# dgrzech/ir-sgmcmc

Measured on AMD Instinct MI355X. Metric: SG-MCMC transitions/sec (full _SGLD_transition), higher is better.
Workload: dtype f32; 1 GPU; 256^3 synthetic pair, SVF_3D 12 steps, GMM(K=4)/LCC(s=1) + virtual decimation, RegLoss_L2 w=1.4, Sobolev s=3, uniform noise 0.1, SGLD lr 0.4, Philox noise; init=identity, chains=1, parallelism=1 independent chain(s)

## Files before the change

### include/irsgmcmc.h

```cpp
#ifndef IRSGMCMC_H
#define IRSGMCMC_H

#include <stddef.h>
#include <stdint.h>

#ifdef __cplusplus
extern "C" {
#endif
#pragma GCC visibility push(default)

#define IRS_MAX_COMPONENTS 8
#define IRS_MAX_CHAINS 8
#define IRS_MAX_HALF_WIDTH 4
#define IRS_MAX_LABELS 64
#define IRS_HAUSDORFF_MAX_PERCENTILES 4

enum { IRS_DATA_GMM_LCC = 0, IRS_DATA_SSD = 1 };
enum { IRS_REG_L2 = 0, IRS_REG_LOGNORMAL = 1, IRS_REG_STUDENT = 2, IRS_REG_LOGNORMAL_L2 = 3 };


int irs_perturb_smooth(const float* v, const float* sigma, const float* eps, float tau, const float* kernel, int s,
                       int C, int D, int H, int W, float* tmp, float* out, uint64_t seed, uint64_t iteration,
                       void* stream);

// ... 178 lines not shown
#define IRS_RESIDUAL_MAX_BINS 512
#define IRS_RESIDUAL_MAX_BLOCKS 1024
#define IRS_RESIDUAL_WS_BYTES (IRS_MAX_CHAINS * IRS_RESIDUAL_MAX_BLOCKS * (3 + 4) * 8)
#define IRS_RESIDUAL_MAP_SUMMARY_INTS 2
#define IRS_RESIDUAL_MAP_SUMMARY_FLOATS 2
#define IRS_RESIDUAL_MAP_WS_BYTES (1024 * (IRS_RESIDUAL_MAP_SUMMARY_INTS + IRS_RESIDUAL_MAP_SUMMARY_FLOATS) * 8)
int irs_residual_histogram(const float* residuals, int C, const uint8_t* mask, int D, int H, int W, float half_range, int bins,
                           long long* hist, long long* counts, double* sums, int records_before, void* ws, size_t ws_bytes,
                           void* stream);
int irs_residual_nll_update(const float* residuals, int C, int D, int H, int W, const double* log_weight, const double* inv_std,
                            int K, float* mean, int32_t* count, int records_before, void* stream);
int irs_residual_nll_finalize(const float* mean, const int32_t* count, const uint8_t* mask, int D, int H, int W,
                              long long* isummary, double* fsummary, void* ws, size_t ws_bytes, void* stream);

int irs_restrict_image(const float* im, int Cim, int D, int H, int W, float* out, int d, int h, int w, void* stream);
int irs_restrict_mask(const uint8_t* mask, int Cm, int D, int H, int W, uint8_t* out, int d, int h, int w, void* stream);
int irs_prolong_field(const float* x, int C, int ch, int d, int h, int w, float* out, int D, int H, int W, void* stream);

#define IRS_AFFINE_SUMS 94
#define IRS_AFFINE_PARTIALS 76
#define IRS_AFFINE_MAX_BLOCKS 512
#define IRS_AFFINE_WS_BYTES (IRS_AFFINE_MAX_BLOCKS * IRS_AFFINE_PARTIALS * 8)
int irs_affine_normal_equations(const float* fixed, const float* moving, const uint8_t* mask, int D, int H, int W, const double* lin,
                                const double* shift, double* sums, void* ws, size_t ws_bytes, void* stream);
int irs_affine_transformation(const double* lin, const double* shift, float* out, int D, int H, int W, void* stream);
int irs_affine_compose(const float* transformation, const double* lin, const double* shift, float* total_transformation,
                       float* total_displacement, int C, int D, int H, int W, void* stream);

int irs_bspline_prefilter(const float* im, float* coeff, int Cim, int D, int H, int W, void* stream);
int irs_bspline_warp(const float* coeff, int Cim, const float* transformation, float* out, int C, int D, int H, int W, void* stream);
int irs_native_warp_cubic(const float* displacement, int C, const int32_t* dims, const int32_t* native, const int32_t* padding,
                          const float* im, const float* coeff, int Cim, float fill, float* im_out, void* stream);

#define IRS_MASK_MIN_BINS 2
#define IRS_MASK_MAX_BINS 4096
#define IRS_MASK_MAX_KEEP 64
#define IRS_MASK_MAX_RADIUS 16
int irs_intensity_histogram(const float* im, int C, const uint8_t* mask, int Cm, int D, int H, int W, float lo, float hi, int bins,
                            long long* hist, void* stream);
int irs_mask_threshold(const float* im, int C, int D, int H, int W, float threshold, uint8_t* out, void* stream);
int irs_connected_components_workspace(int C, int D, int H, int W, size_t* bytes);
int irs_connected_components(const uint8_t* mask, int C, int D, int H, int W, int connectivity, int32_t* labels, int32_t* counts,
                             void* ws, size_t ws_bytes, void* stream);
int irs_mask_select_workspace(int C, int D, int H, int W, size_t* bytes);
int irs_mask_keep_largest(const uint8_t* mask, int C, int D, int H, int W, int connectivity, int keep, uint8_t* out, void* ws,
                          size_t ws_bytes, void* stream);
int irs_mask_fill_holes(const uint8_t* mask, int C, int D, int H, int W, uint8_t* out, void* ws, size_t ws_bytes, void* stream);
int irs_mask_morphology_workspace(int C, int D, int H, int W, size_t* bytes);
int irs_mask_dilate(const uint8_t* mask, int C, int D, int H, int W, int r2, int erode, uint8_t* out, void* ws, size_t ws_bytes,
                    void* stream);

#define IRS_LANDMARK_MAX_POINTS (1 << 24)
#define IRS_LANDMARK_COLUMNS 10
#define IRS_LANDMARK_SUMMARY_INTS 3
#define IRS_LANDMARK_SUMMARY_FLOATS 4
#define IRS_LANDMARK_WS_BYTES (1024 * (IRS_LANDMARK_SUMMARY_INTS + IRS_LANDMARK_SUMMARY_FLOATS) * 8)
int irs_transform_points(const float* points, int K, const float* displacement, int C, int D, int H, int W, const float* scale,
                         const float* offset, float* sampled, float* mapped, void* stream);
int irs_landmark_update(const float* mapped, const float* target, int C, int K, double* mean, double* comoment, double* tre_mean,
                        double* tre_m2, double* tre_max, int32_t* count, int records_before, void* stream);
int irs_landmark_finalize(const double* mean, const double* comoment, const double* tre_mean, const double* tre_m2,
                          const double* tre_max, const int32_t* count, const float* target, int K, double* out, long long* isummary,
                          double* fsummary, void* ws, size_t ws_bytes, void* stream);


typedef struct irs_config {
    int32_t dims[3];
    int32_t cps[3];
    int32_t no_chains;
    int32_t no_steps;
    int32_t sobolev_s;
    float sobolev_kernel[2 * IRS_MAX_HALF_WIDTH + 1];
    float lr;
    float uniform_alpha;
    int32_t virtual_decimation;
    int32_t data_loss;
    int32_t lcc_s;
    int32_t gmm_components;
    float ssd_sigma;
    float gmm_lr_log_std, gmm_lr_logits, gmm_lr_decay;
    float adam_beta1, adam_beta2, adam_eps;
    float scale_prior_loc, scale_prior_scale;
    float dirichlet_concentration[IRS_MAX_COMPONENTS];
    int32_t reg_loss;
    int32_t reg_learnable;
    float w_reg;
    double dof;
    float reg_lr0, reg_lr1, reg_lr_decay;
    float loc_prior_nu, loc_prior_w_reg;
    float reg_scale_prior_loc, reg_scale_prior_scale;
    double w_reg_prior_shape, w_reg_prior_rate;
    uint64_t seed;
} irs_config;

typedef struct irs_state {
    float gmm_log_std[IRS_MAX_COMPONENTS];
    float gmm_logits[IRS_MAX_COMPONENTS];
    double gmm_adam_m[2][IRS_MAX_COMPONENTS];
    double gmm_adam_v[2][IRS_MAX_COMPONENTS];
    int64_t gmm_adam_step[2];
    double reg_param[2];
    double reg_adam_m[2], reg_adam_v[2];
    int64_t reg_adam_step[2];
    uint64_t iteration;
} irs_state;

typedef struct irs_scalars {
    double alpha[IRS_MAX_CHAINS];
    double data_term[IRS_MAX_CHAINS];
    double reg_term[IRS_MAX_CHAINS];
    double reg_energy[IRS_MAX_CHAINS];
    double n_mask[IRS_MAX_CHAINS];
} irs_scalars;

typedef struct irs_io {
    const float* fixed_im;
    const float* moving_im;
    const uint8_t* mask;
    int32_t fixed_chains, moving_chains, mask_chains;
    float* v;
    const float* sigma;
    const float* eps;
    const float* unif;
    float* curr_state;
    float* im_moving_warped;
    float* residuals;
    float* displacement;
    float* transformation;
    float* grad_v;
} irs_io;

typedef struct irs_ctx irs_ctx;

int irs_create(const irs_config* cfg, irs_ctx** out);
void irs_destroy(irs_ctx* ctx);
size_t irs_workspace_bytes(const irs_ctx* ctx);
int irs_velocity_dims(const irs_ctx* ctx, int32_t out[3]);

int irs_set_fixed(irs_ctx* ctx, const float* fixed_im, int fixed_chains, void* stream);
int irs_get_state(irs_ctx* ctx, irs_state* out, void* stream);
int irs_set_state(irs_ctx* ctx, const irs_state* in, void* stream);
int irs_get_scalars(irs_ctx* ctx, irs_scalars* out, void* stream);

int irs_gmm_init(irs_ctx* ctx, const irs_io* io, const float* v_sample, int warm_up, void* stream);

int irs_transition(irs_ctx* ctx, const irs_io* io, void* stream);

int irs_flush(irs_ctx* ctx, void* stream);
int irs_recovered_transitions(const irs_ctx* ctx, uint64_t* out);
int irs_sparse_adjoint_set(irs_ctx* ctx, int on);
int irs_sparse_adjoint_get(irs_ctx* ctx, int32_t* out, void* stream);
int irs_sparse_data_set(irs_ctx* ctx, int on);
int irs_sparse_data_get(irs_ctx* ctx, int32_t* out, void* stream);

typedef struct irs_timings {
    float total_ms;
    float exp_fwd_ms;
    float exp_bwd_kernel_ms;
    float exp_bwd_total_ms;
    float smooth_ms;
    float data_ms;
    float update_ms;
    float exp_bwd_primary_avg_ms;
} irs_timings;
int irs_transition_timed(irs_ctx* ctx, const irs_io* io, void* stream, irs_timings* out);

typedef struct irs_comm irs_comm;
#define IRS_COMM_ID_BYTES 128
int irs_comm_unique_id(uint8_t id[IRS_COMM_ID_BYTES]);
int irs_comm_create_rccl(const uint8_t id[IRS_COMM_ID_BYTES], int rank, int world, irs_comm** out);
int irs_comm_create_ipc(const char* name, int rank, int world, irs_comm** out);
typedef struct irs_xfer {
    void* ptr;
    size_t bytes;
    int32_t peer;
    int32_t recv;
} irs_xfer;
typedef int (*irs_exchange_fn)(void* user, const irs_xfer* xfers, int n, void* stream);
typedef int (*irs_allreduce_fn)(void* user, void* buf, size_t count, int kind, void* stream);
int irs_comm_create_callbacks(irs_exchange_fn ex, irs_allreduce_fn ar, void* user, int rank, int world, irs_comm** out);
void irs_comm_destroy(irs_comm* comm);
int irs_comm_probe(irs_comm* comm, size_t bytes, size_t ar_doubles, int iters, void* stream, double usec[2]);
int irs_comm_describe(const irs_comm* comm, char* out, size_t n);
int irs_comm_rank(const irs_comm* comm);
int irs_comm_world(const irs_comm* comm);
int irs_comm_selftest(irs_comm* comm, void* stream);

typedef struct irs_slab_config {
    int32_t ghost_max;
    int32_t margin;
} irs_slab_config;
typedef struct irs_slab_layout {
    int32_t rank, world;
    int32_t a, b;
    int32_t lo, hi;
    int32_t margin, ghost_max;
} irs_slab_layout;
int irs_slab_plan_layout(const irs_config* cfg, const irs_slab_config* scfg, int rank, int world, irs_slab_layout* out);
int irs_slab_create(const irs_config* cfg, const irs_slab_config* scfg, irs_comm* comm, irs_ctx** out);
int irs_slab_get_layout(const irs_ctx* ctx, irs_slab_layout* out);
int irs_slab_transition(irs_ctx* ctx, const irs_io* io, void* stream);
int irs_slab_gmm_init(irs_ctx* ctx, const irs_io* io, const float* v_sample, int warm_up, void* stream);
typedef struct irs_slab_status {
    uint64_t transitions, exact_transitions;
    uint64_t exchanges, exchanged_bytes;
    uint64_t mispredictions;
    int32_t last_fwd_rounds, last_bwd_rounds;
} irs_slab_status;
int irs_slab_status_get(irs_ctx* ctx, irs_slab_status* out, void* stream);
typedef struct irs_slab_timeline_entry {
    int32_t kind;
    int32_t stage;
    int32_t k, width;
    float ready_us;
    float handover_us;
    float wait_at_us;
    float stall_us;
} irs_slab_timeline_entry;
int irs_slab_timeline_arm(irs_ctx* ctx, int transitions);
int irs_slab_timeline_get(irs_ctx* ctx, irs_slab_timeline_entry* out, int max_entries, int32_t* n_entries, float* total_us, void* stream);

int irs_slab_plan_rounds(const int32_t* h, int n, int ghost_max, int min_slab, int n_buffers, int32_t* fwd_round, int32_t* fwd_width,
                         int32_t* n_fwd, int32_t* bwd_round, int32_t* bwd_width, int32_t* n_bwd);

enum { IRS_OP_LAUNCH = 0, IRS_OP_EXCHANGE = 1, IRS_OP_ALLREDUCE = 2, IRS_OP_WAIT = 3 };
enum {
    IRS_SG_PERTURB = 0, IRS_SG_COPY_V, IRS_SG_SMOOTH, IRS_SG_ENERGY, IRS_SG_EXP_FWD, IRS_SG_OUTPUTS, IRS_SG_WARP, IRS_SG_RESIDUAL,
    IRS_SG_STATS, IRS_SG_DATA_BWD, IRS_SG_WARP_BWD, IRS_SG_EXP_BWD, IRS_SG_UPDATE, IRS_SG_FFD_UP, IRS_SG_FFD_ADJ,
    IRS_SG_SCALARS = 32,
    IRS_SG_CHAIN_SCALAR = 32, IRS_SG_REG_SCALAR, IRS_SG_FINALIZE, IRS_SG_VERDICT
};
enum {
    IRS_SB_V = 0, IRS_SB_NOISY, IRS_SB_VS, IRS_SB_WARPED, IRS_SB_Z, IRS_SB_GM, IRS_SB_GRAD_A, IRS_SB_GRAD_B,
    IRS_SB_DENSE,
    IRS_SB_GRAD_C,
    IRS_SB_STEP0 = 16
};
enum { IRS_AR_ENERGY = 0, IRS_AR_DMAX = 1, IRS_AR_NLL = 2, IRS_AR_STATS = 3, IRS_AR_CPGRAD = 4, IRS_AR_MOMENTS = 7 };
typedef struct irs_slab_op {
    int32_t kind;
    int32_t stage;
    int32_t k;
    int32_t lo0, hi0, lo1, hi1;
    int32_t in0, in1;
    int32_t reach;
    int32_t out;
    int32_t width;
    int32_t id;
} irs_slab_op;
int irs_slab_trace(const irs_config* cfg, const irs_slab_config* scfg, int rank, int world, const int32_t* h, irs_slab_op* ops,
                   int max_ops, int32_t* n_ops);

int irs_option_set(irs_ctx* ctx, const char* name, int value);

const char* irs_last_error(void);
const char* irs_version(void);

#pragma GCC visibility pop
#ifdef __cplusplus
}
#endif
#endif
```

### ir_sgmcmc_amd/_lib.py

```python
import ctypes as C
import os

import torch

_HERE = os.path.dirname(os.path.abspath(__file__))
LIB_PATH = os.environ.get('IRS_LIB') or os.path.join(_HERE, 'csrc', 'libirsgmcmc.so')

IRS_MAX_COMPONENTS = 8
IRS_MAX_CHAINS = 8
IRS_MAX_HALF_WIDTH = 4
IRS_MAX_LABELS = 64
IRS_HAUSDORFF_MAX_PERCENTILES = 4
IRS_LABEL_BINS = 10
IRS_JACOBIAN_SUMMARY_INTS, IRS_JACOBIAN_SUMMARY_FLOATS = 4, 5
IRS_JACOBIAN_WS_BYTES = 1024 * (IRS_JACOBIAN_SUMMARY_INTS + IRS_JACOBIAN_SUMMARY_FLOATS) * 8
IRS_IMAGE_POSTERIOR_MAX_VOLUMES, IRS_IMAGE_POSTERIOR_SUMMARY_INTS, IRS_IMAGE_POSTERIOR_SUMMARY_FLOATS = 8, 4, 6
IRS_IMAGE_POSTERIOR_WS_BYTES = 1024 * (IRS_IMAGE_POSTERIOR_SUMMARY_INTS + IRS_IMAGE_POSTERIOR_SUMMARY_FLOATS) * 8
IRS_COVARIANCE_SUMMARY_INTS, IRS_COVARIANCE_SUMMARY_FLOATS = 2, 8
IRS_COVARIANCE_WS_BYTES = 1024 * (IRS_COVARIANCE_SUMMARY_INTS + IRS_COVARIANCE_SUMMARY_FLOATS) * 8
IRS_COMPARE_SUMMARY_INTS, IRS_COMPARE_SUMMARY_FLOATS = 4, 13
IRS_COMPARE_WS_BYTES = 1024 * (IRS_COMPARE_SUMMARY_INTS + IRS_COMPARE_SUMMARY_FLOATS) * 8
IRS_QUANTILE_MIN_BINS, IRS_QUANTILE_MAX_BINS, IRS_QUANTILE_MAX_PROBS, IRS_QUANTILE_MAX_RECORDS = 4, 256, 8, 65535
IRS_QUANTILE_SUMMARY_INTS, IRS_QUANTILE_SUMMARY_FLOATS = 3, 5
IRS_QUANTILE_WS_BYTES = 1024 * (IRS_QUANTILE_SUMMARY_INTS + IRS_QUANTILE_SUMMARY_FLOATS) * 8
# ... 61 lines not shown
        ('fixed_im', C.c_void_p), ('moving_im', C.c_void_p), ('mask', C.c_void_p),
        ('fixed_chains', C.c_int32), ('moving_chains', C.c_int32), ('mask_chains', C.c_int32),
        ('v', C.c_void_p), ('sigma', C.c_void_p), ('eps', C.c_void_p), ('unif', C.c_void_p),
        ('curr_state', C.c_void_p), ('im_moving_warped', C.c_void_p), ('residuals', C.c_void_p),
        ('displacement', C.c_void_p), ('transformation', C.c_void_p), ('grad_v', C.c_void_p),
    ]


class IrsTimings(C.Structure):
    _fields_ = [(n, C.c_float) for n in ('total_ms', 'exp_fwd_ms', 'exp_bwd_kernel_ms', 'exp_bwd_total_ms', 'smooth_ms',
                                         'data_ms', 'update_ms', 'exp_bwd_primary_avg_ms')]


class IrsXfer(C.Structure):
    _fields_ = [('ptr', C.c_void_p), ('bytes', C.c_size_t), ('peer', C.c_int32), ('recv', C.c_int32)]


class IrsSlabConfig(C.Structure):
    _fields_ = [('ghost_max', C.c_int32), ('margin', C.c_int32)]


class IrsSlabLayout(C.Structure):
    _fields_ = [(n, C.c_int32) for n in ('rank', 'world', 'a', 'b', 'lo', 'hi', 'margin', 'ghost_max')]


class IrsSlabStatus(C.Structure):
    _fields_ = [('transitions', C.c_uint64), ('exact_transitions', C.c_uint64), ('exchanges', C.c_uint64),
                ('exchanged_bytes', C.c_uint64), ('mispredictions', C.c_uint64), ('last_fwd_rounds', C.c_int32),
                ('last_bwd_rounds', C.c_int32)]


class IrsSlabTimelineEntry(C.Structure):
    _fields_ = [('kind', C.c_int32), ('stage', C.c_int32), ('k', C.c_int32), ('width', C.c_int32), ('ready_us', C.c_float),
                ('handover_us', C.c_float), ('wait_at_us', C.c_float), ('stall_us', C.c_float)]


class IrsSlabOp(C.Structure):
    _fields_ = [(n, C.c_int32) for n in ('kind', 'stage', 'k', 'lo0', 'hi0', 'lo1', 'hi1', 'in0', 'in1', 'reach', 'out', 'width', 'id')]


IRS_OP_LAUNCH, IRS_OP_EXCHANGE, IRS_OP_ALLREDUCE, IRS_OP_WAIT = range(4)
(IRS_SG_PERTURB, IRS_SG_COPY_V, IRS_SG_SMOOTH, IRS_SG_ENERGY, IRS_SG_EXP_FWD, IRS_SG_OUTPUTS, IRS_SG_WARP, IRS_SG_RESIDUAL, IRS_SG_STATS,
 IRS_SG_DATA_BWD, IRS_SG_WARP_BWD, IRS_SG_EXP_BWD, IRS_SG_UPDATE, IRS_SG_FFD_UP, IRS_SG_FFD_ADJ) = range(15)
IRS_SG_CHAIN_SCALAR, IRS_SG_REG_SCALAR, IRS_SG_FINALIZE = 32, 33, 34
(IRS_SB_V, IRS_SB_NOISY, IRS_SB_VS, IRS_SB_WARPED, IRS_SB_Z, IRS_SB_GM, IRS_SB_GRAD_A, IRS_SB_GRAD_B, IRS_SB_DENSE, IRS_SB_GRAD_C) = range(10)
IRS_SB_STEP0 = 16
IRS_COMM_ID_BYTES = 128
EXCHANGE_FN = C.CFUNCTYPE(C.c_int, C.c_void_p, C.POINTER(IrsXfer), C.c_int, C.c_void_p)
ALLREDUCE_FN = C.CFUNCTYPE(C.c_int, C.c_void_p, C.c_void_p, C.c_size_t, C.c_int, C.c_void_p)

_P, _I, _F, _U64 = C.c_void_p, C.c_int, C.c_float, C.c_uint64
_I32P = C.POINTER(C.c_int32)

SIGNATURES = {
    'irs_perturb_smooth': [_P, _P, _P, _F, _P, _I, _I, _I, _I, _I, _P, _P, _U64, _U64, _P],
    'irs_svf_exp_fwd': [_P, _P, _P, _P, _I, _I, _I, _I, _I, _P],
    'irs_svf_exp_bwd': [_P, _P, _P, _P, _P, _I, _I, _I, _I, _I, _P],
    'irs_ffd_up': [_P, _P, _P, _I, _I, _I, _I, _I, _I, _I, _P],
    'irs_ffd_adjoint': [_P, _P, _P, _I, _I, _I, _I, _I, _I, _I, _P],
    'irs_warp_fwd': [_P, _I, _P, _P, _F, _P, _I, _I, _I, _I, _U64, _U64, _P],
    'irs_warp_bwd': [_P, _I, _P, _P, _F, _P, _P, _I, _I, _I, _I, _U64, _U64, _P],
    'irs_warp_transformation': [_P, _I, _P, _P, _I, _I, _I, _I, _P],
    'irs_warp_nearest_u8': [_P, _I, _P, _P, _I, _I, _I, _I, _P],
    'irs_warp_nearest_i16': [_P, _I, _P, _P, _I, _I, _I, _I, _P],
    'irs_lcc_normalise': [_P, _P, _P, _I, _I, _I, _I, _I, _P],
    'irs_lcc_map_fwd': [_P, _I, _P, _P, _P, _I, _I, _I, _I, _I, _P],
    'irs_lcc_map_bwd': [_P, _I, _P, _P, _P, _P, _I, _I, _I, _I, _I, _P],
    'irs_reg_energy': [_P, _P, _P, _I, _I, _I, _I, _P],
    'irs_reduce_scratch_doubles': [],
    'irs_gradient_operator': [_P, _P, _I, _I, _I, _I, _I, _P],
    'irs_log_det_jacobian': [_P, _P, _P, _I, _I, _I, _I, _P],
    'irs_label_boxes': [_P, _I, _P, _I32P, _I, _P, _I, _I, _I, _I, _P],
    'irs_surface_distance_workspace': [_I32P, _I, _I, _I, _I, C.POINTER(C.c_size_t)],
    'irs_label_surface_distance': [_P, _I, _P, _I32P, _I, C.POINTER(C.c_float), _I32P, _P, C.c_size_t, _P, _P, _I, _I, _I, _I,
                                   _P],
    'irs_hausdorff_workspace': [_I32P, _I, _I, _I, _I, _I, C.POINTER(C.c_size_t)],
    'irs_label_hausdorff_distance': [_P, _I, _P, _I32P, _I, C.POINTER(C.c_float), _I32P, _P, C.c_size_t, C.POINTER(C.c_double), _I,
                                     _P, _P, _P, _P, _I, _I, _I, _I, _P],
    'irs_surface_posterior_workspace': [_I32P, _I, _I, _I, _I, C.POINTER(C.c_size_t)],
    'irs_surface_posterior_update': [_P, _P, _I32P, _I, C.POINTER(C.c_float), _I32P, _P, C.c_size_t, _P, _P, _P, _I, _I, _I, _I, _P],
    'irs_surface_posterior_finalize': [_P, _I32P, _I, _P, _P, _P, _P, C.POINTER(C.c_double), _I, _P, _P, _P, _P, _P, C.c_size_t,
                                       _I, _I, _I, _P],
    'irs_chain_moments_update': [_P, _I, _I, _I, _I, _I, _I, _P, _P, _P],
    'irs_split_rhat_workspace': [_I, _I, _I, _I, C.POINTER(C.c_size_t)],
    'irs_split_rhat': [_P, _P, _I, _I, _P, C.c_float, C.c_float, _P, _P, _P, C.c_size_t, _I, _I, _I, _P],
    'irs_chain_variogram_update': [_P, _I, _I, _I, _I, _I, _I, _P, _P, _P],
    'irs_split_ess_workspace': [_I, _I, _I, _I, C.POINTER(C.c_size_t)],
    'irs_split_ess': [_P, _P, _P, _I, _I, _I, _P, C.c_float, _P, _P, _P, _P, C.c_size_t, _I, _I, _I, _P],
    'irs_label_posterior_workspace': [_I, _I, _I, _I, _I, C.POINTER(C.c_size_t)],
    'irs_label_posterior_update': [_P, _I, _I, _I, _I, _I32P, _I, _P, _P, _I, _P, C.c_size_t, _P],
    'irs_label_posterior_finalize': [_P, _I, _I, _I, _I, _I, _I32P, _P, _P, _P, _P, _P, _P, _P, C.c_size_t, _P],
    'irs_jacobian_posterior_update': [_P, _I, _I, _I, _I, _P, _P, _P, _I, _P],
    'irs_jacobian_posterior_finalize': [_P, _P, _P, _I, _I, _I, _I, _P, _P, _P, _P, _P, _P, _P, C.c_size_t, _P],
    'irs_image_posterior_update': [_P, _I, _P, _I, _I, _I, _I, _P, _P, _P, _P, _I, _P],
    'irs_image_posterior_finalize': [_P, _P, _P, _P, _I, _I, _I, _I, _P, _F, _P, _P, _P, _P, _P, _P, _P, C.c_size_t, _P],
    'irs_displacement_covariance_update': [_P, _I, _I, _I, _I, _P, _P, _I, _P],
    'irs_displacement_covariance_finalize': [_P, _P, _I, _I, _I, _I, C.POINTER(C.c_float), _P, _P, _P, _P, _P, _P, _P, C.c_size_t, _P],
    'irs_posterior_compare': [_P, _P, _I, _P, _P, _I, _I, _I, _I, C.POINTER(C.c_float), C.c_double, _P, _P, _P, _P, _P, _P, _P, _P, C.c_size_t,
                              _P],
    'irs_displacement_quantiles_update': [_P, _I, _I, _I, _I, _P, _P, _I, C.POINTER(C.c_float), _I, _P],
    'irs_displacement_quantiles_finalize': [_P, _P, _I, _I, _I, _I, _I, C.POINTER(C.c_float), C.POINTER(C.c_float),
                                            C.POINTER(C.c_double), _I, _P, _P, _P, _P, _P, _P, C.c_size_t, _P],
    'irs_svf_exp_inverse': [_P, _P, _P, _P, _I, _I, _I, _I, _I, _P],
    'irs_inverse_consistency': [_P, _P, _P, C.POINTER(C.c_float), _P, _I, _P, _P, _P, _P, _P, C.c_size_t, _I, _I, _I, _I, _P],
    'irs_inverse_consistency_update': [_P, _I, _I, _I, _I, _P, _P, _I, _P],
    'irs_inverse_consistency_finalize': [_P, _P, _I, _I, _I, _P, _F, _P, _P, _P, C.c_size_t, _P],
    'irs_native_warp': [_P, _I, _I32P, _I32P, _I32P, _P, _P, _P, _I, _F, C.POINTER(C.c_float), _P, _P, _P, _P, _P],
    'irs_image_similarity_workspace': [_I, _I, C.POINTER(C.c_size_t)],
    'irs_image_similarity': [_P, _I, _P, _I, _P, _I, _I, _I, _F, _F, _F, _F, _I, _P, _P, _P, C.c_size_t, _P],
    'irs_transform_points': [_P, _I, _P, _I, _I, _I, _I, C.POINTER(C.c_float), _P, _P, _P, _P],
    'irs_landmark_update': [_P, _P, _I, _I, _P, _P, _P, _P, _P, _P, _I, _P],
    'irs_landmark_finalize': [_P, _P, _P, _P, _P, _P, _P, _I, _P, _P, _P, _P, C.c_size_t, _P],
    'irs_local_similarity': [_P, _I, _P, _I, _P, _I, _I, _I, _I, C.c_double, C.c_double, C.c_double, C.c_double, _P, _P, _P, _P,
                             C.c_size_t, _P],
    'irs_local_similarity_update': [_P, _I, _I, _I, _I, _P, _P, _P, _I, _P],
    'irs_local_similarity_finalize': [_P, _P, _P, _P, _I, _I, _I, _P, _P, _P, C.c_size_t, _P],
    'irs_residual_histogram': [_P, _I, _P, _I, _I, _I, _F, _I, _P, _P, _P, _I, _P, C.c_size_t, _P],
    'irs_residual_nll_update': [_P, _I, _I, _I, _I, C.POINTER(C.c_double), C.POINTER(C.c_double), _I, _P, _P, _I, _P],
    'irs_residual_nll_finalize': [_P, _P, _P, _I, _I, _I, _P, _P, _P, C.c_size_t, _P],
    'irs_restrict_image': [_P, _I, _I, _I, _I, _P, _I, _I, _I, _P],
    'irs_restrict_mask': [_P, _I, _I, _I, _I, _P, _I, _I, _I, _P],
    'irs_prolong_field': [_P, _I, _I, _I, _I, _I, _P, _I, _I, _I, _P],
    'irs_affine_normal_equations': [_P, _P, _P, _I, _I, _I, C.POINTER(C.c_double), C.POINTER(C.c_double), _P, _P, C.c_size_t, _P],
    'irs_affine_transformation': [C.POINTER(C.c_double), C.POINTER(C.c_double), _P, _I, _I, _I, _P],
    'irs_affine_compose': [_P, C.POINTER(C.c_double), C.POINTER(C.c_double), _P, _P, _I, _I, _I, _I, _P],
    'irs_bspline_prefilter': [_P, _P, _I, _I, _I, _I, _P],
    'irs_bspline_warp': [_P, _I, _P, _P, _I, _I, _I, _I, _P],
    'irs_native_warp_cubic': [_P, _I, _I32P, _I32P, _I32P, _P, _P, _I, _F, _P, _P],
    'irs_intensity_histogram': [_P, _I, _P, _I, _I, _I, _I, _F, _F, _I, _P, _P],
    'irs_mask_threshold': [_P, _I, _I, _I, _I, _F, _P, _P],
    'irs_connected_components_workspace': [_I, _I, _I, _I, C.POINTER(C.c_size_t)],
    'irs_connected_components': [_P, _I, _I, _I, _I, _I, _P, _P, _P, C.c_size_t, _P],
    'irs_mask_select_workspace': [_I, _I, _I, _I, C.POINTER(C.c_size_t)],
    'irs_mask_keep_largest': [_P, _I, _I, _I, _I, _I, _I, _P, _P, C.c_size_t, _P],
    'irs_mask_fill_holes': [_P, _I, _I, _I, _I, _P, _P, C.c_size_t, _P],
    'irs_mask_morphology_workspace': [_I, _I, _I, _I, C.POINTER(C.c_size_t)],
    'irs_mask_dilate': [_P, _I, _I, _I, _I, _I, _I, _P, _P, C.c_size_t, _P],
    'irs_create': [C.POINTER(IrsConfig), C.POINTER(_P)],
    'irs_destroy': [_P],
    'irs_workspace_bytes': [_P],
    'irs_velocity_dims': [_P, C.POINTER(C.c_int32 * 3)],
    'irs_set_fixed': [_P, _P, _I, _P],
    'irs_get_state': [_P, C.POINTER(IrsState), _P],
    'irs_set_state': [_P, C.POINTER(IrsState), _P],
    'irs_get_scalars': [_P, C.POINTER(IrsScalars), _P],
    'irs_gmm_init': [_P, C.POINTER(IrsIO), _P, _I, _P],
    'irs_transition': [_P, C.POINTER(IrsIO), _P],
    'irs_flush': [_P, _P],
    'irs_recovered_transitions': [_P, C.POINTER(C.c_uint64)],
    'irs_sparse_adjoint_set': [_P, _I],
    'irs_sparse_adjoint_get': [_P, _I32P, _P],
    'irs_sparse_data_set': [_P, _I],
    'irs_sparse_data_get': [_P, _I32P, _P],
    'irs_transition_timed': [_P, C.POINTER(IrsIO), _P, C.POINTER(IrsTimings)],
    'irs_comm_unique_id': [C.POINTER(C.c_uint8 * IRS_COMM_ID_BYTES)],
    'irs_comm_create_rccl': [C.POINTER(C.c_uint8 * IRS_COMM_ID_BYTES), _I, _I, C.POINTER(_P)],
    'irs_comm_create_ipc': [C.c_char_p, _I, _I, C.POINTER(_P)],
    'irs_comm_create_callbacks': [EXCHANGE_FN, ALLREDUCE_FN, _P, _I, _I, C.POINTER(_P)],
    'irs_comm_destroy': [_P],
    'irs_comm_probe': [_P, C.c_size_t, C.c_size_t, _I, _P, C.POINTER(C.c_double * 2)],
    'irs_comm_describe': [_P, C.c_char_p, C.c_size_t],
    'irs_comm_rank': [_P],
    'irs_comm_world': [_P],
    'irs_comm_selftest': [_P, _P],
    'irs_slab_plan_layout': [C.POINTER(IrsConfig), C.POINTER(IrsSlabConfig), _I, _I, C.POINTER(IrsSlabLayout)],
    'irs_slab_create': [C.POINTER(IrsConfig), C.POINTER(IrsSlabConfig), _P, C.POINTER(_P)],
    'irs_slab_get_layout': [_P, C.POINTER(IrsSlabLayout)],
    'irs_slab_transition': [_P, C.POINTER(IrsIO), _P],
    'irs_slab_gmm_init': [_P, C.POINTER(IrsIO), _P, _I, _P],
    'irs_slab_status_get': [_P, C.POINTER(IrsSlabStatus), _P],
    'irs_slab_timeline_arm': [_P, _I],
    'irs_slab_timeline_get': [_P, C.POINTER(IrsSlabTimelineEntry), _I, _I32P, C.POINTER(C.c_float), _P],
    'irs_slab_trace': [C.POINTER(IrsConfig), C.POINTER(IrsSlabConfig), _I, _I, _I32P, C.POINTER(IrsSlabOp), _I, _I32P],
    'irs_slab_plan_rounds': [_I32P, _I, _I, _I, _I, _I32P, _I32P, _I32P, _I32P, _I32P, _I32P],
    'irs_option_set': [_P, C.c_char_p, _I],
    'irs_last_error': [],
    'irs_version': [],
}
_RESTYPES = {'irs_reduce_scratch_doubles': C.c_size_t, 'irs_workspace_bytes': C.c_size_t, 'irs_destroy': None,
             'irs_comm_destroy': None,
             'irs_last_error': C.c_char_p, 'irs_version': C.c_char_p}

_lib = None


class IrsError(RuntimeError):
    pass


def load(path=None):
    global _lib
    if _lib is not None and path is None:
        return _lib
    p = path or LIB_PATH
    if not os.path.isfile(p):
        raise IrsError(f'{p} not found: build it with `python -c "import __graft_entry__ as g; g.build()"` '
                       f'(or `make -C ir_sgmcmc_amd/csrc`). There is no CPU fallback.')
    lib = C.CDLL(p)
    for name, argtypes in SIGNATURES.items():
        fn = getattr(lib, name)
        fn.argtypes = argtypes
        fn.restype = _RESTYPES.get(name, C.c_int)
    if path is None:
        _lib = lib
    return lib


def option_set(name, value, ctx=None):
    check(load().irs_option_set(ctx, name.encode(), int(value)))


def check(rc):
    if rc != 0:
        raise IrsError(load().irs_last_error().decode())


def stream_ptr():
    return C.c_void_p(torch.cuda.current_stream().cuda_stream)


def dev_ptr(t, dtype=None, allow_none=False):
    if t is None:
        if allow_none:
            return None
        raise IrsError('required tensor is None')
    if not t.is_cuda:
        raise IrsError('ir_sgmcmc_amd operators run on the GPU only (got a CPU tensor); there is no CPU fallback')
    if dtype is not None and t.dtype != dtype:
        raise IrsError(f'expected {dtype}, got {t.dtype}')
    if not t.is_contiguous():
        raise IrsError('tensor must be contiguous')
    return C.c_void_p(t.data_ptr())
```

### ir_sgmcmc_amd/csrc/adjoint_plan.h

```cpp
#pragma once

#if defined(__HIPCC__)
#define IRS_HD __host__ __device__ inline
#else
#define IRS_HD inline
#endif

namespace irs {

#ifndef IRS_MTX
#define IRS_MTX 32
#define IRS_MTY 8
#endif
constexpr int kPlanTX = IRS_MTX, kPlanTY = IRS_MTY;
#ifndef IRS_BWD_MAX_SEG
#define IRS_BWD_MAX_SEG 64
#endif
constexpr int kPlanMaxLen = IRS_BWD_MAX_SEG;
constexpr int kPlanMinLen = 8;
constexpr int kPlanMinForced = 4;
constexpr int kPlanStats = 4;

struct PlanEntry {
    int chain, tile, z0, z1, fill, pad;
};

struct ColPlan {
    int lo, hi, f0, f1;
};

IRS_HD int plan_min(int a, int b) { return a < b ? a : b; }
IRS_HD int plan_max(int a, int b) { return a > b ? a : b; }

IRS_HD void plan_widen(int a, int b, int m, int D, int& lo, int& hi) {
    lo = hi = 0;
    if (b <= 0) return;
    lo = plan_max(D - a - m, 0);
    hi = plan_min(b + m, D);
}

IRS_HD ColPlan plan_column(int lo, int hi, int nlo, int nhi) {
    const bool run = hi > lo, need = nhi > nlo;
    if (!run) return need ? ColPlan{nhi, nhi, nlo, nhi} : ColPlan{0, 0, 0, 0};
    return ColPlan{lo, hi, need ? plan_min(lo, nlo) : lo, need ? plan_max(hi, nhi) : hi};
}

IRS_HD ColPlan plan_column_of(const int* runs, int k, int col, int C, int ntx, int nty, int D) {
    const int tiles = ntx * nty, chain = col / tiles, tile = col - chain * tiles, tx = tile % ntx, ty = tile / ntx;
    const int* r = runs + ((long long)k * C * tiles + col) * 2;
    int nlo = 0, nhi = D;
    if (k > 0) {
        nlo = D;
        nhi = 0;
        const int* prev = runs + ((long long)(k - 1) * C + chain) * tiles * 2;
        for (int dy = -1; dy <= 1; ++dy)
            for (int dx = -1; dx <= 1; ++dx) {
                const int ux = plan_min(plan_max(tx + dx, 0), ntx - 1), uy = plan_min(plan_max(ty + dy, 0), nty - 1);
                const int l = prev[(uy * ntx + ux) * 2], h = prev[(uy * ntx + ux) * 2 + 1];
                if (h > l) {
                    nlo = plan_min(nlo, plan_max(l - 1, 0));
                    nhi = plan_max(nhi, plan_min(h + 1, D));
                }
            }
    }
    return plan_column(r[0], r[1], nlo, nhi);
}

constexpr int kLccTX = 32, kLccTY = 16;
constexpr int kWarpTX = 64, kWarpTY = 8;
constexpr int kDataKernels = 4;
enum PlanFill { kFillNext = 0, kFillAll = 1, kFillNone = 2 };
struct PlanShape {
    int tx, ty;
    int reach0, reach_dec;
    int fill[2];
    int G[2];
    int lmin;
};
IRS_HD int plan_reach(const PlanShape& s, int k) { return s.reach0 - k * s.reach_dec; }
IRS_HD int plan_fill_of(const PlanShape& s, int k) { return s.fill[k > 0 ? 1 : 0]; }
IRS_HD int plan_resident_of(const PlanShape& s, int k) { return s.G[k > 0 ? 1 : 0]; }
IRS_HD void plan_tile_window(int t, int size, int m, int n, int& a, int& b) {
    a = plan_max(t * size - m, 0);
    b = plan_min(t * size + size + m, n);
}
IRS_HD ColPlan plan_column_by(const int* runs, int k, int col, int C, int ntx, int nty, int D, int fill) {
    if (fill == kFillNext) return plan_column_of(runs, k, col, C, ntx, nty, D);
    const int* r = runs + ((long long)k * C * ntx * nty + col) * 2;
    return fill == kFillAll ? plan_column(r[0], r[1], 0, D) : plan_column(r[0], r[1], 0, 0);
}

IRS_HD int plan_pieces(int len, int L) { return len > 0 ? (len + L - 1) / L : 0; }

IRS_HD void plan_cut(int lo, int len, int np, int j, int& z0, int& z1) {
    z0 = lo + (int)((long long)len * j / np);
    z1 = lo + (int)((long long)len * (j + 1) / np);
}

IRS_HD PlanEntry plan_entry(const ColPlan& c, int chain, int tile, int np, int j) {
    int z0, z1;
    plan_cut(c.lo, c.hi - c.lo, np, j, z0, z1);
    return PlanEntry{chain, tile, z0, z1, 0, 0};
}
IRS_HD bool plan_has_fill(const ColPlan& c, int side) { return side == 0 ? c.f0 < c.lo : c.hi < c.f1 && c.hi > c.lo; }
IRS_HD PlanEntry plan_fill_entry(const ColPlan& c, int chain, int tile, int side) {
    return side == 0 ? PlanEntry{chain, tile, c.f0, c.lo, 1, 0} : PlanEntry{chain, tile, c.hi, c.f1, 1, 0};
}

IRS_HD int plan_pick_len(const int* pieces, int G, int lmin, int lmax) {
    for (int L = lmin; L < lmax; ++L)
        if (pieces[L] <= G) return L;
    return lmax;
}

IRS_HD int plan_run_bound(int columns, int D, int G, int forced_len) {
    const int lmax = plan_max(plan_min(kPlanMaxLen, D), 1);
    if (forced_len > 0) return columns * plan_pieces(D, plan_min(plan_max(forced_len, kPlanMinForced), lmax));
    return plan_max(G, columns * plan_pieces(D, lmax));
}

IRS_HD int plan_entries_cap(int columns, int D) { return columns * ((D + kPlanMinForced - 1) / kPlanMinForced + 2); }

IRS_HD int plan_swizzle(int id, int count, int run) {
    if (run <= 1) return id;
    const int group = 8 * run;
    if (id >= count / group * group) return id;
    const int g = id / group, w = id - g * group;
    return g * group + (w & 7) * run + (w >> 3);
}

}
```

### ir_sgmcmc_amd/csrc/adjoint_plan.hip

```cpp
#include "adjoint_plan.h"

#include "kernels.h"

namespace irs {

constexpr int kExtChunk = 32;

template <typename T>
__device__ __forceinline__ void extent_body(const T* __restrict__ g, int* __restrict__ ext, const Vol& vol) {
    const int x = (int)blockIdx.x * 64 + ((int)threadIdx.x & 63), y = (int)blockIdx.y * 4 + ((int)threadIdx.x >> 6);
    const int nch = (vol.D + kExtChunk - 1) / kExtChunk;
    const int chain = (int)blockIdx.z / nch, za = ((int)blockIdx.z - chain * nch) * kExtChunk, zb = min(za + kExtChunk, vol.D);
    if (x >= vol.W || y >= vol.H) return;
    const int64_t plane = (int64_t)vol.H * vol.W;
    const T* __restrict__ p = g + (int64_t)chain * vol.V + (int64_t)y * vol.W + x;
    int lo = vol.D, hi = -1;
#pragma unroll 8
    for (int z = za; z < zb; ++z) {
        const bool nz = p[z * plane] != (T)0;
        lo = nz ? min(lo, z) : lo;
        hi = nz ? z : hi;
    }
    if (hi < 0) return;
    int* e = ext + ((int64_t)chain * plane + (int64_t)y * vol.W + x) * 2;
// ... 14 lines not shown
    else hipLaunchKernelGGL(mask_extent_kernel, grid, dim3(kBlock), 0, st, mask, ext, vol);
}

__device__ __forceinline__ bool chain_is_dense(const unsigned* __restrict__ dmax, int chain, int C, int no_steps) {
    bool dense = false;
    if (!dmax) return false;
    for (int k = 0; k < no_steps; ++k) {
        const unsigned* b = dmax + ((int64_t)k * C + chain) * 4;
        const float m = fmaxf(fmaxf(__uint_as_float(b[0]), __uint_as_float(b[1])), __uint_as_float(b[2]));
        dense |= !(m < 1.0f);
    }
    return dense;
}

__global__ __launch_bounds__(kWave) void plan_runs_kernel(const int* __restrict__ ext, int ext_chains, const unsigned* __restrict__ dmax,
                                                          int* __restrict__ runs, Vol vol, int C, int no_steps, int ntx, int nty,
                                                          PlanShape shape) {
    const int col = (int)blockIdx.x, k = (int)blockIdx.y, tiles = ntx * nty;
    const int chain = col / tiles, tile = col - chain * tiles, tx = tile % ntx, ty = tile / ntx;
    int* out = runs + ((int64_t)k * C * tiles + col) * 2;
    if (chain_is_dense(dmax, chain, C, no_steps)) {
        if (threadIdx.x == 0) {
            out[0] = 0;
            out[1] = vol.D;
        }
        return;
    }
    const int m = plan_reach(shape, k);
    int x0, x1, y0, y1;
    plan_tile_window(tx, shape.tx, m, vol.W, x0, x1);
    plan_tile_window(ty, shape.ty, m, vol.H, y0, y1);
    const int nx = x1 - x0, n = nx * (y1 - y0);
    const int* __restrict__ e = ext + (int64_t)(ext_chains == 1 ? 0 : chain) * vol.H * vol.W * 2;
    int lo = vol.D, hi = 0;
    for (int i = (int)threadIdx.x; i < n; i += kWave) {
        const int yy = i / nx, xx = i - yy * nx;
        const int2 ab = *reinterpret_cast<const int2*>(e + ((int64_t)(y0 + yy) * vol.W + x0 + xx) * 2);
        int l, h;
        plan_widen(ab.x, ab.y, m, vol.D, l, h);
        if (h > l) {
            lo = min(lo, l);
            hi = max(hi, h);
        }
    }
#pragma unroll
    for (int off = kWave / 2; off > 0; off >>= 1) {
        lo = min(lo, __shfl_xor(lo, off, kWave));
        hi = max(hi, __shfl_xor(hi, off, kWave));
    }
    if (threadIdx.x == 0) {
        out[0] = hi > lo ? lo : 0;
        out[1] = hi > lo ? hi : 0;
    }
}

constexpr int kPlanBlock = 1024;
__device__ __forceinline__ int block_rank(bool flag, int* wave_tot, int& total) {
    const unsigned long long b = __ballot(flag);
    const int lane = (int)threadIdx.x & (kWave - 1), w = (int)threadIdx.x / kWave;
    if (lane == 0) wave_tot[w] = __popcll(b);
    __syncthreads();
    int before = 0;
    total = 0;
#pragma unroll
    for (int i = 0; i < kPlanBlock / kWave; ++i) {
        before += i < w ? wave_tot[i] : 0;
        total += wave_tot[i];
    }
    __syncthreads();
    return before + __popcll(b & ((1ull << lane) - 1ull));
}

__global__ __launch_bounds__(kPlanBlock) void plan_lists_kernel(const int* __restrict__ runs, const unsigned* __restrict__ dmax,
                                                                ColPlan* __restrict__ colplan, PlanEntry* __restrict__ entries,
                                                                int* __restrict__ count, int* __restrict__ stats, Vol vol, int C,
                                                                int no_steps, int ntx, int nty, int cap, PlanShape shape, int forced_len) {
    __shared__ int pieces[kPlanMaxLen + 1], s_maxlen, s_L, s_nrun, wave_tot[kPlanBlock / kWave];
    __shared__ int s_pieces[IRS_MAX_CHAINS], s_planes[IRS_MAX_CHAINS];
    const int k = (int)blockIdx.x, tiles = ntx * nty, cols = C * tiles, tid = (int)threadIdx.x;
    const int lmax = max(min(kPlanMaxLen, vol.D), 1), lmin = min(shape.lmin, lmax);
    const int fill = plan_fill_of(shape, k);
    ColPlan* __restrict__ cps = colplan + (int64_t)k * cols;
    for (int i = tid; i <= kPlanMaxLen; i += kPlanBlock) pieces[i] = 0;
    if (tid < IRS_MAX_CHAINS) s_pieces[tid] = s_planes[tid] = 0;
    if (tid == 0) s_maxlen = s_nrun = 0;
    __syncthreads();
    for (int col = tid; col < cols; col += kPlanBlock) {
        const ColPlan cp = plan_column_by(runs, k, col, C, ntx, nty, vol.D, fill);
        cps[col] = cp;
        const int len = cp.hi - cp.lo;
        if (len > 0) {
            atomicMax(&s_maxlen, len);
            atomicAdd(&s_planes[col / tiles], len);
        }
    }
    __syncthreads();
    const int n_len = lmax - lmin + 1, groups = kPlanBlock / n_len;
    if (forced_len <= 0 && tid < groups * n_len) {
        const int L = lmin + tid % n_len;
        int sum = 0;
        for (int col = tid / n_len; col < cols; col += groups) sum += plan_pieces(cps[col].hi - cps[col].lo, L);
        atomicAdd(&pieces[L], sum);
    }
    __syncthreads();
    if (tid == 0)
        s_L = forced_len > 0 ? min(max(forced_len, kPlanMinForced), lmax) : plan_pick_len(pieces, plan_resident_of(shape, k), lmin, lmax);
    __syncthreads();
    const int L = s_L, levels = plan_pieces(s_maxlen, L);
    PlanEntry* list = entries + (int64_t)k * cap;
    const int stream = (levels + 2) * cols;
    int base = 0;
    for (int i0 = 0; i0 < stream; i0 += kPlanBlock) {
        const int i = i0 + tid;
        bool flag = false;
        ColPlan cp = {0, 0, 0, 0};
        int np = 0, j = 0, col = 0;
        if (i < stream) {
            j = i / cols;
            col = i - j * cols;
            cp = cps[col];
            np = plan_pieces(cp.hi - cp.lo, L);
            flag = j < levels ? j < np : plan_has_fill(cp, j - levels);
        }
        const unsigned long long runs_here = __ballot(flag && j < levels);
        if ((tid & (kWave - 1)) == 0 && runs_here) atomicAdd(&s_nrun, __popcll(runs_here));
        int total;
        const int pos = base + block_rank(flag, wave_tot, total);
        if (flag && pos < cap) {
            list[pos] = j < levels ? plan_entry(cp, col / tiles, col % tiles, np, j) : plan_fill_entry(cp, col / tiles, col % tiles, j - levels);
            atomicAdd(&s_pieces[col / tiles], 1);
        }
        base += total;
    }
    __syncthreads();
    if (tid == 0) {
        count[2 * k] = min(base, cap);
        count[2 * k + 1] = min(s_nrun, cap);
    }
    if (tid < C) {
        int* s = stats + ((int64_t)k * C + tid) * kPlanStats;
        s[0] = chain_is_dense(dmax, tid, C, no_steps) ? 0 : 1;
        s[1] = L;
        s[2] = s_pieces[tid];
        s[3] = s_planes[tid];
    }
}

static size_t plan_align(size_t b) { return (b + 255) / 256 * 256; }

struct PlanLayout {
    size_t ext, runs, colplan, entries, count, stats, total;
    int cap, ntx, nty;
};
static PlanLayout plan_layout(Vol vol, int C, int no_steps) {
    PlanLayout l;
    l.ntx = (vol.W + kPlanTX - 1) / kPlanTX;
    l.nty = (vol.H + kPlanTY - 1) / kPlanTY;
    const size_t cols = (size_t)C * l.ntx * l.nty;
    l.cap = plan_entries_cap((int)cols, vol.D);
    size_t off = 0;
    auto take = [&](size_t bytes) { const size_t o = off; off += plan_align(bytes); return o; };
    l.ext = take(sizeof(int) * 2 * (size_t)C * vol.H * vol.W);
    l.runs = take(sizeof(int) * 2 * cols * no_steps);
    l.colplan = take(sizeof(ColPlan) * cols * no_steps);
    l.entries = take(sizeof(PlanEntry) * (size_t)l.cap * no_steps);
    l.count = take(sizeof(int) * 2 * no_steps);
    l.stats = take(sizeof(int) * kPlanStats * (size_t)C * no_steps);
    l.total = off;
    return l;
}

size_t adjoint_plan_bytes(Vol vol, int C, int no_steps) { return plan_layout(vol, C, no_steps).total; }

AdjointPlan adjoint_plan_views(char* base, Vol vol, int C, int no_steps) {
    const PlanLayout l = plan_layout(vol, C, no_steps);
    AdjointPlan p;
    p.ext = (int*)(base + l.ext);
    p.runs = (int*)(base + l.runs);
    p.colplan = (ColPlan*)(base + l.colplan);
    p.entries = (PlanEntry*)(base + l.entries);
    p.count = (int*)(base + l.count);
    p.stats = (int*)(base + l.stats);
    p.cap = l.cap;
    p.ntx = l.ntx;
    p.nty = l.nty;
    return p;
}

void launch_adjoint_plan(const float* g_warped, const unsigned* dmax, const AdjointPlan& plan, int no_steps, int C, Vol vol,
                         int64_t G, int forced_len, hipStream_t st) {
    const int g = (int)(G > 0 ? G : 1024);
    const PlanShape shape{kPlanTX, kPlanTY, no_steps, 1, {kFillNext, kFillNext}, {g, g}, kPlanMinLen};
    launch_extent(g_warped, nullptr, plan.ext, C, vol, st);
    hipLaunchKernelGGL(plan_runs_kernel, dim3((unsigned)(C * plan.ntx * plan.nty), (unsigned)no_steps), dim3(kWave), 0, st, plan.ext, C, dmax,
                       plan.runs, vol, C, no_steps, plan.ntx, plan.nty, shape);
    hipLaunchKernelGGL(plan_lists_kernel, dim3((unsigned)no_steps), dim3(kPlanBlock), 0, st, plan.runs, dmax, plan.colplan, plan.entries, plan.count,
                       plan.stats, vol, C, no_steps, plan.ntx, plan.nty, plan.cap, shape, forced_len);
}

struct DataLayout {
    size_t ext, runs, hull, colplan, entries, count, stats, nll, total;
    int cap, ntx, nty, wtx, wty;
};
static DataLayout data_layout(Vol vol, int C) {
    DataLayout l;
    l.ntx = (vol.W + kLccTX - 1) / kLccTX;
    l.nty = (vol.H + kLccTY - 1) / kLccTY;
    l.wtx = (vol.W + kWarpTX - 1) / kWarpTX;
    l.wty = (vol.H + kWarpTY - 1) / kWarpTY;
    const size_t cols = (size_t)C * l.ntx * l.nty;
    l.cap = plan_entries_cap((int)cols, vol.D);
    size_t off = 0;
    auto take = [&](size_t bytes) { const size_t o = off; off += plan_align(bytes); return o; };
    l.ext = take(sizeof(int) * 2 * (size_t)C * vol.H * vol.W);
    l.runs = take(sizeof(int) * 2 * cols * 2);
    l.hull = take(sizeof(int) * 2 * (size_t)C * l.wtx * l.wty);
    l.colplan = take(sizeof(ColPlan) * cols * 2);
    l.entries = take(sizeof(PlanEntry) * (size_t)l.cap * 2);
    l.count = take(sizeof(int) * 2 * 2);
    l.stats = take(sizeof(int) * kPlanStats * (size_t)C * 2);
    l.nll = take(sizeof(double) * (size_t)l.cap);
    l.total = off;
    return l;
}

size_t data_plan_bytes(Vol vol, int C) { return data_layout(vol, C).total; }

DataPlan data_plan_views(char* base, Vol vol, int C) {
    const DataLayout l = data_layout(vol, C);
    DataPlan p;
    p.ext = (int*)(base + l.ext);
    p.runs = (int*)(base + l.runs);
    p.hull = (int*)(base + l.hull);
    p.colplan = (ColPlan*)(base + l.colplan);
    p.entries = (PlanEntry*)(base + l.entries);
    p.count = (int*)(base + l.count);
    p.stats = (int*)(base + l.stats);
    p.nll = (double*)(base + l.nll);
    p.cap = l.cap;
    p.ntx = l.ntx;
    p.nty = l.nty;
    p.wtx = l.wtx;
    p.wty = l.wty;
    return p;
}

static int data_list_resident(int s, bool bwd, int C) {
    const int64_t res = lcc_plan_resident(s, bwd, bwd && C > 1);
    return (int)(res > 0 ? res : 1024);
}
int data_plan_run_bound(const DataPlan& plan, int s, bool bwd, int C, Vol vol) {
    return plan_run_bound(C * plan.ntx * plan.nty, vol.D, data_list_resident(s, bwd, C), plan.forced_len);
}

void launch_data_plan(const uint8_t* mask, int mask_chains, const DataPlan& plan, int s, bool lists, int C, Vol vol, hipStream_t st) {
    launch_extent(nullptr, mask, plan.ext, mask_chains, vol, st);
    const PlanShape warp{kWarpTX, kWarpTY, 3 * s, 0, {kFillNone, kFillNone}, {1, 1}, kPlanMinLen};
    hipLaunchKernelGGL(plan_runs_kernel, dim3((unsigned)(C * plan.wtx * plan.wty), 1u), dim3(kWave), 0, st, plan.ext, mask_chains, nullptr,
                       plan.hull, vol, C, 1, plan.wtx, plan.wty, warp);
    if (!lists) return;
    const PlanShape lcc{kLccTX, kLccTY, 2 * s, s, {kFillAll, kFillNone}, {data_list_resident(s, true, C), data_list_resident(s, false, C)},
                        kPlanMinLen};
    hipLaunchKernelGGL(plan_runs_kernel, dim3((unsigned)(C * plan.ntx * plan.nty), 2u), dim3(kWave), 0, st, plan.ext, mask_chains, nullptr,
                       plan.runs, vol, C, 2, plan.ntx, plan.nty, lcc);
    hipLaunchKernelGGL(plan_lists_kernel, dim3(2u), dim3(kPlanBlock), 0, st, plan.runs, nullptr, plan.colplan, plan.entries, plan.count, plan.stats,
                       vol, C, 2, plan.ntx, plan.nty, plan.cap, lcc, plan.forced_len);
}

}
```

### ir_sgmcmc_amd/csrc/api_ctx.hip

```cpp
#include <math.h>
#include <string.h>

#include <new>

#include "adjoint_plan.h"
#include "api_checks.h"
#include "comm.h"

using namespace irs;

static size_t align_up(size_t x) { return (x + 255) & ~(size_t)255; }

static bool is_capturing(hipStream_t st) {
    hipStreamCaptureStatus cap = hipStreamCaptureStatusNone;
    (void)hipStreamIsCapturing(st, &cap);
    return cap != hipStreamCaptureStatusNone;
}


int irs::create_ctx(const irs_config* cfg, const SlabInfo* sl, irs_ctx** out) {
    if (!cfg || !out) return fail("irs_create: null argument");
    const int D = cfg->dims[0], H = cfg->dims[1], W = cfg->dims[2], C = cfg->no_chains;
    if (!dims_ok(C, D, H, W) || !chain_count_ok(C)) return fail("irs_create: bad dims / chains (C <= %d)", IRS_MAX_CHAINS);
    if (cfg->no_steps < 1 || cfg->no_steps > 30) return fail("irs_create: no_steps out of range");
    if (cfg->sobolev_s < 0 || cfg->sobolev_s > IRS_MAX_HALF_WIDTH) return fail("irs_create: sobolev_s out of range");
    if (cfg->data_loss != IRS_DATA_GMM_LCC && cfg->data_loss != IRS_DATA_SSD) return fail("irs_create: unknown data loss");
    if (cfg->data_loss == IRS_DATA_GMM_LCC) {
        if (!lcc_ok(cfg->lcc_s, D, H, W)) return fail("irs_create: LCC half width must be 1 or 2");
        if (cfg->gmm_components < 1 || cfg->gmm_components > IRS_MAX_COMPONENTS) return fail("irs_create: 1..%d mixture components", IRS_MAX_COMPONENTS);
    } else if (!(cfg->ssd_sigma > 0.0f)) return fail("irs_create: ssd_sigma must be positive");
    if (cfg->reg_loss < IRS_REG_L2 || cfg->reg_loss > IRS_REG_LOGNORMAL_L2) return fail("irs_create: unknown regulariser");
    if ((cfg->reg_loss == IRS_REG_STUDENT || cfg->reg_loss == IRS_REG_LOGNORMAL_L2) && cfg->reg_learnable)
        return fail("irs_create: RegLoss_Student / RegLoss_LogNormal_L2 have no learnable parameters");
    if (cfg->reg_loss == IRS_REG_STUDENT && !(cfg->w_reg_prior_rate > 0.0 && cfg->w_reg_prior_shape > 0.0))
        return fail("irs_create: RegLoss_Student needs a0 > 0 and b0 > 0 (w_reg_prior_shape / w_reg_prior_rate)");
    const bool any_cps = cfg->cps[0] || cfg->cps[1] || cfg->cps[2];
    if (any_cps && (cfg->cps[0] < 1 || cfg->cps[1] < 1 || cfg->cps[2] < 1 || cfg->cps[0] > 8 || cfg->cps[1] > 8 || cfg->cps[2] > 8))
        return fail("irs_create: control point spacing must be 1..8 on every axis");

    irs_ctx* c = new (std::nothrow) irs_ctx();
    if (!c) return fail("irs_create: out of host memory");
    memset((void*)c, 0, sizeof(*c));
    context_born();
    c->kn = global_knobs();
    c->sparse_adjoint = true;
    c->sparse_data = 1;
    c->cfg = *cfg;
    c->C = C;
    c->vol = make_vol(D, H, W);
    if (sl && sl->on) {
        c->sl = *sl;
        c->vol.V = (int64_t)(sl->hi - sl->lo) * H * W;
    }
    c->ffd = any_cps;
    c->volv = c->ffd ? make_vol(control_points(D, cfg->cps[0]), control_points(H, cfg->cps[1]), control_points(W, cfg->cps[2]))
                     : c->vol;
    c->sob.s = cfg->sobolev_s;
    for (int i = 0; i <= 2 * cfg->sobolev_s; ++i) c->sob.k[i] = cfg->sobolev_kernel[i];
    if (c->ffd)
        for (int a = 0; a < 3; ++a) c->spl[a] = make_spline(cfg->cps[a]);

    DevCfg& d = c->dcfg;
    d.K = cfg->data_loss == IRS_DATA_GMM_LCC ? cfg->gmm_components : 1;
    d.mode = cfg->data_loss;
    d.vd = cfg->virtual_decimation;
    d.C = C;
    d.gmm_lr_log_std = cfg->gmm_lr_log_std;
    d.gmm_lr_logits = cfg->gmm_lr_logits;
    d.gmm_lr_decay = cfg->gmm_lr_decay;
    d.beta1 = cfg->adam_beta1 > 0 ? cfg->adam_beta1 : 0.9f;
    d.beta2 = cfg->adam_beta2 > 0 ? cfg->adam_beta2 : 0.999f;
    d.eps = cfg->adam_eps > 0 ? cfg->adam_eps : 1e-8f;
    d.scale_prior_loc = cfg->scale_prior_loc;
    d.scale_prior_scale = cfg->scale_prior_scale;
    for (int k = 0; k < IRS_MAX_COMPONENTS; ++k) d.conc[k] = cfg->dirichlet_concentration[k];
    d.reg_loss = cfg->reg_loss;
    d.reg_learnable = cfg->reg_learnable;
    d.dof = cfg->dof;
    d.reg_lr0 = cfg->reg_lr0;
    d.reg_lr1 = cfg->reg_lr1;
    d.reg_lr_decay = cfg->reg_lr_decay;
    d.loc_prior_nu = cfg->loc_prior_nu;
    d.loc_prior_w_reg = cfg->loc_prior_w_reg;
    d.reg_scale_prior_loc = cfg->reg_scale_prior_loc;
    d.reg_scale_prior_scale = cfg->reg_scale_prior_scale;
    d.w_reg_prior_shape = cfg->w_reg_prior_shape;
    d.w_reg_prior_rate = cfg->w_reg_prior_rate;

    const size_t fieldI = (size_t)C * 3 * c->vol.V * sizeof(float);
    const size_t fieldV = (size_t)C * 3 * c->volv.V * sizeof(float);
    const size_t imageI = (size_t)C * c->vol.V * sizeof(float);
    size_t ffd_tmp = 0;
    if (c->ffd) {
        const size_t planes = (size_t)(c->vol.V / ((int64_t)H * W)), g1 = c->volv.H, g2 = c->volv.W;
        ffd_tmp = sizeof(float) * (size_t)C * 3 * planes * ((size_t)g1 * g2 + (size_t)H * g2 + (size_t)H * W);
    }
    c->nll_seg_C = (C > 1 && !sl && cfg->data_loss == IRS_DATA_GMM_LCC && c->kn.data_batch != 0) ? C : 1;
    c->nll_blocks = data_bwd_blocks(cfg->data_loss, c->vol, c->nll_seg_C);
    size_t off = 0;
    auto take = [&](size_t bytes) { size_t o = off; off += align_up(bytes); return o; };
    const size_t o_steps = take(fieldI * cfg->no_steps);
    const size_t o_tmpA = take(fieldV > ffd_tmp ? fieldV : ffd_tmp);
    const size_t o_tmpB = take(fieldV);
    const size_t o_vs = take(fieldV);
    const size_t o_gA = take(fieldI), o_gB = take(fieldI);
    const bool third = sl && sl->on && sl->world > 1;
    const size_t o_gC = third ? take(fieldI) : 0;
    const size_t o_warped = take(imageI), o_z = take(imageI), o_sig = take(imageI), o_fhat = take(imageI), o_gM = take(imageI);
    const size_t o_dense = take(c->ffd ? fieldI : 0);
    const size_t o_stat = take(sizeof(double) * kMaxPartialBlocks * kStatVals);
    const size_t o_energy = take(sizeof(double) * kMaxPartialBlocks * IRS_MAX_CHAINS);
    const size_t o_nll = take(sizeof(double) * (size_t)c->nll_blocks * C);
    const size_t o_sums = take(sizeof(double) * (kStatVals + 2 * IRS_MAX_CHAINS));
    const size_t o_dmax = take(sizeof(unsigned) * 4 * IRS_MAX_CHAINS * 32);
    const size_t o_cmm = take(coarse_minmax_bytes(c->vol, C));
    const bool planned = !sl;
    const size_t o_plan = take(planned ? adjoint_plan_bytes(c->vol, C, cfg->no_steps) : 0);
    const size_t o_dplan = take(planned ? data_plan_bytes(c->vol, C) : 0);
    const size_t o_state = take(sizeof(DevState));
    c->slab_bytes = off;
    if (hipMalloc((void**)&c->slab, off) != hipSuccess) {
        irs_destroy(c);
        return fail("irs_create: hipMalloc of %zu workspace bytes failed", off);
    }
    if (hipMemset(c->slab, 0, off) != hipSuccess ||
        hipMemsetD32((hipDeviceptr_t)(c->slab + o_sig), 0x3f800000, imageI / sizeof(float)) != hipSuccess) {
        irs_destroy(c);
        return fail("irs_create: clearing the workspace failed");
    }
    c->steps = (float*)(c->slab + o_steps);
    c->tmpA = (float*)(c->slab + o_tmpA);
    c->tmpB = (float*)(c->slab + o_tmpB);
    c->vs = (float*)(c->slab + o_vs);
    c->gA = (float*)(c->slab + o_gA);
    c->gB = (float*)(c->slab + o_gB);
    c->gC = third ? (float*)(c->slab + o_gC) : nullptr;
    c->warped = (float*)(c->slab + o_warped);
    c->z = (float*)(c->slab + o_z);
    c->sigM = (float*)(c->slab + o_sig);
    c->fhat = (float*)(c->slab + o_fhat);
    c->gM = (float*)(c->slab + o_gM);
    c->dense = c->ffd ? (float*)(c->slab + o_dense) : nullptr;
    c->stat_partials = (double*)(c->slab + o_stat);
    c->energy_partials = (double*)(c->slab + o_energy);
    c->nll_partials = (double*)(c->slab + o_nll);
    c->stat_sum = (double*)(c->slab + o_sums);
    c->energy_sum = c->stat_sum + kStatVals;
    c->nll_sum = c->energy_sum + IRS_MAX_CHAINS;
    c->dmax = (unsigned*)(c->slab + o_dmax);
    c->cmm = (float*)(c->slab + o_cmm);
    if (planned) c->plan = adjoint_plan_views(c->slab + o_plan, c->vol, C, cfg->no_steps);
    if (planned) c->dplan = data_plan_views(c->slab + o_dplan, c->vol, C);
    c->state = (DevState*)(c->slab + o_state);

    if (ensure_lin_tables(c->lin, D, H, W, nullptr)) {
        irs_destroy(c);
        return fail("irs_create: identity grid allocation failed");
    }
    DevState init;
    memset(&init, 0, sizeof(init));
    init.K = d.K;
    init.mode = d.mode;
    init.ssd_inv_sigma = cfg->data_loss == IRS_DATA_SSD ? 1.0f / cfg->ssd_sigma : 0.0f;
    if (cfg->reg_loss == IRS_REG_L2 || cfg->reg_loss == IRS_REG_LOGNORMAL_L2) init.st.reg_param[0] = log((double)cfg->w_reg);
    for (int ch = 0; ch < IRS_MAX_CHAINS; ++ch) init.sc.alpha[ch] = 1.0;
    hipError_t e = hipMemcpy(c->state, &init, sizeof(init), hipMemcpyHostToDevice);
    if (e == hipSuccess) {
        launch_refresh_derived(c->state, c->dcfg, nullptr);
        e = hipDeviceSynchronize();
    }
    for (int i = 0; i < 8 && e == hipSuccess; ++i) e = hipEventCreate(&c->ev[i]);
    for (int i = 0; i < 64 && e == hipSuccess; ++i) e = hipEventCreate(&c->ev_bwd[i]);
    for (int i = 0; i < 4 && e == hipSuccess; ++i) e = hipEventCreateWithFlags(&c->ra_ev[i], hipEventDisableTiming);
    if (c->C > 1 && !c->sl.on && c->kn.chain_overlap) {
        if (e == hipSuccess) e = hipStreamCreateWithFlags(&c->side, hipStreamNonBlocking);
        for (int i = 0; i < 2 * c->C && e == hipSuccess; ++i) e = hipEventCreateWithFlags(&c->ev_side[i], hipEventDisableTiming);
    }
    if (e == hipSuccess) e = hipHostMalloc((void**)&c->hint, sizeof(unsigned) * kHintWords, hipHostMallocDefault);
    if (e == hipSuccess)
        for (int i = 0; i < kHintWords; ++i) c->hint[i] = i < kHintWords - 8 ? 0x7f800000u : 0u;
    if (e != hipSuccess) {
        irs_destroy(c);
        return fail("irs_create: state initialisation failed: %s", hipGetErrorString(e));
    }
    *out = c;
    return 0;
}

int irs::check_io(const irs_ctx* c, const irs_io* io, const char* who) {
    if (!c || !io) return fail("%s: null argument", who);
    if (!io->fixed_im || !io->moving_im || !io->mask) return fail("%s: fixed_im, moving_im and mask are required", who);
    if (!broadcast_ok(io->fixed_chains, c->C) || !broadcast_ok(io->moving_chains, c->C) || !broadcast_ok(io->mask_chains, c->C))
        return fail("%s: *_chains must be 1 or no_chains", who);
    if (c->cfg.data_loss == IRS_DATA_GMM_LCC && !c->fixed_set) return fail("%s: call irs_set_fixed first", who);
    return 0;
}

extern "C" {

int irs_create(const irs_config* cfg, irs_ctx** out) { return irs::create_ctx(cfg, nullptr, out); }

void irs_destroy(irs_ctx* c) {
    if (!c) return;
    (void)hipDeviceSynchronize();
    if (c->sl.on) slab_release(c);
    for (int i = 0; i < 8; ++i)
        if (c->ev[i]) (void)hipEventDestroy(c->ev[i]);
    for (int i = 0; i < 64; ++i)
        if (c->ev_bwd[i]) (void)hipEventDestroy(c->ev_bwd[i]);
    for (int i = 0; i < 4; ++i)
        if (c->ra_ev[i]) (void)hipEventDestroy(c->ra_ev[i]);
    for (int i = 0; i < 2 * IRS_MAX_CHAINS; ++i)
        if (c->ev_side[i]) (void)hipEventDestroy(c->ev_side[i]);
    if (c->side) (void)hipStreamDestroy(c->side);
    if (c->lin.dev) (void)hipFree(c->lin.dev);
    if (c->hint) (void)hipHostFree(c->hint);
    if (c->slab) (void)hipFree(c->slab);
    delete c;
    context_gone();
}

size_t irs_workspace_bytes(const irs_ctx* c) { return c ? c->slab_bytes : 0; }

int irs_velocity_dims(const irs_ctx* c, int32_t out[3]) {
    if (!c || !out) return fail("irs_velocity_dims: null argument");
    out[0] = c->volv.D;
    out[1] = c->volv.H;
    out[2] = c->volv.W;
    return 0;
}

int irs_set_fixed(irs_ctx* c, const float* fixed_im, int fixed_chains, void* stream) {
    if (!c || !fixed_im || !broadcast_ok(fixed_chains, c->C)) return fail("irs_set_fixed: bad arguments");
    if (c->cfg.data_loss == IRS_DATA_GMM_LCC) {
        Vol w = c->vol;
        int64_t shift = 0;
        if (c->sl.on) {
            const int ls = c->cfg.lcc_s;
            w = window(c->vol, c->sl.lo + (c->sl.lo > 0 ? 2 * ls : 0), c->sl.hi - (c->sl.hi < c->vol.D ? 2 * ls : 0));
            shift = (int64_t)c->sl.lo * c->vol.H * c->vol.W;
        }
        launch_lcc_fwd_march(nullptr, 0, fixed_im - shift, c->fhat - shift, nullptr, c->cfg.lcc_s, fixed_chains, w, (hipStream_t)stream);
        LAUNCH_CHECK();
    }
    c->fhat_chains = fixed_chains;
    c->fixed_set = true;
    return 0;
}

static int flush_or_failed_transport(irs_ctx* c, void* stream) {
    if (!irs_flush(c, stream)) return 0;
    if (!(c->sl.on && c->comm && irs::comm_check(c->comm))) return 1;
    (void)hipStreamSynchronize((hipStream_t)stream);
    if (c->cs) (void)hipStreamSynchronize(c->cs);
    return 0;
}

int irs_get_state(irs_ctx* c, irs_state* out, void* stream) {
    if (!c || !out) return fail("irs_get_state: null argument");
    if (flush_or_failed_transport(c, stream)) return 1;
    HIP_TRY(hipMemcpyAsync(out, &c->state->st, sizeof(irs_state), hipMemcpyDeviceToHost, (hipStream_t)stream));
    HIP_TRY(hipStreamSynchronize((hipStream_t)stream));
    return 0;
}

static void drop_pending(irs_ctx* c);

int irs_set_state(irs_ctx* c, const irs_state* in, void* stream) {
    if (!c || !in) return fail("irs_set_state: null argument");
    if (is_capturing((hipStream_t)stream))
        return fail("irs_set_state: the stream is being captured -- this call waits for the stream, which a capture forbids");
    HIP_TRY(hipStreamSynchronize((hipStream_t)stream));
    if (c->sl.on) irs::slab_drop_pending(c);
    else drop_pending(c);
    HIP_TRY(hipMemcpyAsync(&c->state->st, in, sizeof(irs_state), hipMemcpyHostToDevice, (hipStream_t)stream));
    launch_refresh_derived(c->state, c->dcfg, (hipStream_t)stream);
    LAUNCH_CHECK();
    HIP_TRY(hipStreamSynchronize((hipStream_t)stream));
    return 0;
}

int irs_get_scalars(irs_ctx* c, irs_scalars* out, void* stream) {
    if (!c || !out) return fail("irs_get_scalars: null argument");
    if (flush_or_failed_transport(c, stream)) return 1;
    HIP_TRY(hipMemcpyAsync(out, &c->state->sc, sizeof(irs_scalars), hipMemcpyDeviceToHost, (hipStream_t)stream));
    HIP_TRY(hipStreamSynchronize((hipStream_t)stream));
    return 0;
}

static int forward_pass(irs_ctx* c, const irs_io* io, const float* v, bool with_noise, bool with_jitter, float* vs,
                        float* warped, float* z, float* gradm, int chains, hipStream_t st, int timed, int data_on = 0) {
    const irs_config& cfg = c->cfg;
    const int C = chains;
    const uint64_t* it = &c->state->st.iteration;
    if (!c->dmax_clean) HIP_TRY(hipMemsetAsync(c->dmax, 0, sizeof(unsigned) * 4 * c->C * (cfg.no_steps + 1), st));
    c->dmax_clean = false;
    bool have_dmax0 = false;
    const float amp = (float)sqrt(2.0 * (double)cfg.lr);
    if (with_noise && cfg.sobolev_s > 0 && !c->ffd && c->kn.fuse_noise && !(io->sigma && io->eps)) {
        have_dmax0 = true;
        launch_perturb_sobolev_march(v, io->sigma, io->eps, amp, vs, c->sob, C, c->volv, c->dmax, cfg.no_steps, cfg.seed, 0, it, st);
    } else {
        float* first = cfg.sobolev_s > 0 ? c->tmpA : vs;
        if (with_noise) launch_perturb(v, io->sigma, io->eps, amp, first, C, c->volv, cfg.seed, 0, it, st);
        else HIP_TRY(hipMemcpyAsync(first, v, (size_t)C * 3 * c->volv.V * sizeof(float), hipMemcpyDeviceToDevice, st));
        if (cfg.sobolev_s > 0) {
            have_dmax0 = !c->ffd;
            launch_sobolev_march(c->tmpA, vs, c->sob, C * 3, c->volv, have_dmax0 ? c->dmax : nullptr, cfg.no_steps, st);
        }
    }
    const float* dense = vs;
    if (c->ffd) {
        const int G[3] = {c->volv.D, c->volv.H, c->volv.W};
        ffd_up(vs, c->dense, c->tmpA, C, c->vol, G, c->spl, st);
        dense = c->dense;
    }
    if (timed) HIP_TRY(hipEventRecord(c->ev[1], st));
    const int64_t field = (int64_t)c->C * 3 * c->vol.V;
    const Lin lin = c->lin.lin();
    if (!have_dmax0) launch_field_absmax(dense, true, cfg.no_steps, c->dmax, C, c->vol, st);
    for (int k = 0; k < cfg.no_steps; ++k) {
        const float* in = k == 0 ? dense : c->steps + (int64_t)(k - 1) * field;
        float* out = c->steps + (int64_t)k * field;
        launch_exp_step_fwd_march(in, out, k == 0, cfg.no_steps, C, c->vol, lin, c->dmax + (int64_t)k * c->C * 4,
                                  c->dmax + (int64_t)(k + 1) * c->C * 4, predicted_small(c, k), fwd_lay(c, k), st);
    }
    if (timed) HIP_TRY(hipEventRecord(c->ev[2], st));
    const float* d_last = c->steps + (int64_t)(cfg.no_steps - 1) * field;
    const float alpha = with_jitter ? cfg.uniform_alpha : 0.0f;
    launch_warp_fwd(io->moving_im, io->moving_chains == 1 ? 0 : c->vol.V, d_last, io->unif, alpha, warped, gradm, 1, C, c->vol, lin,
                    cfg.seed, 0, it, st, data_on > 0 ? c->dplan.hull : nullptr);
    if (cfg.data_loss == IRS_DATA_GMM_LCC && data_on > 1)
        launch_lcc_fwd_plan(c->fhat, c->fhat_chains == 1 ? 0 : c->vol.V, warped, z, c->sigM, cfg.lcc_s, C, c->vol, c->dplan, st);
    else if (cfg.data_loss == IRS_DATA_GMM_LCC)
        launch_lcc_fwd_march(c->fhat, c->fhat_chains == 1 ? 0 : c->vol.V, warped, z, c->sigM, cfg.lcc_s, C, c->vol, st);
    else
        launch_residual_ssd(io->fixed_im, io->fixed_chains == 1 ? 0 : c->vol.V, warped, z, C, c->vol, st);
    LAUNCH_CHECK();
    return 0;
}

int irs_gmm_init(irs_ctx* c, const irs_io* io, const float* v_sample, int warm_up, void* stream) {
    if (check_io(c, io, "irs_gmm_init")) return 1;
    if (c->cfg.data_loss != IRS_DATA_GMM_LCC) return 0;
    hipStream_t st = (hipStream_t)stream;
    const size_t bytes = (size_t)3 * c->volv.V * sizeof(float);
    if (v_sample) HIP_TRY(hipMemcpyAsync(c->tmpB, v_sample, bytes, hipMemcpyDeviceToDevice, st));
    else HIP_TRY(hipMemsetAsync(c->tmpB, 0, bytes, st));
    if (forward_pass(c, io, c->tmpB, false, false, c->vs, c->warped, c->z, nullptr, 1, st, 0)) return 1;
    launch_masked_moments(c->z, io->mask, c->stat_partials, c->vol, st);
    launch_gmm_init_from_moments(c->state, c->stat_partials, stats_blocks(c->vol), c->dcfg, st);
    launch_stats(c->cfg.virtual_decimation, c->z, io->mask, c->state, c->stat_partials, c->vol, st, c->dcfg.K);
    launch_chain_scalar(c->state, c->stat_partials, stats_blocks(c->vol), 0, 1, c->dcfg, st);
    for (int i = 0; i < warm_up; ++i) {
        launch_stats(0, c->z, io->mask, c->state, c->stat_partials, c->vol, st, c->dcfg.K);
        launch_chain_scalar(c->state, c->stat_partials, stats_blocks(c->vol), 0, 2, c->dcfg, st);
    }
    LAUNCH_CHECK();
    return 0;
}

static int enqueue_transition(irs_ctx* c, const irs_io* io, hipStream_t st, int timed, bool no_assumptions) {

    const irs_config& cfg = c->cfg;
    const int C = c->C;
    const Vol vol = c->vol, volv = c->volv;
    const Lin lin = c->lin.lin();
    float* vs = io->curr_state ? io->curr_state : c->vs;
    float* warped = io->im_moving_warped ? io->im_moving_warped : c->warped;
    float* z = io->residuals ? io->residuals : c->z;
    const uint64_t* it = &c->state->st.iteration;
    const int saved_mode = c->kn.predict_variants;
    if (no_assumptions) c->kn.predict_variants = 0;
    struct Restore {
        irs_ctx* c;
        int mode;
        ~Restore() { c->kn.predict_variants = mode; }
    } restore{c, saved_mode};

    bool skip_any[32], skip_r2[32];
    note_hint_trend(c);
    Verdict vd = no_verdict();
    vd.bounds = c->dmax;
    vd.n = cfg.no_steps;
    vd.C = C;
    for (int k = 0; k < cfg.no_steps && k < 32; ++k) {
        skip_any[k] = predicted_below(c, k, global_knobs().lds_from <= 2 ? 0.75f : 1.5f);
        skip_r2[k] = skip_any[k] && predicted_tiny(c, k);
        if (skip_r2[k]) vd.need_lt1 |= 1u << k;
        else if (skip_any[k]) (global_knobs().lds_from > 2 ? vd.need_lt2 : vd.need_lt1) |= 1u << k;
    }

    if (timed) HIP_TRY(hipEventRecord(c->ev[0], st));
    const bool fuse_warp_bwd = c->kn.fuse_warp_bwd != 0;
    const bool lcc = cfg.data_loss == IRS_DATA_GMM_LCC;
    const int forced_piece = c->sparse_data > 1 ? c->sparse_data : 0;
    int data_on = 0;
    c->dplan.forced_len = forced_piece;
    if (c->sparse_data && c->dplan.entries && !io->im_moving_warped && !io->residuals &&
        (forced_piece > 0 || plan_min(lcc_dense_seg_len(vol, C, false), lcc_dense_seg_len(vol, c->nll_seg_C, true)) > kPlanMinLen)) {
        const bool one_launch = C == 1 || (c->kn.data_batch != 0 && !(c->side && c->kn.chain_overlap != 0));
        data_on = !lcc ? 1 : one_launch ? 3 : 2;
        launch_data_plan(io->mask, io->mask_chains, c->dplan, lcc ? cfg.lcc_s : 0, lcc, C, vol, st);
    }
    c->data_on = data_on;
    if (forward_pass(c, io, io->v, true, cfg.uniform_alpha > 0.0f, vs, warped, z, fuse_warp_bwd ? c->gA : nullptr, C, st, timed, data_on)) return 1;
    const int64_t field = (int64_t)C * 3 * vol.V;
    const float* d_last = c->steps + (int64_t)(cfg.no_steps - 1) * field;
    if (io->transformation || io->displacement) launch_svf_outputs(d_last, io->transformation, io->displacement, C, vol, lin, st);

    const int upd_blocks = sgld_update_blocks_per_chain(volv, C);
    const bool energy_in_update = (cfg.reg_loss == IRS_REG_L2 || cfg.reg_loss == IRS_REG_LOGNORMAL_L2) &&
                                  (int64_t)upd_blocks * C <= (int64_t)kMaxPartialBlocks * IRS_MAX_CHAINS &&
                                  c->kn.energy_in_update != 0;
    if (!energy_in_update) {
        launch_reg_energy(vs, c->energy_partials, C, volv, st);
        launch_reg_scalar(c->state, c->energy_partials, energy_blocks(volv), c->dcfg, st, vd);
    }

    const int sb = stats_blocks(vol);
    const bool overlap = C > 1 && c->side && c->kn.chain_overlap != 0;
    const bool batch = C > 1 && !overlap && cfg.data_loss == IRS_DATA_GMM_LCC && c->kn.data_batch != 0;
    for (int ch = 0; ch < C; ++ch) {
        const uint8_t* mask = io->mask + (io->mask_chains == 1 ? 0 : (int64_t)ch * vol.V);
        const float* zc = z + (int64_t)ch * vol.V;
        launch_stats(cfg.virtual_decimation, zc, mask, c->state, c->stat_partials, vol, st, c->dcfg.K);
        if (overlap && ch > 0) HIP_TRY(hipStreamWaitEvent(st, c->ev_side[2 * (ch - 1) + 1], 0));
        launch_chain_scalar(c->state, c->stat_partials, sb, ch, (ch == 0 ? 7 : 3) | (batch ? 8 : 0), c->dcfg, st, vd);
        if (batch || data_on == 3) continue;
        const float* f = cfg.data_loss == IRS_DATA_GMM_LCC ? c->fhat + (c->fhat_chains == 1 ? 0 : (int64_t)ch * vol.V) : nullptr;
        hipStream_t ds = st;
        if (overlap && ch + 1 < C) {
            HIP_TRY(hipEventRecord(c->ev_side[2 * ch], st));
            HIP_TRY(hipStreamWaitEvent(c->side, c->ev_side[2 * ch], 0));
            ds = c->side;
        }
        launch_data_bwd(cfg.data_loss, f, 0, zc, c->sigM + (int64_t)ch * vol.V, mask, 0, nullptr, c->state, ch,
                        c->gM + (int64_t)ch * vol.V, c->nll_partials + (int64_t)ch * c->nll_blocks, cfg.lcc_s, 1, vol, ds, c->nll_seg_C);
        if (ds != st) HIP_TRY(hipEventRecord(c->ev_side[2 * ch + 1], c->side));
    }
    if (data_on == 3)
        launch_lcc_data_bwd_plan(c->fhat, c->fhat_chains == 1 ? 0 : vol.V, z, c->sigM, io->mask, io->mask_chains == 1 ? 0 : vol.V, c->state, c->gM,
                                 cfg.lcc_s, C, vol, c->dplan, st);
    else if (batch)
        launch_data_bwd(cfg.data_loss, c->fhat, c->fhat_chains == 1 ? 0 : vol.V, z, c->sigM, io->mask, io->mask_chains == 1 ? 0 : vol.V, nullptr,
                        c->state, 0, c->gM, c->nll_partials, cfg.lcc_s, C, vol, st, c->nll_seg_C);
    if (!fuse_warp_bwd)
        launch_warp_bwd(io->moving_im, io->moving_chains == 1 ? 0 : vol.V, d_last, io->unif,
                        cfg.uniform_alpha > 0.0f ? cfg.uniform_alpha : 0.0f, c->gM, c->gA, C, vol, lin, cfg.seed, 0, it, st);
    const bool sparse = c->sparse_adjoint && c->plan.entries != nullptr &&
                        (global_knobs().march_seg > 0 || exp_bwd_dense_seg_len(vol, C) > kPlanMinLen);
    c->plan_on = sparse;
    if (sparse) launch_adjoint_plan(c->gM, c->dmax, c->plan, cfg.no_steps, C, vol, exp_bwd_plan_resident(), global_knobs().march_seg, st);
    LAUNCH_CHECK();
    if (timed) HIP_TRY(hipEventRecord(c->ev[3], st));
    const float* dense = c->ffd ? c->dense : vs;
    float* g0 = nullptr;
    {
        const float* G = c->gA;
        float* bufs[2] = {c->gB, c->gA};
        int cur = 0;
        for (int k = cfg.no_steps - 1; k >= 0; --k) {
            float* out = bufs[cur];
            const float* dk = k == 0 ? dense : c->steps + (int64_t)(k - 1) * field;
            if (timed) HIP_TRY(hipEventRecord(c->ev_bwd[2 * k], st));
            const unsigned* dm = c->dmax + (int64_t)k * C * 4;
            const float* gscale = fuse_warp_bwd && k == cfg.no_steps - 1 ? c->gM : nullptr;
            const int lay = bwd_lay(c, k) | (gscale ? 2 : 0);
            const bool sa = k < 32 && skip_any[k], s2 = k < 32 && skip_r2[k];
            const int gr = global_knobs().lds_from <= 2 ? 1 : 2;
            launch_exp_step_bwd_march(G, dk, out, k == 0, cfg.no_steps, C, vol, lin, dm, (s2 || (gr == 1 && !sa)) ? 1 : 2, sa, gscale, lay,
                                      timed ? c->ev_bwd[2 * k + 1] : nullptr, st, sparse ? &c->plan : nullptr, k);
            if (!sa) launch_exp_step_bwd_lds(G, dk, out, k == 0, cfg.no_steps, C, vol, lin, dm, 2, gr, gscale, lay, c->cmm, st);
            G = out;
            cur ^= 1;
        }
        g0 = const_cast<float*>(G);
    }
    if (timed) HIP_TRY(hipEventRecord(c->ev[4], st));
    float s[3];
    prescale_factors(vol, cfg.no_steps, s);
    if (c->ffd) {
        float* scaled = g0 == c->gA ? c->gB : c->gA;
        launch_scale_channels(g0, scaled, s[0], s[1], s[2], C, vol, st);
        const int G[3] = {volv.D, volv.H, volv.W};
        ffd_adjoint(scaled, c->tmpB, c->tmpA, C, vol, G, c->spl, st);
        launch_sgld_update(io->v, io->sigma, c->tmpB, vs, c->state, cfg.lr, 1.0f, 1.0f, 1.0f, io->grad_v, C, volv, st,
                           energy_in_update ? c->energy_partials : nullptr, energy_in_update);
    } else {
        launch_sgld_update(io->v, io->sigma, g0, vs, c->state, cfg.lr, s[0], s[1], s[2], io->grad_v, C, volv, st,
                           energy_in_update ? c->energy_partials : nullptr, energy_in_update);
    }
    launch_finalize(c->state, data_on == 3 ? c->dplan.nll : c->nll_partials, c->nll_blocks, c->dcfg, true, c->dmax, c->hint,
                    4 * C * (cfg.no_steps + 1), vd, kHintWords - 7, true, st, energy_in_update ? c->energy_partials : nullptr, upd_blocks,
                    data_on == 3 ? c->dplan.entries : nullptr, data_on == 3 ? c->dplan.count : nullptr);
    c->dmax_clean = true;
    LAUNCH_CHECK();
    if (timed) HIP_TRY(hipEventRecord(c->ev[5], st));
    if (is_capturing(st)) return 0;
    HIP_TRY(hipEventRecord(c->ra_ev[c->n_enqueued % 4], st));
    ++c->n_enqueued;
    return 0;
}

static void poll_failures(irs_ctx* c) {
    if (!c->hint) return;
    const unsigned f = ((volatile unsigned*)c->hint)[kHintWords - 7];
    if (f == c->fails_seen || (int)(f - c->fails_seen) < 0) return;
    c->makeup += (uint64_t)(f - c->fails_seen);
    c->fails_total += (uint64_t)(f - c->fails_seen);
    c->fails_seen = f;
    c->force_all_until = c->n_enqueued + c->makeup + 3;
}

static void drop_pending(irs_ctx* c) {
    poll_failures(c);
    c->makeup = 0;
}

static int transition_impl(irs_ctx* c, const irs_io* io, hipStream_t st, int timed) {
    if (check_io(c, io, "irs_transition")) return 1;
    if (!io->v) return fail("irs_transition: v is required");
    if (is_capturing(st)) {
        if (timed) return fail("irs_transition_timed: the stream is being captured -- per-stage timings need a stream that executes");
        c->last_io = *io;
        c->have_last_io = true;
        return enqueue_transition(c, io, st, 0, true);
    }
    const int depth = c->kn.run_ahead;
    if (depth > 0 && depth <= 3 && c->n_enqueued >= (uint64_t)depth) HIP_TRY(hipEventSynchronize(c->ra_ev[(c->n_enqueued - depth) % 4]));
    poll_failures(c);
    if (c->makeup && !c->kn.recover)
        return fail("irs_transition: an earlier transition skipped a kernel variant its displacement then needed and was dropped "
                    "(recover = 0); predict_variants = 0 launches every variant");
    while (c->makeup > 0) {
        --c->makeup;
        if (enqueue_transition(c, io, st, 0, true)) return 1;
    }
    c->last_io = *io;
    c->have_last_io = true;
    return enqueue_transition(c, io, st, timed, c->n_enqueued < c->force_all_until);
}

static int flush_impl(irs_ctx* c, hipStream_t st) {
    for (int guard = 0; guard < 8; ++guard) {
        HIP_TRY(hipStreamSynchronize(st));
        if (c->n_enqueued) HIP_TRY(hipEventSynchronize(c->ra_ev[(c->n_enqueued - 1) % 4]));
        poll_failures(c);
        if (!c->makeup) return 0;
        if (!c->kn.recover || !c->have_last_io) return fail("irs_flush: %llu transition(s) were dropped after a failed variant prediction", (unsigned long long)c->makeup);
        while (c->makeup > 0) {
            --c->makeup;
            if (enqueue_transition(c, &c->last_io, st, 0, true)) return 1;
        }
    }
    return fail("irs_flush: transitions keep failing");
}

int irs_flush(irs_ctx* c, void* stream) {
    if (!c) return fail("irs_flush: null argument");
    if (c->sl.on) return irs::slab_flush(c, (hipStream_t)stream);
    return flush_impl(c, (hipStream_t)stream);
}

int irs_recovered_transitions(const irs_ctx* c, uint64_t* out) {
    if (!c || !out) return fail("irs_recovered_transitions: null argument");
    *out = c->fails_total;
    return 0;
}

int irs_sparse_adjoint_set(irs_ctx* c, int on) {
    if (!c) return fail("irs_sparse_adjoint_set: null argument");
    c->sparse_adjoint = on != 0;
    return 0;
}

int irs_sparse_adjoint_get(irs_ctx* c, int32_t* out, void* stream) {
    if (!c || !out) return fail("irs_sparse_adjoint_get: null argument");
    const size_t n = (size_t)c->cfg.no_steps * c->C * kPlanStats;
    memset(out, 0, n * sizeof(int32_t));
    if (!c->plan.stats || !c->plan_on || c->n_enqueued == 0) return 0;
    if (irs_flush(c, stream)) return 1;
    HIP_TRY(hipMemcpyAsync(out, c->plan.stats, n * sizeof(int32_t), hipMemcpyDeviceToHost, (hipStream_t)stream));
    HIP_TRY(hipStreamSynchronize((hipStream_t)stream));
    return 0;
}

int irs_sparse_data_set(irs_ctx* c, int on) {
    if (!c) return fail("irs_sparse_data_set: null argument");
    if (on < 0) return fail("irs_sparse_data_set: 0 (off), 1 (on) or a piece length");
    c->sparse_data = on;
    return 0;
}

int irs_sparse_data_get(irs_ctx* c, int32_t* out, void* stream) {
    if (!c || !out) return fail("irs_sparse_data_get: null argument");
    const int C = c->C;
    memset(out, 0, (size_t)kDataKernels * C * kPlanStats * sizeof(int32_t));
    if (!c->dplan.entries || c->data_on == 0 || c->n_enqueued == 0) return 0;
    if (irs_flush(c, stream)) return 1;
    const size_t tiles = (size_t)c->dplan.wtx * c->dplan.wty;
    int* hull = (int*)malloc(sizeof(int) * 2 * tiles * C);
    int32_t lists[2 * IRS_MAX_CHAINS * kPlanStats];
    if (!hull) return fail("irs_sparse_data_get: out of host memory");
    hipError_t e = hipMemcpyAsync(hull, c->dplan.hull, sizeof(int) * 2 * tiles * C, hipMemcpyDeviceToHost, (hipStream_t)stream);
    if (e == hipSuccess) e = hipMemcpyAsync(lists, c->dplan.stats, sizeof(int32_t) * 2 * C * kPlanStats, hipMemcpyDeviceToHost, (hipStream_t)stream);
    if (e == hipSuccess) e = hipStreamSynchronize((hipStream_t)stream);
    if (e != hipSuccess) {
        free(hull);
        return fail("irs_sparse_data_get: read-back failed: %s", hipGetErrorString(e));
    }
    for (int ch = 0; ch < C; ++ch) {
        int32_t planes = 0;
        for (size_t t = 0; t < tiles; ++t) planes += hull[(ch * tiles + t) * 2 + 1] - hull[(ch * tiles + t) * 2];
        out[(size_t)ch * kPlanStats] = 1;
        out[(size_t)ch * kPlanStats + 3] = planes;
        if (c->data_on >= 2) memcpy(out + ((size_t)1 * C + ch) * kPlanStats, lists + ((size_t)C + ch) * kPlanStats, sizeof(int32_t) * kPlanStats);
        if (c->data_on >= 3) memcpy(out + ((size_t)3 * C + ch) * kPlanStats, lists + (size_t)ch * kPlanStats, sizeof(int32_t) * kPlanStats);
    }
    free(hull);
    return 0;
}

int irs_transition(irs_ctx* c, const irs_io* io, void* stream) { return transition_impl(c, io, (hipStream_t)stream, 0); }

int irs_transition_timed(irs_ctx* c, const irs_io* io, void* stream, irs_timings* out) {
    if (!out) return fail("irs_transition_timed: null output");
    if (c && c->cfg.no_steps > 32) return fail("irs_transition_timed: at most 32 steps");
    if (transition_impl(c, io, (hipStream_t)stream, 1)) return 1;
    HIP_TRY(hipEventSynchronize(c->ev[5]));
    memset(out, 0, sizeof(*out));
    HIP_TRY(hipEventElapsedTime(&out->total_ms, c->ev[0], c->ev[5]));
    HIP_TRY(hipEventElapsedTime(&out->smooth_ms, c->ev[0], c->ev[1]));
    HIP_TRY(hipEventElapsedTime(&out->exp_fwd_ms, c->ev[1], c->ev[2]));
    HIP_TRY(hipEventElapsedTime(&out->data_ms, c->ev[2], c->ev[3]));
    HIP_TRY(hipEventElapsedTime(&out->exp_bwd_total_ms, c->ev[3], c->ev[4]));
    HIP_TRY(hipEventElapsedTime(&out->update_ms, c->ev[4], c->ev[5]));
    for (int k = 0; k < c->cfg.no_steps; ++k) {
        float ms = 0.0f;
        HIP_TRY(hipEventElapsedTime(&ms, c->ev_bwd[2 * k], c->ev_bwd[2 * k + 1]));
        out->exp_bwd_kernel_ms += ms;
        if (k >= 1) out->exp_bwd_primary_avg_ms += ms / (float)(c->cfg.no_steps > 1 ? c->cfg.no_steps - 1 : 1);
    }
    return 0;
}

}
```

### ir_sgmcmc_amd/csrc/ctx.h

```cpp
#pragma once
#include <stdlib.h>
#include <string.h>

#include "kernels.h"
#include "scalar_kernels.h"

struct irs_comm;

namespace irs {

int fail(const char* fmt, ...);

#define HIP_TRY(expr)                                                                               \
    do {                                                                                            \
        hipError_t e_ = (expr);                                                                     \
        if (e_ != hipSuccess) return irs::fail("%s failed: %s", #expr, hipGetErrorString(e_));      \
    } while (0)

#define LAUNCH_CHECK()                                                                              \
    do {                                                                                            \
        hipError_t e_ = hipGetLastError();                                                          \
        if (e_ != hipSuccess) return irs::fail("kernel launch failed: %s", hipGetErrorString(e_)); \
    } while (0)


struct SlabInfo {
    bool on = false;
    int rank = 0, world = 1;
    int a = 0, b = 0;
    int lo = 0, hi = 0;
    int margin = 0;
    int gmax = 8;
    int min_slab = 0;
    bool has_lo = false, has_hi = false;
};

}

struct irs_ctx {
    irs_config cfg;
    irs::DevCfg dcfg;
    irs::Vol vol, volv;
    bool ffd;
    int C;
    irs::LinTables lin;
    irs::Taps sob;
    irs::SplineTaps spl[3];
    char* slab;
    size_t slab_bytes;
    float *steps, *tmpA, *tmpB, *vs, *gA, *gB, *gC, *warped, *z, *sigM, *fhat, *gM, *dense;
    double *stat_partials, *energy_partials, *nll_partials;
    double *stat_sum, *energy_sum, *nll_sum;
    unsigned* dmax;
    irs::AdjointPlan plan;
    bool sparse_adjoint = true;
    bool plan_on = false;
    irs::DataPlan dplan;
    int sparse_data = 1;
    int data_on = 0;
    float* cmm;
    unsigned* hint = nullptr;
    irs::DevState* state;
    int fhat_chains;
    bool fixed_set;
    int nll_blocks;
    int nll_seg_C;
    hipEvent_t ev[8];
    hipEvent_t ev_bwd[64];
    hipEvent_t ra_ev[4];
    hipStream_t side = nullptr;
    hipEvent_t ev_side[2 * IRS_MAX_CHAINS] = {};
    uint64_t n_enqueued = 0;
    irs::Knobs kn;
    bool dmax_clean = false;
    unsigned fails_seen = 0;
    uint64_t makeup = 0;
    uint64_t fails_total = 0;
    uint64_t force_all_until = 0;
    uint64_t exact_until = 0;
    float hint_seen[32] = {}, hint_before[32] = {};
    bool hint_trend[32] = {};
    irs_io last_io;
    bool have_last_io = false;
    irs::SlabInfo sl;
    irs_comm* comm = nullptr;
    hipStream_t cs = nullptr;
    hipEvent_t sev[28];
    unsigned* plan_hint = nullptr;
    double* hsum = nullptr;
    int pred[32];
    bool have_pred = false;
    uint64_t slab_exchanged_bytes = 0;
    uint64_t slab_exchanges = 0;
    uint64_t slab_exact = 0;
    uint64_t slab_mispredictions = 0;
    int last_nf = 0, last_nb = 0;
    struct TlRec {
        int32_t kind, stage, k, width;
        int eP, eR, eW0, eW1;
    };
    int tl_arm = 0;
    hipEvent_t* tl_ev = nullptr;
    int tl_ev_n = 0, tl_ev_used = 0;
    TlRec tl_rec[128];
    int tl_n = 0, tl_t0 = -1, tl_t1 = -1;
    bool tl_have = false;
};

namespace irs {

constexpr int kHintWords = 4 * IRS_MAX_CHAINS * 32 + 8;

inline float hint_row_max(const unsigned* row, int n, bool* valid) {
    const volatile unsigned* h = row;
    float m = 0.0f;
    *valid = true;
    for (int i = 0; i < n; ++i) {
        const unsigned bits = h[i];
        float f;
        memcpy(&f, &bits, sizeof(f));
        if (!(f >= 0.0f)) *valid = false;
        m = f > m ? f : m;
    }
    return m;
}

inline bool predicted_below(const irs_ctx* c, int k, float bound) {
    const int mode = c->kn.predict_variants;
    if (mode == 2 || mode == 3) return true;
    if (!mode || !c->hint) return false;
    bool valid;
    const float m = hint_row_max(c->hint + (size_t)k * c->C * 4, c->C * 4, &valid);
    return valid && m < bound;
}
inline bool bound_is_steady(const irs_ctx* c, int k) {
    if (k >= 32 || !c->hint_trend[k]) return false;
    const float a = c->hint_before[k], b = c->hint_seen[k];
    return a > 0.0f && b < 1.1f * a;
}
inline bool predicted_small(const irs_ctx* c, int k) {
    if (predicted_below(c, k, 0.9f)) return true;
    return c->kn.predict_variants == 1 && bound_is_steady(c, k) && predicted_below(c, k, 0.97f);
}
inline bool predicted_tiny(const irs_ctx* c, int k) {
    if (c->kn.predict_variants == 3) return true;
    if (c->kn.predict_variants != 1) return false;
    if (predicted_below(c, k, 0.4f)) return true;
    return bound_is_steady(c, k) && predicted_below(c, k, 0.66f);
}
inline void note_hint_trend(irs_ctx* c) {
    if (!c->hint) return;
    for (int k = 0; k < c->cfg.no_steps && k < 32; ++k) {
        bool valid;
        const float m = hint_row_max(c->hint + (size_t)k * c->C * 4, c->C * 4, &valid);
        if (!valid || m > 1.0e6f) {
            c->hint_trend[k] = false;
            c->hint_seen[k] = 0.0f;
            continue;
        }
        if (m != c->hint_seen[k]) {
            c->hint_trend[k] = c->hint_seen[k] > 0.0f;
            c->hint_before[k] = c->hint_seen[k];
            c->hint_seen[k] = m;
        }
    }
}

inline int fwd_lay(const irs_ctx* c, int k) { return (k > 0 ? 1 : 0) | (k < c->cfg.no_steps - 1 ? 4 : 0); }
inline int bwd_lay(const irs_ctx* c, int k) {
    return (k > 0 ? 1 : 0) | (k < c->cfg.no_steps - 1 ? 2 : 0) | (k > 0 ? 4 : 0);
}

inline void prescale_factors(Vol vol, int no_steps, float s[3]) {
    const double p = 1.0 / (double)(1 << no_steps);
    s[0] = (float)(2.0 / (double)(vol.W - 1) * p);
    s[1] = (float)(2.0 / (double)(vol.H - 1) * p);
    s[2] = (float)(2.0 / (double)(vol.D - 1) * p);
}

int create_ctx(const irs_config* cfg, const SlabInfo* sl, irs_ctx** out);
int check_io(const irs_ctx* c, const irs_io* io, const char* who);
void context_born();
void context_gone();
void slab_release(irs_ctx* c);
int slab_flush(irs_ctx* c, hipStream_t st);
void slab_drop_pending(irs_ctx* c);
int ffd_up(const float* v_cp, float* dense, float* tmp, int C, Vol vol, const int G[3], const SplineTaps spl[3], hipStream_t st,
           int w_lo = 0, int w_n = -1, int store_lo = 0, int store_n = -1);
int ffd_adjoint(const float* g_dense, float* g_cp, float* tmp, int C, Vol vol, const int G[3], const SplineTaps spl[3], hipStream_t st,
                int w_lo = 0, int w_n = -1, int store_lo = 0, int store_n = -1);

}
```

### ir_sgmcmc_amd/csrc/exp_kernels.hip

```cpp
#include "adjoint_plan.h"
#include "kernels.h"

#include <type_traits>

namespace irs {

#ifndef IRS_ETX
#define IRS_ETX 32
#define IRS_ETY 8
#define IRS_ETZ 8
#endif
constexpr int ETX = IRS_ETX, ETY = IRS_ETY, ETZ = IRS_ETZ, ETN = ETX * ETY * ETZ;
constexpr int kExpBlock = 512;

struct Scale3L {
    float nm1[3];
    float rnm1[3];
    float inv_pow;
};

typedef float F3 __attribute__((ext_vector_type(3)));
__device__ __forceinline__ F3 ld3g(const float* __restrict__ p) {
    F3 v;
    __builtin_memcpy(&v, p, 12);
// ... 1042 lines not shown
#endif
        }
    }
    };
    run();
}

template <bool PRESCALE, int R>
__global__ __launch_bounds__(kMarchBlock, R == 1 ? IRS_MARCH_WAVES : IRS_MARCH_WAVES_R2) void exp_bwd_march_kernel(
    const float* __restrict__ G, const float* __restrict__ dk, float* __restrict__ gout, Vol vol, Lin lin, Scale3L sc,
    const unsigned* __restrict__ dmax, int seg_len, int nseg, int r_lo, int own_rest, int swz_run, dim3 tiles,
    const float* __restrict__ gscale, int lay) {
    const int total = (int)(tiles.x * tiles.y * tiles.z);
    for (int id = blockIdx.x; id < total; id += gridDim.x)
        exp_bwd_march_tile<PRESCALE, R>(G, dk, gout, vol, lin, sc, dmax, seg_len, nseg, r_lo, own_rest, swz_run, id, tiles, gscale, lay);
}


constexpr int kPlanFillBlocks = 256;
__device__ __forceinline__ void plan_zero_fill(float* __restrict__ o, const Lay3 LO, const Vol vol, const int ox, const int oy, int za, int zb) {
    za = max(za, 0);
    zb = min(zb, vol.D);
    const int lx = threadIdx.x % MTX, ly = threadIdx.x / MTX;
    const int x = ox + lx, y = oy + ly;
    if (!(x < vol.W && y < vol.H)) return;
    const unsigned g = (unsigned)(y * vol.W + x) * 4u * (unsigned)LO.em;
    for (int z = za; z < zb; ++z) {
        const int64_t pl = (int64_t)z * vol.H * vol.W * LO.em;
        if (LO.em == 3) {
            st3_off(o + pl, g, 0.0f, 0.0f, 0.0f);
        } else {
            st_off(o + pl, g, 0.0f);
            st_off(o + LO.cs + pl, g, 0.0f);
            st_off(o + 2 * LO.cs + pl, g, 0.0f);
        }
    }
}
template <bool PRESCALE>
__global__ __launch_bounds__(kMarchBlock, IRS_MARCH_WAVES) void exp_bwd_march_plan_kernel(
    const float* __restrict__ G, const float* __restrict__ dk, float* __restrict__ gout, Vol vol, Lin lin, Scale3L sc,
    const unsigned* __restrict__ dmax, const PlanEntry* __restrict__ entries, const int* __restrict__ count, int swz_run, dim3 tiles,
    const float* __restrict__ gscale, int lay) {
    const int n = count[0], n_run = count[1];
    if (blockIdx.x < kPlanFillBlocks) {
        for (int id = n_run + (int)blockIdx.x; id < n; id += kPlanFillBlocks) {
            const PlanEntry e = entries[id];
            plan_zero_fill(gout + (int64_t)e.chain * 3 * vol.V, lay3(lay & 4, vol.V), vol, (e.tile % (int)tiles.x) * MTX,
                           (e.tile / (int)tiles.x) * MTY, e.z0, e.z1);
        }
        return;
    }
    const int first = (int)blockIdx.x - kPlanFillBlocks, stride = (int)gridDim.x - kPlanFillBlocks;
    for (int id = first; id < n_run; id += stride)
        exp_bwd_march_tile<PRESCALE, 1, true>(G, dk, gout, vol, lin, sc, dmax, 0, 1, 0, 0, 0, id, tiles, gscale, lay,
                                              entries[plan_swizzle(id, n_run, swz_run)]);
}
int64_t exp_bwd_plan_resident() {
    static int cache = 0;
    return resident_blocks((const void*)exp_bwd_march_plan_kernel<false>, kMarchBlock, &cache);
}

constexpr int kRareGrid = 256 * IRS_MARCH_WAVES_R2;


int exp_bwd_dense_seg_len(Vol vol, int C) {
    const int seg_env = global_knobs().march_seg;
    const int64_t per_layer = (int64_t)((vol.W + MTX - 1) / MTX) * ((vol.H + MTY - 1) / MTY) * C;
    int seg_len = pick_seg_len(vol.nz + vol.nzb, per_layer, 8, seg_env);
    if (global_knobs().seg_fit && seg_env <= 0) {
        static int cache = 0;
        const int64_t res = resident_blocks((const void*)exp_bwd_march_kernel<false, 1>, kMarchBlock, &cache);
        if (res > 0) seg_len = pick_seg_len_fit(vol.nz, vol.nzb, per_layer, 8, 2, res, 0, IRS_BWD_MAX_SEG);
    }
    return seg_len;
}

void launch_exp_step_bwd_march(const float* G, const float* dk, float* gout, bool prescale_in, int no_steps, int C, Vol vol,
                               Lin lin, const unsigned* dmax, int max_radius, bool r2_owns_rest, const float* gscale, int lay,
                               hipEvent_t after_primary, hipStream_t st, const AdjointPlan* plan, int step) {
    const int seg_env = global_knobs().march_seg;
    const int64_t per_layer = (int64_t)((vol.W + MTX - 1) / MTX) * ((vol.H + MTY - 1) / MTY) * C;
    const int seg_len = exp_bwd_dense_seg_len(vol, C);
    const int nseg = vol_nseg(vol, seg_len);
    const dim3 tiles((vol.W + MTX - 1) / MTX, (vol.H + MTY - 1) / MTY, (unsigned)(nseg * C));
    const int total = (int)(tiles.x * tiles.y * tiles.z);
    const Scale3L sc = make_scale_l(vol, no_steps);
    const int swz_env = global_knobs().swz_run;
    const int swz_run = swz_env >= 0 ? swz_env : (int)tiles.x;
    if (global_knobs().launch_log) {
        static int cache_l = 0;
        log_launch("exp_bwd_march_kernel<R=1>", MTX, MTY, total, kMarchBlock, seg_len, 2, vol.nz + vol.nzb, C,
                   resident_blocks((const void*)exp_bwd_march_kernel<false, 1>, kMarchBlock, &cache_l));
    }
    auto launch = [&](auto P, auto RR, int r_lo, int grid, int seg, int nseg_, dim3 tiles_, int total_) {
        hipLaunchKernelGGL((exp_bwd_march_kernel<decltype(P)::value, decltype(RR)::value>), dim3(grid), dim3(kMarchBlock), 0, st, G, dk, gout, vol,
                           lin, sc, dmax, seg, nseg_, r_lo, r2_owns_rest ? 1 : 0, grid == total_ ? swz_run : 0, tiles_, gscale, lay);
    };
    if (plan && vol.nzb == 0 && vol.z0 == 0 && vol.nz == vol.D) {
        const int64_t res = exp_bwd_plan_resident();
        const dim3 tiles2d(tiles.x, tiles.y, 1);
        with_bool(prescale_in, [&](auto P) {
            hipLaunchKernelGGL((exp_bwd_march_plan_kernel<decltype(P)::value>), dim3((unsigned)((res > 0 ? res : kExpGridCap) + kPlanFillBlocks)), dim3(kMarchBlock), 0,
                               st, G, dk, gout, vol, lin, sc, dmax, plan->entries + (int64_t)step * plan->cap, plan->count + 2 * step, swz_run, tiles2d,
                               gscale, lay);
        });
    } else {
        with_bool(prescale_in, [&](auto P) { launch(P, Int<1>{}, 0, total, seg_len, nseg, tiles, total); });
    }
    if (after_primary) (void)hipEventRecord(after_primary, st);
    if (max_radius >= 2) {
        int seg2 = seg_len;
        if (global_knobs().seg_fit && seg_env <= 0)
            seg2 = pick_seg_len_fit(vol.nz, vol.nzb, per_layer, 8, 4, kRareGrid, 0, IRS_BWD_MAX_SEG);
        const int nseg2 = vol_nseg(vol, seg2);
        const dim3 tiles2(tiles.x, tiles.y, (unsigned)(nseg2 * C));
        const int total2 = (int)(tiles2.x * tiles2.y * tiles2.z);
        const int rare = total2 < kRareGrid ? total2 : kRareGrid;
        with_bool(prescale_in, [&](auto P) { launch(P, Int<2>{}, 1, rare, seg2, nseg2, tiles2, total2); });
    }
}

#ifndef IRS_FTX
#define IRS_FTX 64
#define IRS_FTY 8
#define IRS_FROWS 2
#endif
#ifndef IRS_FWD_PITCH_ALIGN
#define IRS_FWD_PITCH_ALIGN 16
#endif
#ifndef IRS_FWD_WAVES
#define IRS_FWD_WAVES 4
#endif
constexpr int FTX = IRS_FTX, FTY = IRS_FTY, FROWS_BIG = IRS_FROWS;
template <int R, int FROWS = FROWS_BIG>
struct MarchF {
    static constexpr int kFwdBlock = FTX * FTY / FROWS;
    static constexpr int NP = 2 * R + 1, PX = FTX + 2 * R, PY = FTY + 2 * R, PN = PX * PY;
    static constexpr int NIT = (PN + kFwdBlock - 1) / kFwdBlock;
    static constexpr int PITCH = (IRS_FWD_PITCH_ALIGN > 1 && R == 1) ? (PX + IRS_FWD_PITCH_ALIGN - 1) / IRS_FWD_PITCH_ALIGN * IRS_FWD_PITCH_ALIGN : PX;
    static constexpr int PNP = PITCH * PY;
};
#ifdef IRS_FWD_TRACE
__device__ unsigned long long g_fwd_trace[8 * 64];
extern "C" __attribute__((visibility("default"))) int irs_debug_fwd_trace(unsigned long long* out) {
    return hipMemcpyFromSymbol(out, HIP_SYMBOL(g_fwd_trace), sizeof(g_fwd_trace)) == hipSuccess ? 0 : 1;
}
#define IRS_TR(slot)                                                                           \
    do {                                                                                       \
        if (trace_on && trace_it < 64) g_fwd_trace[trace_it * 8 + (slot)] = clock64();         \
    } while (0)
#else
#define IRS_TR(slot)
#endif
template <bool PRESCALE, int R, int FROWS, int PF>
__device__ __forceinline__ void exp_fwd_march_tile(const float* __restrict__ din, float* __restrict__ dout, const Vol vol,
                                                   const Lin lin, const Scale3L sc, const unsigned* __restrict__ dmax_in,
                                                   unsigned* __restrict__ dmax_out, const int seg_len, const int nseg,
                                                   const int h_lo, const int h_hi, const int swz_run, const int tile_id,
                                                   const dim3 tiles, const int lay) {
    using M = MarchF<R, FROWS>;
    constexpr int PX = M::PX, PN = M::PN, NIT = M::NIT, PITCH = M::PITCH, PNP = M::PNP, kFwdBlock = M::kFwdBlock;
    constexpr int NS = M::NP + 1;
    __shared__ float2 r_xy[NS * PNP];
    __shared__ float r_z[NS * PNP];
    __shared__ float red[3 * (kFwdBlock / kWave)];
    const int tile_ = xcd_swizzle_runs(tile_id, (int)(tiles.x * tiles.y * tiles.z), swz_run);
    const int tbx = tile_ % tiles.x, tby = (tile_ / tiles.x) % tiles.y, tbz = tile_ / (tiles.x * tiles.y);
    const int chain = tbz / nseg, seg = tbz % nseg;
    if (dmax_in) {
        const int need = max(max((int)ceilf(__uint_as_float(dmax_in[chain * 4 + 0])), (int)ceilf(__uint_as_float(dmax_in[chain * 4 + 1]))),
                             (int)ceilf(__uint_as_float(dmax_in[chain * 4 + 2])));
        if (need <= h_lo || need > h_hi) return;
    }
    const int ox = tbx * FTX, oy = tby * FTY;
    int z0, z1;
    seg_range(vol, seg, seg_len, z0, z1);
    const int64_t V = vol.V;
    const int64_t cb = (int64_t)chain * 3 * V;
    auto run = [&](auto LC) {
    constexpr int LAYC = decltype(LC)::value;
    const Lay3 LD = lay3(LAYC & 1, V), LO = lay3(LAYC & 4, V);
    const float* __restrict__ dx_ = din + cb;
    const float* __restrict__ dy_ = dx_ + LD.cs;
    const float* __restrict__ dz_ = dy_ + LD.cs;
    float* __restrict__ o = dout + cb;
    const int lx = threadIdx.x % FTX, ly0 = threadIdx.x / FTX;
    const int x = ox + lx;
    const float linx = x < vol.W ? lin.x[x] : 0.0f;

    int sxy[NIT], sld[NIT];
#pragma unroll
    for (int it = 0; it < NIT; ++it) {
        const int i = threadIdx.x + it * kFwdBlock;
        const int px = i % PX, py = i / PX;
        const int cx = min(max(ox - R + px, 0), vol.W - 1), cy = min(max(oy - R + py, 0), vol.H - 1);
        sxy[it] = i < PN ? cy * vol.W + cx : -1;
        sld[it] = py * PITCH + px;
    }
    float pre[PF][NIT][3];
    auto prefetch = [&](int s, float (&pre)[NIT][3]) {
        const int sc_ = min(max(s, 0), vol.D - 1);
        const int64_t zo = (int64_t)sc_ * vol.H * vol.W * LD.em;
        const float* __restrict__ px_ = dx_ + zo;
        const float* __restrict__ py_ = dy_ + zo;
        const float* __restrict__ pz_ = dz_ + zo;
#pragma unroll
        for (int it = 0; it < NIT; ++it) {
            if (sxy[it] < 0) continue;
            const unsigned g = (unsigned)sxy[it] * 4u * (unsigned)LD.em;
            if (LD.em == 3) {
                const F3 v = ld3_off(px_, g);
                pre[it][0] = v.x;
                pre[it][1] = v.y;
                pre[it][2] = v.z;
            } else {
                pre[it][0] = ld_off(px_, g);
                pre[it][1] = ld_off(py_, g);
                pre[it][2] = ld_off(pz_, g);
            }
        }
    };
    auto commit = [&](int slot, const float (&pre)[NIT][3]) {
#pragma unroll
        for (int it = 0; it < NIT; ++it) {
            if (sxy[it] < 0) continue;
            const int i = slot * PNP + sld[it];
            r_xy[i] = make_float2(PRESCALE ? prescale(pre[it][0], sc.nm1[0], sc.rnm1[0], sc.inv_pow) : pre[it][0],
                                  PRESCALE ? prescale(pre[it][1], sc.nm1[1], sc.rnm1[1], sc.inv_pow) : pre[it][1]);
            r_z[i] = PRESCALE ? prescale(pre[it][2], sc.nm1[2], sc.rnm1[2], sc.inv_pow) : pre[it][2];
        }
    };

    float m0 = 0.0f, m1 = 0.0f, m2 = 0.0f;
    const int sbase = z0 - R, slast = z1 - 1 + R;
    float liny_[FROWS];
#pragma unroll
    for (int j = 0; j < FROWS; ++j) liny_[j] = lin.y[min(oy + ly0 + j * (FTY / FROWS), vol.H - 1)];
    float linz_nx = lin.z[min(max(sbase - R, 0), vol.D - 1)];
#ifdef IRS_FWD_TRACE
    const bool trace_on = R == 1 && !PRESCALE && tile_id == (int)(tiles.x * tiles.y * tiles.z) / 2 + 3 && threadIdx.x == 64;
    int trace_it = 0;
    if (trace_on) {
        g_fwd_trace[63 * 8 + 0] = clock64();
        g_fwd_trace[63 * 8 + 1] = wall_clock64();
        g_fwd_trace[63 * 8 + 4] = (unsigned long long)(slast - sbase + 1);
    }
#endif
    static_assert(NS % PF == 0, "the buffer of plane s is (s - sbase) % PF == PH % PF");
    prefetch(sbase, pre[0]);
    if (PF > 1) prefetch(sbase + 1, pre[PF - 1]);
    for (int sb = sbase; sb <= slast; sb += NS) {
#pragma unroll
        for (int PH = 0; PH < NS; ++PH) {
            const int s = sb + PH;
            if (s > slast) break;
#ifdef IRS_FWD_TRACE
            IRS_TR(0);
            __builtin_amdgcn_s_waitcnt(0);
            IRS_TR(1);
#endif
            if (PF == 1) __builtin_amdgcn_s_waitcnt(0x0F70);
            commit(PH, pre[PH % PF]);
            IRS_TR(2);
            const float linz = linz_nx;
            linz_nx = lin.z[min(max(s + 1 - R, 0), vol.D - 1)];
            if (s + PF <= slast) prefetch(s + PF, pre[PH % PF]);
            IRS_TR(3);
            __syncthreads();
            IRS_TR(4);
            const int zo = s - R;
            if (zo >= z0 && zo < z1) {
#pragma unroll
                for (int j = 0; j < FROWS; ++j) {
                const int ly = ly0 + j * (FTY / FROWS), y = oy + ly;
                if (x >= vol.W || y >= vol.H) continue;
                const float liny = liny_[j];
                const int a = (PH - R + NS) % NS;
                const int ci = a * PNP + (ly + R) * PITCH + (lx + R);
                const float2 dxy = r_xy[ci];
                const float d0 = dxy.x, d1 = dxy.y, d2 = r_z[ci];
                const AxisTap tx = axis_tap(__fadd_rn(linx, d0), vol.W);
                const AxisTap ty = axis_tap(__fadd_rn(liny, d1), vol.H);
                const AxisTap tz = axis_tap(__fadd_rn(linz, d2), vol.D);
                const int bx0 = tx.i0 - (ox - R), by0 = ty.i0 - (oy - R), rel = tz.i0 - zo;
                const bool in_ring = (unsigned)bx0 < (unsigned)(PX - 1) && (unsigned)by0 < (unsigned)(M::PY - 1) && rel >= -R && rel < R;
                float a0 = 0.0f, a1 = 0.0f, a2 = 0.0f;
                auto ring_taps = [&]() {
                    const float wxy[2][2] = {{__fmul_rn(tx.w0, ty.w0), __fmul_rn(tx.w1, ty.w0)},
                                             {__fmul_rn(tx.w0, ty.w1), __fmul_rn(tx.w1, ty.w1)}};
                    int sl0 = ((a - R + NS) % NS) * PNP, sl1 = ((a - R + 1 + NS) % NS) * PNP;
#pragma unroll
                    for (int q = -R + 1; q < R; ++q) {
                        sl0 = rel == q ? ((a + q + NS) % NS) * PNP : sl0;
                        sl1 = rel == q ? ((a + q + 1 + NS) % NS) * PNP : sl1;
                    }
                    const int off = by0 * PITCH + bx0;
#pragma unroll
                    for (int cz = 0; cz < 2; ++cz) {
                        const int bs = (cz ? sl1 : sl0) + off;
#pragma unroll
                        for (int cy = 0; cy < 2; ++cy)
#pragma unroll
                            for (int cx = 0; cx < 2; ++cx) {
                                const float w = __fmul_rn(wxy[cy][cx], cz ? tz.w1 : tz.w0);
                                typedef float VF2 __attribute__((ext_vector_type(2)));
                                const VF2 tv = *(const volatile __attribute__((address_space(3))) VF2*)(&r_xy[bs + cy * PITCH + cx]);
                                const float t1 = *(const volatile __attribute__((address_space(3))) float*)(&r_z[bs + cy * PITCH + cx]);
                                a0 = fmaf(tv.x, w, a0);
                                a1 = fmaf(tv.y, w, a1);
                                a2 = fmaf(t1, w, a2);
                            }
                    }
                };
                if (__all(in_ring)) {
                    ring_taps();
                } else if (in_ring) {
                    ring_taps();
                } else {
#pragma unroll
                    for (int cz = 0; cz < 2; ++cz)
#pragma unroll
                        for (int cy = 0; cy < 2; ++cy)
#pragma unroll
                            for (int cx = 0; cx < 2; ++cx) {
                                const float w = __fmul_rn(__fmul_rn(cx ? tx.w1 : tx.w0, cy ? ty.w1 : ty.w0), cz ? tz.w1 : tz.w0);
                                const int64_t idx = (((int64_t)(cz ? tz.i1 : tz.i0) * vol.H + (cy ? ty.i1 : ty.i0)) * vol.W + (cx ? tx.i1 : tx.i0)) * LD.em;
                                a0 = fmaf(ldp<PRESCALE>(dx_, idx, sc.nm1[0], sc.rnm1[0], sc.inv_pow), w, a0);
                                a1 = fmaf(ldp<PRESCALE>(dy_, idx, sc.nm1[1], sc.rnm1[1], sc.inv_pow), w, a1);
                                a2 = fmaf(ldp<PRESCALE>(dz_, idx, sc.nm1[2], sc.rnm1[2], sc.inv_pow), w, a2);
                            }
                }
                const int64_t pl = (int64_t)zo * vol.H * vol.W * LO.em;
                const unsigned g = (unsigned)(y * vol.W + x) * 4u * (unsigned)LO.em;
                const float r0 = __fadd_rn(d0, a0), r1 = __fadd_rn(d1, a1), r2 = __fadd_rn(d2, a2);
                if (LO.em == 3) {
                    st3_off(o + pl, g, r0, r1, r2);
                } else {
                    st_off(o + pl, g, r0);
                    st_off(o + LO.cs + pl, g, r1);
                    st_off(o + 2 * LO.cs + pl, g, r2);
                }
                m0 = fmaxf(m0, fabsf(r0));
                m1 = fmaxf(m1, fabsf(r1));
                m2 = fmaxf(m2, fabsf(r2));
                }
            }
#ifdef IRS_FWD_TRACE
            IRS_TR(5);
            ++trace_it;
#endif
        }
    }
#ifdef IRS_FWD_TRACE
    if (trace_on) {
        g_fwd_trace[63 * 8 + 2] = clock64();
        g_fwd_trace[63 * 8 + 3] = wall_clock64();
    }
#endif
    if (dmax_out) {
        m0 *= 0.5f * sc.nm1[0];
        m1 *= 0.5f * sc.nm1[1];
        m2 *= 0.5f * sc.nm1[2];
#pragma unroll
        for (int off = kWave / 2; off > 0; off >>= 1) {
            m0 = fmaxf(m0, __shfl_down(m0, off, kWave));
            m1 = fmaxf(m1, __shfl_down(m1, off, kWave));
            m2 = fmaxf(m2, __shfl_down(m2, off, kWave));
        }
        const int wid = threadIdx.x / kWave;
        if ((threadIdx.x & (kWave - 1)) == 0) {
            red[wid] = m0;
            red[(kFwdBlock / kWave) + wid] = m1;
            red[2 * (kFwdBlock / kWave) + wid] = m2;
        }
        __syncthreads();
        if (threadIdx.x < 3) {
            float m = 0.0f;
#pragma unroll
            for (int w = 0; w < kFwdBlock / kWave; ++w) m = fmaxf(m, red[threadIdx.x * (kFwdBlock / kWave) + w]);
            unsigned* slot = dmax_out + chain * 4 + threadIdx.x;
            if (__float_as_uint(m) > __hip_atomic_load(slot, __ATOMIC_RELAXED, __HIP_MEMORY_SCOPE_AGENT)) atomic_max_nonneg(slot, m);
        }
    }
    };
    switch (lay & 5) {
        case 0: run(Int<0>{}); break;
        case 1: run(Int<1>{}); break;
        case 4: run(Int<4>{}); break;
        default: run(Int<5>{}); break;
    }
}

#ifndef IRS_FWD_SMALL_TILES
#define IRS_FWD_SMALL_TILES 1024
#endif
template <bool PRESCALE, int R, int FROWS = FROWS_BIG, int PF = 1>
__global__ __launch_bounds__(FTX * FTY / FROWS, R == 1 ? IRS_FWD_WAVES : 1) void exp_fwd_march_kernel(const float* __restrict__ din, float* __restrict__ dout,
                                                                  Vol vol, Lin lin, Scale3L sc,
                                                                  const unsigned* __restrict__ dmax_in,
                                                                  unsigned* __restrict__ dmax_out, int seg_len, int nseg,
                                                                  int h_lo, int h_hi, int swz_run, dim3 tiles, int lay) {
    const int total = (int)(tiles.x * tiles.y * tiles.z);
    for (int id = blockIdx.x; id < total; id += gridDim.x) {
        exp_fwd_march_tile<PRESCALE, R, FROWS, PF>(din, dout, vol, lin, sc, dmax_in, dmax_out, seg_len, nseg, h_lo, h_hi, swz_run, id, tiles, lay);
        __syncthreads();
    }
}

void launch_exp_step_fwd_march(const float* din, float* dout, bool prescale_in, int no_steps, int C, Vol vol, Lin lin,
                               const unsigned* dmax_in, unsigned* dmax_out, bool only_r1, int lay, hipStream_t st) {
    const int seg_env = global_knobs().march_seg_fwd;
    const int64_t per_layer = (int64_t)((vol.W + FTX - 1) / FTX) * ((vol.H + FTY - 1) / FTY) * C;
    int seg_len = pick_seg_len(vol.nz + vol.nzb, per_layer, 8, seg_env);
    const int small_env = global_knobs().fwd_rows1;
    const bool small = FROWS_BIG != 1 && (small_env >= 0 ? small_env != 0 : seg_len <= 8 && per_layer * vol_nseg(vol, seg_len) <= IRS_FWD_SMALL_TILES);
    if (global_knobs().seg_fit && seg_env <= 0) {
        static int cache_big = 0, cache_small = 0;
        const int64_t res = small ? resident_blocks((const void*)exp_fwd_march_kernel<false, 1, 1, 2>, FTX * FTY, &cache_small)
                                  : resident_blocks((const void*)exp_fwd_march_kernel<false, 1, FROWS_BIG, 1>, FTX * FTY / FROWS_BIG, &cache_big);
        if (res > 0) seg_len = pick_seg_len_fit(vol.nz, vol.nzb, per_layer, 8, 2, res, 0);
    }
    const int nseg = vol_nseg(vol, seg_len);
    const dim3 tiles((vol.W + FTX - 1) / FTX, (vol.H + FTY - 1) / FTY, (unsigned)(nseg * C));
    const int total = (int)(tiles.x * tiles.y * tiles.z);
    const Scale3L sc = make_scale_l(vol, no_steps);
    const int swz_env = global_knobs().swz_run;
    const int swz_run = swz_env >= 0 ? swz_env : (int)tiles.x;
    if (global_knobs().launch_log) {
        static int cache_ls = 0, cache_lb = 0;
        log_launch(small ? "exp_fwd_march_kernel<R=1,rows=1>" : "exp_fwd_march_kernel<R=1,rows=2>", FTX, FTY, total, small ? FTX * FTY : FTX * FTY / FROWS_BIG,
                   seg_len, 2, vol.nz + vol.nzb, C,
                   small ? resident_blocks((const void*)exp_fwd_march_kernel<false, 1, 1, 2>, FTX * FTY, &cache_ls)
                         : resident_blocks((const void*)exp_fwd_march_kernel<false, 1, FROWS_BIG, 1>, FTX * FTY / FROWS_BIG, &cache_lb));
    }
    const bool r2_rows1 = global_knobs().fwd_r2_rows1 != 0;
    int seg2 = seg_len;
    int64_t res2 = kRareGrid;
    if (global_knobs().seg_fit && seg_env <= 0) {
        static int cache_r2a = 0, cache_r2b = 0;
        const int64_t r = r2_rows1 ? resident_blocks((const void*)exp_fwd_march_kernel<false, 2, 1>, FTX * FTY, &cache_r2a)
                                   : resident_blocks((const void*)exp_fwd_march_kernel<false, 2>, FTX * FTY / FROWS_BIG, &cache_r2b);
        if (r > 0) {
            res2 = r;
            seg2 = pick_seg_len_fit(vol.nz, vol.nzb, per_layer, 8, 4, res2, 0, 64);
        }
    }
    const int nseg2 = vol_nseg(vol, seg2);
    const dim3 tiles2(tiles.x, tiles.y, (unsigned)(nseg2 * C));
    const int total2 = (int)(tiles2.x * tiles2.y * tiles2.z);
    const int rare = total2 < res2 ? total2 : (int)res2;
    auto launch = [&](auto P, auto RR, auto ROWS, auto PF, int h_lo, int h_hi, int grid, int seg, int nseg_, dim3 tiles_, int total_) {
        constexpr int kRows = decltype(ROWS)::value;
        hipLaunchKernelGGL((exp_fwd_march_kernel<decltype(P)::value, decltype(RR)::value, kRows, decltype(PF)::value>), dim3(grid),
                           dim3(FTX * FTY / kRows), 0, st, din, dout, vol, lin, sc, dmax_in, dmax_out, seg, nseg_, h_lo, h_hi,
                           grid == total_ ? swz_run : 0, tiles_, lay);
    };
    const bool r1_only = !dmax_in || only_r1;
    with_bool(prescale_in, [&](auto P) {
        auto r1 = [&](auto ROWS, auto PF) { launch(P, Int<1>{}, ROWS, PF, -1, r1_only ? 1 << 30 : 1, total, seg_len, nseg, tiles, total); };
        if (!small) r1(Int<FROWS_BIG>{}, Int<1>{});
        else if (global_knobs().fwd_pf >= 2) r1(Int<1>{}, Int<2>{});
        else r1(Int<1>{}, Int<1>{});
        if (r1_only) return;
        auto r2 = [&](auto ROWS) { launch(P, Int<2>{}, ROWS, Int<1>{}, 1, 1 << 30, rare, seg2, nseg2, tiles2, total2); };
        if (r2_rows1) r2(Int<1>{}); else r2(Int<FROWS_BIG>{});
    });
}

template <bool PRESCALE>
__global__ __launch_bounds__(kBlock) void field_absmax_kernel(const float* __restrict__ d, unsigned* __restrict__ dmax,
                                                              Vol vol, Scale3L sc) {
    __shared__ float red[3 * (kBlock / kWave)];
    const int chain = blockIdx.y;
    const float* c0 = d + (int64_t)chain * 3 * vol.V;
    float m[3] = {0.0f, 0.0f, 0.0f};
    IRS_ROWS_BEGIN(vol, x, y, z, v)
        (void)x; (void)y; (void)z;
#pragma unroll
        for (int c = 0; c < 3; ++c) m[c] = fmaxf(m[c], fabsf(ldp<PRESCALE>(c0 + c * vol.V, v, sc.nm1[c], sc.rnm1[c], sc.inv_pow)));
    IRS_ROWS_END
#pragma unroll
    for (int c = 0; c < 3; ++c) {
        m[c] *= 0.5f * sc.nm1[c];
#pragma unroll
        for (int off = kWave / 2; off > 0; off >>= 1) m[c] = fmaxf(m[c], __shfl_down(m[c], off, kWave));
        if ((threadIdx.x & (kWave - 1)) == 0) red[c * (kBlock / kWave) + threadIdx.x / kWave] = m[c];
    }
    __syncthreads();
    if (threadIdx.x < 3) {
        float mm = 0.0f;
#pragma unroll
        for (int w = 0; w < kBlock / kWave; ++w) mm = fmaxf(mm, red[threadIdx.x * (kBlock / kWave) + w]);
        unsigned* slot = dmax + chain * 4 + threadIdx.x;
        if (__float_as_uint(mm) > __hip_atomic_load(slot, __ATOMIC_RELAXED, __HIP_MEMORY_SCOPE_AGENT)) atomic_max_nonneg(slot, mm);
    }
}

void launch_field_absmax(const float* d, bool prescale_in, int no_steps, unsigned* dmax, int C, Vol vol, hipStream_t st) {
    const int rows = vol.H * vol.nz;
    dim3 grid((unsigned)(rows / 4 < 2048 ? (rows + 3) / 4 : 2048), C);
    const Scale3L sc = make_scale_l(vol, no_steps);
    if (prescale_in) hipLaunchKernelGGL(field_absmax_kernel<true>, grid, dim3(kBlock), 0, st, d, dmax, vol, sc);
    else hipLaunchKernelGGL(field_absmax_kernel<false>, grid, dim3(kBlock), 0, st, d, dmax, vol, sc);
}

}
```

### ir_sgmcmc_amd/csrc/kernels.h

```cpp
#pragma once
#include "common.h"

namespace irs {

struct Taps {
    float k[2 * IRS_MAX_HALF_WIDTH + 1];
    int s;
};

struct SplineTaps {
    float k[32];
    int cps;
};

struct LinTables {
    float* dev = nullptr;
    int D = 0, H = 0, W = 0;
    Lin lin() const { return Lin{dev, dev + W, dev + W + H}; }
};
int ensure_lin_tables(LinTables& t, int D, int H, int W, hipStream_t st);
int cached_lin(int D, int H, int W, hipStream_t st, Lin* out);

void launch_perturb(const float* v, const float* sigma, const float* eps, float amp, float* out, int C, Vol vol,
                    uint64_t seed, uint64_t iteration, const uint64_t* dev_iteration, hipStream_t st);
void launch_svf_outputs(const float* d, float* transformation, float* displacement, int C, Vol vol, Lin lin,
                        hipStream_t st);
void launch_warp_fwd(const float* im, int64_t im_stride, const float* d, const float* unif, float alpha, float* out,
                     float* gradm, int gradm_aos, int C, Vol vol, Lin lin, uint64_t seed, uint64_t iteration,
                     const uint64_t* dev_iteration, hipStream_t st, const int* hull = nullptr);
void launch_warp_bwd(const float* im, int64_t im_stride, const float* d, const float* unif, float alpha,
                     const float* g_warped, float* g_d, int C, Vol vol, Lin lin, uint64_t seed, uint64_t iteration,
                     const uint64_t* dev_iteration, hipStream_t st);
void launch_warp_transformation(const float* im, int64_t im_stride, const float* t, float* out, int C, Vol vol,
                                hipStream_t st);
void launch_warp_nearest_u8(const uint8_t* im, int64_t im_stride, const float* t, uint8_t* out, int C, Vol vol,
                            hipStream_t st);
void launch_warp_nearest_i16(const int16_t* im, int64_t im_stride, const float* t, int16_t* out, int C, Vol vol,
                             hipStream_t st);
void launch_ffd_axis(const float* in, float* out, const SplineTaps& taps, bool adjoint, int64_t outer, int n_in,
                     int n_out, int64_t inner, hipStream_t st, int w_lo = 0, int w_n = -1, int store_lo = 0, int store_n = -1);
void launch_scale_channels(const float* in, float* out, float s0, float s1, float s2, int C, Vol vol, hipStream_t st);

void launch_exp_step_fwd_march(const float* din, float* dout, bool prescale, int no_steps, int C, Vol vol, Lin lin,
                               const unsigned* dmax_in, unsigned* dmax_out, bool only_r1, int lay, hipStream_t st);
struct AdjointPlan;
void launch_exp_step_bwd_march(const float* G, const float* dk, float* gout, bool prescale, int no_steps, int C, Vol vol,
                               Lin lin, const unsigned* dmax, int max_radius, bool r2_owns_rest, const float* gscale, int lay,
                               hipEvent_t after_primary, hipStream_t st, const AdjointPlan* plan = nullptr, int step = 0);
int exp_bwd_dense_seg_len(Vol vol, int C);
int64_t exp_bwd_plan_resident();
size_t coarse_minmax_bytes(Vol vol, int C);
void launch_exp_step_bwd_lds(const float* G, const float* dk, float* gout, bool prescale, int no_steps, int C, Vol vol,
                             Lin lin, const unsigned* dmax, int halo, int gather_radius, const float* gscale, int lay,
                             float* cmm, hipStream_t st);
void launch_field_absmax(const float* d, bool prescale, int no_steps, unsigned* dmax, int C, Vol vol, hipStream_t st);

struct PlanEntry;
struct ColPlan;
struct AdjointPlan {
    int* ext = nullptr;
    int* runs = nullptr;
    ColPlan* colplan = nullptr;
    PlanEntry* entries = nullptr;
    int* count = nullptr;
    int* stats = nullptr;
    int cap = 0, ntx = 0, nty = 0;
};
size_t adjoint_plan_bytes(Vol vol, int C, int no_steps);
AdjointPlan adjoint_plan_views(char* base, Vol vol, int C, int no_steps);
void launch_adjoint_plan(const float* g_warped, const unsigned* dmax, const AdjointPlan& plan, int no_steps, int C, Vol vol,
                         int64_t G, int forced_len, hipStream_t st);
struct DataPlan {
    int* ext = nullptr;
    int* runs = nullptr;
    int* hull = nullptr;
    ColPlan* colplan = nullptr;
    PlanEntry* entries = nullptr;
    int* count = nullptr;
    int* stats = nullptr;
    double* nll = nullptr;
    int cap = 0, ntx = 0, nty = 0, wtx = 0, wty = 0;
    int forced_len = 0;
};
size_t data_plan_bytes(Vol vol, int C);
DataPlan data_plan_views(char* base, Vol vol, int C);
void launch_data_plan(const uint8_t* mask, int mask_chains, const DataPlan& plan, int s, bool lists, int C, Vol vol, hipStream_t st);
int data_plan_run_bound(const DataPlan& plan, int s, bool bwd, int C, Vol vol);

void launch_sobolev_march(const float* in, float* out, const Taps& taps, int planes, Vol vol, unsigned* dmax0, int no_steps,
                          hipStream_t st);
void launch_perturb_sobolev_march(const float* v, const float* sigma, const float* eps, float amp, float* out, const Taps& taps,
                                  int C, Vol vol, unsigned* dmax0, int no_steps, uint64_t seed, uint64_t iteration,
                                  const uint64_t* dev_iteration, hipStream_t st);
void launch_lcc_fwd_march(const float* fhat, int64_t fhat_stride, const float* im, float* z, float* sigma_out, int s, int C,
                    Vol vol, hipStream_t st);
void launch_lcc_fwd_plan(const float* fhat, int64_t fhat_stride, const float* im, float* z, float* sigma_out, int s, int C, Vol vol,
                         const DataPlan& plan, hipStream_t st);
int64_t lcc_plan_resident(int s, bool bwd, bool batch);
int lcc_dense_seg_len(Vol vol, int C, bool bwd);
struct GmmDev;
void launch_data_bwd(int mode, const float* fhat_or_fixed, int64_t f_stride, const float* z, const float* sigma_m,
                     const uint8_t* mask, int64_t mask_stride, const float* g_z_override, const void* dev_state,
                     int chain, float* g_warped, double* nll_partials, int s, int C_launch, Vol vol, hipStream_t st, int seg_C = 1);
void launch_stats(int want_vd, const float* z, const uint8_t* mask, const void* dev_state, double* partials, Vol vol,
                  hipStream_t st, int K = 0);
void launch_residual_ssd(const float* fixed, int64_t f_stride, const float* warped, float* z, int C, Vol vol,
                         hipStream_t st);
int lcc_data_bwd_march_blocks(Vol vol, int seg_C = 1);
void launch_lcc_data_bwd_march(const float* fhat, const float* z, const float* sigma_m, const uint8_t* mask,
                               const float* g_z_override, const void* dev_state, int chain, float* g_warped,
                               double* nll_partials, int s, Vol vol, hipStream_t st, int batch = 0, int64_t f_stride = 0,
                               int64_t m_stride = 0, int seg_C = 1);
void launch_lcc_data_bwd_plan(const float* fhat, int64_t f_stride, const float* z, const float* sigma_m, const uint8_t* mask,
                              int64_t m_stride, const void* dev_state, float* g_warped, int s, int C, Vol vol, const DataPlan& plan,
                              hipStream_t st);
int data_bwd_blocks(int mode, Vol vol, int seg_C = 1);
void launch_masked_moments(const float* z, const uint8_t* mask, double* partials, Vol vol, hipStream_t st);
void launch_reg_energy(const float* v, double* partials, int C, Vol vol, hipStream_t st);
void launch_reduce_partials(const double* partials, int nblocks, int nvals, double* out, hipStream_t st);
void launch_reduce_cols(const double* partials, int nblocks, int ncols, double* out, hipStream_t st);
void launch_sgld_update(float* v, const float* sigma, const float* g_d0, const float* v_s, const void* dev_state,
                        float lr, float s0, float s1, float s2, float* grad_out, int C, Vol vol, hipStream_t st,
                        double* energy_partials = nullptr, bool coef_from_w = false);
int sgld_update_blocks_per_chain(Vol vol, int C);
void launch_gradient_operator(const float* v, float* nabla, int transformation, int C, Vol vol, hipStream_t st);
void launch_log_det_jacobian(const float* t, float* log_det, long long* nan_count, int C, Vol vol, hipStream_t st);
void launch_stats_march(int want_vd, const float* z, const uint8_t* mask, const void* dev_state, double* partials, int blocks,
                        Vol vol, int K, hipStream_t st);
void launch_reg_energy_march(const float* v, double* partials, int blocks, int C, Vol vol, hipStream_t st);
void launch_sgld_update_march(float* v, const float* sigma, const float* g_d0, const float* v_s, const void* dev_state,
                              float lr, float s0, float s1, float s2, float* grad_out, int C, Vol vol, hipStream_t st,
                              double* energy_partials = nullptr, bool coef_from_w = false);
int stats_blocks(Vol vol);
int energy_blocks(Vol vol);

struct SurfLabels {
    int32_t v[IRS_MAX_LABELS];
};
struct SurfPair {
    int32_t z0, y0, x0, nz, ny, nx;
    int64_t vox;
    int64_t tw, th, td;
};
constexpr int kSurfLdsLine = 64;
void launch_surface_boxes(const int16_t* fixed, int64_t f_stride, const int16_t* moving, const SurfLabels& lab, int L,
                          int32_t* boxes, int C, Vol vol, hipStream_t st);
struct SurfPassArgs {
    const SurfPair* plan;
    int P;
    int64_t tasks[3];
    int line[3];
    int lanes;
    float* env_scratch[3];
    int env_slots[3];
    uint8_t* memb;
    float* gA;
    float* gB;
    double* partials;
    uint32_t* maxpart;
};
void launch_surface_distance(const int16_t* fixed, int64_t f_stride, const int16_t* moving, const SurfLabels& lab, int L,
                             const float spacing[3], const SurfPassArgs& a, long long* counts, double* sums, Vol vol,
                             hipStream_t st);

struct HdArgs {
    const SurfPair* plan;
    int P, Q, slices;
    double pct[IRS_HAUSDORFF_MAX_PERCENTILES];
    const uint8_t* memb;
    const float* gA;
    const float* gB;
    const long long* counts;
    const uint32_t* maxpart;
    uint32_t* hist;
    uint32_t* prefix;
    long long* rank;
    double* hd;
    double* hd_pct;
};
void launch_hausdorff_select(const HdArgs& a, hipStream_t st);

void launch_surface_posterior_update(const int16_t* fixed, const int16_t* moving, const SurfLabels& lab, int L, const SurfPair* plan,
                                     const float* gB, int C, float* mean, float* m2, int32_t* count, Vol vol, hipStream_t st);
struct SurfLevels {
    double z[IRS_SURFACE_MAX_LEVELS];
    int n;
};
void launch_surface_posterior_finalize(const int16_t* fixed, const SurfLabels& lab, int L, const float* mean, const float* m2,
                                       const int32_t* count, const uint8_t* mask, const SurfLevels& lv, float* bias, float* std,
                                       long long* isummary, double* fsummary, void* ws, Vol vol, hipStream_t st);

void launch_chain_moments(const float* x, float* mean, float* m2, int64_t n, int k, hipStream_t st);
int split_rhat_blocks(int64_t V);
void launch_split_rhat(const float* mean, const float* m2, int C, int n, const uint8_t* mask, float thr0, float thr1, float* rhat,
                       double* summary, double* partials, int64_t V, hipStream_t st);
void launch_chain_variogram(const float* x, float* ring, float* vsum, int C, int64_t E, int L, int k, hipStream_t st);
void launch_split_ess(const float* mean, const float* m2, const float* vsum, int C, int n, int L, const uint8_t* mask, float thr,
                      float* ess, float* mcse, double* summary, double* partials, int64_t V, hipStream_t st);

int label_update_partials_blocks(int64_t V);
void launch_label_update(const int16_t* seg, int C, int64_t V, const SurfLabels& lab, int K, int32_t* counts, double* volume,
                         int records_before, int32_t* partials, hipStream_t st);
int label_finalize_blocks(int64_t V);
void launch_label_finalize(const int32_t* counts, int K, int64_t V, int n, const SurfLabels& lab, const int16_t* seg_fixed,
                           const uint8_t* mask, float* entropy, int16_t* map_label, long long* summary, double* mask_summary,
                           long long* partials, double* dpartials, hipStream_t st);

void launch_jacobian_update(const float* t, int C, int32_t* folds, float* mean, float* m2, int records_before, Vol vol,
                            hipStream_t st);
void launch_jacobian_finalize(const int32_t* folds, const float* mean, const float* m2, int64_t V, int n, const uint8_t* mask,
                              float* fold_prob, float* logj_mean, float* logj_std, long long* isummary, double* fsummary,
                              void* ws, hipStream_t st);

void launch_covariance_update(const float* x, int C, float* mean, float* comoment, int records_before, Vol vol, hipStream_t st);
void launch_covariance_finalize(const float* mean, const float* comoment, int64_t V, int n, const float* scale, const uint8_t* mask,
                                float* stdev, float* direction, float* anisotropy, long long* isummary, double* fsummary, void* ws,
                                hipStream_t st);

constexpr int kImagePosteriorGroup = 2;
void launch_image_posterior_update(const float* volumes, int S, const float* t, int C, float* mean, float* m2, float* low,
                                   float* high, int records_before, Vol vol, hipStream_t st);
void launch_image_posterior_finalize(const float* mean, const float* m2, const float* low, const float* high, int64_t V, int n,
                                     const float* reference, float std_floor, const uint8_t* mask, float* std_out, float* range_out,
                                     float* z_out, long long* isummary, double* fsummary, void* ws, hipStream_t st);
// ... 117 lines not shown
```

### ir_sgmcmc_amd/csrc/slab.hip

```cpp
#include <math.h>
#include <stdio.h>
#include <new>
#include <vector>

#include "api_checks.h"
#include "comm.h"

using namespace irs;

namespace {

constexpr int kMaxSteps = 32;
constexpr int kDefaultGhostMax = 8;

struct Plan {
    int n = 0;
    int h[kMaxSteps];
    float m[kMaxSteps];
    int fr[kMaxSteps], fw[kMaxSteps], nf;
    int br[kMaxSteps], bw[kMaxSteps], nb;
};

int plan_rounds(Plan& p, int gmax, int min_slab, int nbuf = 2) {
    const int n = p.n;
// ... 472 lines not shown
        hipEvent_t prod = c->sev[16 + 2 * slot], fin = c->sev[17 + 2 * slot];
        HIP_TRY(hipEventRecord(prod, st));
        tl_open(o.id, IRS_OP_ALLREDUCE, o.stage, -1, 0, stamp(st));
        HIP_TRY(hipStreamWaitEvent(cs, prod, 0));
        if (comm_allreduce(c->comm, buf, count, mx, cs)) return 1;
        HIP_TRY(hipEventRecord(fin, cs));
        if (tl) c->tl_rec[o.id].eR = stamp(cs);
        pending[o.id] = fin;
        return 0;
    }
    int launch(const irs_slab_op& o) {
        const irs_config& cfg = c->cfg;
        const Views v = views(c);
        const int n = cfg.no_steps, C = chains;
        const Vol w = o.hi1 > o.lo1 ? window2(c->vol, o.lo0, o.hi0, o.lo1, o.hi1) : window(c->vol, o.lo0, o.hi0);
        const Lin lin = c->lin.lin();
        const uint64_t* it = &c->state->st.iteration;
        float* noisy = c->ffd ? c->tmpA : planar(c->tmpA, v);
        const Vol wv = c->ffd ? c->volv : w;
        const float* d0 = c->ffd ? planar(c->dense, v) : vs;
        const int64_t HW = (int64_t)c->vol.H * c->vol.W;
        switch (o.stage) {
            case IRS_SG_PERTURB:
                launch_perturb(v_src, io.sigma, io.eps, (float)sqrt(2.0 * (double)cfg.lr), cfg.sobolev_s > 0 ? noisy : vs, C, wv, cfg.seed, 0, it, st);
                break;
            case IRS_SG_COPY_V: {
                float* first = cfg.sobolev_s > 0 ? noisy : vs;
                if (c->ffd) {
                    HIP_TRY(hipMemcpyAsync(first, v_src, (size_t)C * 3 * c->volv.V * sizeof(float), hipMemcpyDeviceToDevice, st));
                    break;
                }
                for (int ch = 0; ch < 3 * C; ++ch)
                    HIP_TRY(hipMemcpyAsync(first + (int64_t)ch * c->vol.V + (int64_t)w.z0 * HW, v_src + (int64_t)ch * c->vol.V + (int64_t)w.z0 * HW,
                                           (size_t)w.nz * HW * sizeof(float), hipMemcpyDeviceToDevice, st));
                break;
            }
            case IRS_SG_SMOOTH:
                if (o.k == 1)
                    launch_perturb_sobolev_march(v_src, io.sigma, io.eps, (float)sqrt(2.0 * (double)cfg.lr), vs, c->sob, C, w, c->dmax, n, cfg.seed, 0, it, st);
                else if (cfg.sobolev_s > 0) launch_sobolev_march(noisy, vs, c->sob, C * 3, wv, c->ffd ? nullptr : c->dmax, n, st);
                else if (!c->ffd) launch_field_absmax(vs, true, n, c->dmax, C, w, st);
                break;
            case IRS_SG_ENERGY:
                launch_reg_energy(vs, c->energy_partials, C, wv, st);
                launch_reduce_partials(c->energy_partials, energy_blocks(wv), C, c->energy_sum, st);
                break;
            case IRS_SG_FFD_UP: {
                const int G[3] = {c->volv.D, c->volv.H, c->volv.W};
                ffd_up(vs, c->dense, c->tmpA, C, c->vol, G, c->spl, st, w.z0, w.nz, c->sl.lo, c->sl.hi - c->sl.lo);
                launch_field_absmax(d0, true, n, c->dmax, C, w, st);
                break;
            }
            case IRS_SG_FFD_ADJ: {
                float sc3[3];
                prescale_factors(c->vol, n, sc3);
                float* g0 = grad_raw(c, 0, false);
                float* scaled = g0 == c->gA ? c->gB : c->gA;
                launch_scale_channels(planar(g0, v), planar(scaled, v), sc3[0], sc3[1], sc3[2], C, w, st);
                const int G[3] = {c->volv.D, c->volv.H, c->volv.W};
                ffd_adjoint(scaled, c->tmpB, c->tmpA, C, c->vol, G, c->spl, st, w.z0, w.nz, c->sl.lo, c->sl.hi - c->sl.lo);
                break;
            }
            case IRS_SG_EXP_FWD: {
                const int k = o.k;
                const float* in = k == 0 ? d0 : step_buf(c, v, k - 1);
                launch_exp_step_fwd_march(in, step_buf(c, v, k), k == 0, n, C, w, lin, c->dmax + (int64_t)k * c->C * 4,
                                          c->dmax + (int64_t)(k + 1) * c->C * 4, predicted_small(c, k), fwd_lay(c, k), st);
                break;
            }
            case IRS_SG_OUTPUTS:
                launch_svf_outputs(step_buf(c, v, n - 1), io.transformation, io.displacement, C, w, lin, st);
                break;
            case IRS_SG_WARP:
                launch_warp_fwd(io.moving_im, io.moving_chains == 1 ? 0 : c->vol.Vg, step_buf(c, v, n - 1), io.unif,
                                jitter && cfg.uniform_alpha > 0.0f ? cfg.uniform_alpha : 0.0f, warped, nullptr, 0, C, w, lin, cfg.seed, 0, it, st);
                break;
            case IRS_SG_RESIDUAL:
                if (cfg.data_loss == IRS_DATA_GMM_LCC)
                    launch_lcc_fwd_march(planar(c->fhat, v), c->fhat_chains == 1 ? 0 : c->vol.V, warped, z, planar(c->sigM, v), cfg.lcc_s, C, w, st);
                else launch_residual_ssd(io.fixed_im, io.fixed_chains == 1 ? 0 : c->vol.V, warped, z, C, w, st);
                break;
            case IRS_SG_STATS: {
                const uint8_t* mask = io.mask + (io.mask_chains == 1 ? 0 : (int64_t)o.k * c->vol.V);
                launch_stats(stats_vd, z + (int64_t)o.k * c->vol.V, mask, c->state, c->stat_partials, w, st, c->dcfg.K);
                launch_reduce_partials(c->stat_partials, stats_blocks(w), kStatVals, c->stat_sum, st);
                break;
            }
            case IRS_SG_CHAIN_SCALAR:
                launch_chain_scalar(c->state, c->stat_sum, 1, o.k, stats_op | (o.k == 0 && in_transition ? 4 : 0), c->dcfg, st, in_transition ? verdict_always() : no_verdict());
                break;
            case IRS_SG_VERDICT:
                launch_chain_scalar(c->state, c->stat_sum, 1, 0, 4, c->dcfg, st, verdict_always());
                break;
            case IRS_SG_DATA_BWD: {
                const int ch = o.k;
                const uint8_t* mask = io.mask + (io.mask_chains == 1 ? 0 : (int64_t)ch * c->vol.V);
                const float* f = cfg.data_loss == IRS_DATA_GMM_LCC ? planar(c->fhat, v) + (c->fhat_chains == 1 ? 0 : (int64_t)ch * c->vol.V) : nullptr;
                double* part = c->nll_partials + (int64_t)ch * c->nll_blocks;
                launch_data_bwd(cfg.data_loss, f, 0, z + (int64_t)ch * c->vol.V, planar(c->sigM, v) + (int64_t)ch * c->vol.V, mask, 0, nullptr, c->state, ch,
                                planar(c->gM, v) + (int64_t)ch * c->vol.V, part, cfg.lcc_s, 1, w, st);
                launch_reduce_partials(part, data_bwd_blocks(cfg.data_loss, w), 1, c->nll_sum + ch, st);
                break;
            }
            case IRS_SG_WARP_BWD:
                launch_warp_bwd(io.moving_im, io.moving_chains == 1 ? 0 : c->vol.Vg, step_buf(c, v, n - 1), io.unif,
                                cfg.uniform_alpha > 0.0f ? cfg.uniform_alpha : 0.0f, planar(c->gM, v), planar(c->gA, v), C, w, lin, cfg.seed, 0, it, st);
                break;
            case IRS_SG_EXP_BWD: {
                const int k = o.k, hplan = plan ? plan->h[k] : 0;
                const int lay = bwd_lay(c, k);
                float* gi = grad_raw(c, k, true);
                float* go = grad_raw(c, k, false);
                const float* G = (lay & 2) ? aos(gi, v) : planar(gi, v);
                float* out = (lay & 4) ? aos(go, v) : planar(go, v);
                const float* dk = k == 0 ? d0 : step_buf(c, v, k - 1);
                const unsigned* dm = c->dmax + (int64_t)k * c->C * 4;
                const bool skip_any = hplan >= 1 && hplan <= 2;
                launch_exp_step_bwd_march(G, dk, out, k == 0, n, c->C, w, lin, dm, hplan == 1 ? 1 : 2, skip_any, nullptr, lay, nullptr, st);
                if (!skip_any) launch_exp_step_bwd_lds(G, dk, out, k == 0, n, c->C, w, lin, dm, 2, 2, nullptr, lay, nullptr, st);
                break;
            }
            case IRS_SG_REG_SCALAR:
                launch_reg_scalar(c->state, c->energy_sum, 1, c->dcfg, st, verdict_always());
                break;
            case IRS_SG_UPDATE: {
                float sc3[3];
                prescale_factors(c->vol, n, sc3);
                if (c->ffd) launch_sgld_update(io.v, io.sigma, c->tmpB, vs, c->state, cfg.lr, 1.0f, 1.0f, 1.0f, io.grad_v, C, wv, st);
                else launch_sgld_update(io.v, io.sigma, planar(grad_raw(c, 0, false), v), vs, c->state, cfg.lr, sc3[0], sc3[1], sc3[2], io.grad_v, C, w, st);
                break;
            }
            case IRS_SG_FINALIZE:
                launch_finalize(c->state, c->nll_sum, 1, c->dcfg, true, c->dmax, c->plan_hint + (c->n_enqueued % 2) * kHintWords,
                                4 * c->C * (n + 1), verdict_always(), kHintWords - 8, true, st);
                c->dmax_clean = true;
                break;
            default:
                return fail("slab: unknown stage %d", o.stage);
        }
        return 0;
    }
    int stats_vd = 0, stats_op = 3;
    bool in_transition = false;
    Verdict verdict_always() const {
        Verdict vd = verdict();
        if (!vd.bounds) {
            vd.bounds = c->dmax;
            vd.n = 0;
            vd.C = c->C;
        }
        return vd;
    }
};

int ghost_width_from_bound(float m, bool safety) {
    if (!(m >= 0.0f) || m > 1.0e6f) return -1;
    return (int)floorf(safety ? 1.25f * m + 0.25f : m) + 1;
}

float hint_bound(const irs_ctx* c, const unsigned* slot, int k) {
    bool valid;
    const float m = hint_row_max(slot + (size_t)k * c->C * 4, c->C * 4, &valid);
    return valid ? m : INFINITY;
}

int forward_exact(Exec& ex, Sched& sch, Plan& plan) {
    irs_ctx* c = ex.c;
    const int n = c->cfg.no_steps;
    plan.n = n;
    for (int k = 0; k < n; ++k) {
        size_t from = sch.ops.size();
        sch.wait(sch.allreduce(IRS_AR_DMAX));
        if (ex.run(sch.ops.data() + from, (int)(sch.ops.size() - from))) return 1;
        unsigned host[4 * IRS_MAX_CHAINS];
        HIP_TRY(hipMemcpyAsync(host, c->dmax + (int64_t)k * c->C * 4, sizeof(unsigned) * 4 * c->C, hipMemcpyDeviceToHost, ex.st));
        HIP_TRY(hipStreamSynchronize(ex.st));
        float m = 0.0f;
        for (int i = 0; i < 4 * c->C; ++i) {
            float f;
            memcpy(&f, &host[i], sizeof(f));
            if (!(f >= 0.0f)) return fail("slab: displacement bound of step %d is not finite", k);
            m = f > m ? f : m;
        }
        const int h = ghost_width_from_bound(m, false);
        if (h < 1) return fail("slab: displacement bound of step %d out of range", k);
        if (k == 0 && h > 1) return fail("slab: |d_0| >= 1 voxel: velocity field too large for %d squaring steps", n);
        plan.h[k] = h;
        plan.m[k] = m;
        plan.fr[k] = k;
        plan.fw[k] = h;
        plan.br[k] = n - 1 - k;
        plan.bw[n - 1 - k] = h;
        from = sch.ops.size();
        sch.forward_exact_step(k, h);
        if (ex.run(sch.ops.data() + from, (int)(sch.ops.size() - from))) return 1;
    }
    plan.nf = plan.nb = n;
    return 0;
}

irs_io shifted_io(const irs_ctx* c, const irs_io* io) {
    const Views v = views(c);
    irs_io o = *io;
    o.fixed_im = planar(io->fixed_im, v);
    o.mask = planar(io->mask, v);
    if (!c->ffd) {
        o.v = planar(io->v, v);
        o.sigma = planar(io->sigma, v);
        o.eps = planar(io->eps, v);
        o.curr_state = planar(io->curr_state, v);
        o.grad_v = planar(io->grad_v, v);
    }
    o.unif = planar(io->unif, v);
    o.im_moving_warped = planar(io->im_moving_warped, v);
    o.residuals = planar(io->residuals, v);
    o.displacement = planar(io->displacement, v);
    o.transformation = planar(io->transformation, v);
    return o;
}

}

namespace irs {
void slab_release(irs_ctx* c) {
    if (!c) return;
    for (int i = 0; i < 28; ++i)
        if (c->sev[i]) (void)hipEventDestroy(c->sev[i]);
    if (c->cs) (void)hipStreamDestroy(c->cs);
    if (c->plan_hint) (void)hipHostFree(c->plan_hint);
    for (int i = 0; i < c->tl_ev_n; ++i) (void)hipEventDestroy(c->tl_ev[i]);
    free(c->tl_ev);
    c->tl_ev = nullptr;
    c->tl_ev_n = 0;
}
}

extern "C" {

int irs_slab_plan_rounds(const int32_t* h, int n, int ghost_max, int min_slab, int n_buffers, int32_t* fwd_round, int32_t* fwd_width,
                         int32_t* n_fwd, int32_t* bwd_round, int32_t* bwd_width, int32_t* n_bwd) {
    if (!h || n < 1 || n > kMaxSteps || !fwd_round || !fwd_width || !n_fwd || !bwd_round || !bwd_width || !n_bwd)
        return fail("irs_slab_plan_rounds: bad arguments");
    Plan p;
    p.n = n;
    for (int k = 0; k < n; ++k) p.h[k] = h[k];
    if (plan_rounds(p, ghost_max > 0 ? ghost_max : kDefaultGhostMax, min_slab, n_buffers >= 3 ? 3 : 2)) return 1;
    for (int k = 0; k < n; ++k) {
        fwd_round[k] = p.fr[k];
        bwd_round[k] = p.br[k];
    }
    for (int r = 0; r < p.nf; ++r) fwd_width[r] = p.fw[r];
    for (int r = 0; r < p.nb; ++r) bwd_width[r] = p.bw[r];
    *n_fwd = p.nf;
    *n_bwd = p.nb;
    return 0;
}

int irs_slab_plan_layout(const irs_config* cfg, const irs_slab_config* scfg, int rank, int world, irs_slab_layout* out) {
    if (!out) return fail("irs_slab_plan_layout: null argument");
    SlabInfo s;
    if (plan_layout(cfg, scfg, rank, world, &s)) return 1;
    *out = irs_slab_layout{s.rank, s.world, s.a, s.b, s.lo, s.hi, s.margin, s.gmax};
    return 0;
}

int irs_slab_create(const irs_config* cfg, const irs_slab_config* scfg, irs_comm* comm, irs_ctx** out) {
    if (!cfg || !out) return fail("irs_slab_create: null argument");
    const int world = comm ? comm->world : 1, rank = comm ? comm->rank : 0;
    if (cfg->no_steps > kMaxSteps) return fail("irs_slab_create: at most %d squaring steps", kMaxSteps);
    SlabInfo s;
    if (plan_layout(cfg, scfg, rank, world, &s)) return 1;
    const int ls = cfg->data_loss == IRS_DATA_GMM_LCC ? cfg->lcc_s : 0;
    if (world > 1 && (s.margin < cfg->sobolev_s + 1 || s.margin < 4 * ls || s.margin < 2))
        return fail("irs_slab_create: margin %d too small for the stencils (Sobolev %d, LCC %d)", s.margin, cfg->sobolev_s, ls);
    if (world > 1 && (s.min_slab < cfg->sobolev_s + 1 || s.min_slab < 4 * ls))
        return fail("irs_slab_create: slabs of %d planes are thinner than the stencil halos: fewer ranks", s.min_slab);
    irs_ctx* c = nullptr;
    if (create_ctx(cfg, &s, &c)) return 1;
    c->comm = comm;
    if (comm && world > 1) {
        const size_t xbytes = (size_t)3 * c->C * s.margin * c->vol.H * c->vol.W * sizeof(float);
        size_t arbytes = sizeof(double) * (kStatVals > 2 * IRS_MAX_CHAINS ? kStatVals : 2 * IRS_MAX_CHAINS);
        const size_t bounds = sizeof(unsigned) * 4 * c->C * (cfg->no_steps + 1);
        arbytes = bounds > arbytes ? bounds : arbytes;
        if (c->ffd && sizeof(float) * c->C * 3 * c->volv.V > arbytes) arbytes = sizeof(float) * c->C * 3 * c->volv.V;
        if (comm_reserve(comm, xbytes, arbytes)) {
            irs_destroy(c);
            return 1;
        }
        const unsigned* ef = comm_error_flag(comm);
        if (ef && hipMemcpy((char*)c->state + offsetof(DevState, comm_err), &ef, sizeof(ef), hipMemcpyHostToDevice) != hipSuccess) {
            irs_destroy(c);
            return fail("irs_slab_create: publishing the transport's error word failed");
        }
    }
    int prio_least = 0, prio_greatest = 0;
    (void)hipDeviceGetStreamPriorityRange(&prio_least, &prio_greatest);
    hipError_t e = hipStreamCreateWithPriority(&c->cs, hipStreamNonBlocking, prio_greatest);
    if (e == hipSuccess) e = hipHostMalloc((void**)&c->plan_hint, sizeof(unsigned) * 2 * kHintWords, hipHostMallocDefault);
    if (e == hipSuccess)
        for (int i = 0; i < 2 * kHintWords; ++i) c->plan_hint[i] = (i % kHintWords) < kHintWords - 8 ? 0x7f800000u : 0u;
    for (int i = 0; i < 28 && e == hipSuccess; ++i) e = hipEventCreateWithFlags(&c->sev[i], hipEventDisableTiming);
    if (e != hipSuccess) {
        irs_destroy(c);
        return fail("irs_slab_create: stream / event creation failed: %s", hipGetErrorString(e));
    }
    c->have_pred = false;
    *out = c;
    return 0;
}

// ... 315 lines not shown
```

### ir_sgmcmc_amd/engine.py

```python
import ctypes as C
import math
from dataclasses import dataclass, field
from typing import Optional, Sequence, Tuple

import torch
from scipy.special import digamma

from . import _lib as L
from .ops import control_grid_size, sobolev_kernel_1d


@dataclass
class EngineConfig:
    dims: Tuple[int, int, int]
    no_chains: int = 1
    cps: Optional[Tuple[int, int, int]] = None
    no_steps: int = 12
    sobolev_s: int = 3
    sobolev_lambda: float = 0.5
    lr: float = 0.4
    uniform_noise: float = 0.1
    virtual_decimation: bool = True
    data_loss: str = 'GMM'
    gmm_components: int = 4
    lcc_s: int = 1
    ssd_sigma: float = 0.1
    gmm_lr_log_std: float = 0.2
    gmm_lr_logits: float = 0.2
    gmm_lr_decay: float = 0.001
    scale_prior: Tuple[float, float] = (0.0, 2.3)
    dirichlet_alpha: Sequence[float] = field(default_factory=lambda: [0.5])
    reg_loss: str = 'RegLoss_L2'
    w_reg: float = 1.4
    student: Tuple[float, float] = (1e-6, 2e-6)
    reg_learnable: bool = False
    reg_lr: Tuple[float, float] = (0.01, 0.01)
    reg_lr_decay: float = 0.001
    loc_prior_nu: float = 1.0
    loc_prior_w_reg: Optional[float] = None
    reg_scale_prior: Tuple[float, float] = (2.8, 5.0)
    seed: int = 0

    @property
    def dims_v(self):
        return control_grid_size(self.dims, self.cps) if self.cps else tuple(self.dims)

    @property
    def dof(self):
        return float(self.dims[0] * self.dims[1] * self.dims[2]) * 3.0


def lognormal_init(w_reg, dof, nu=1.0):
    loc = float(digamma(0.5 * nu * dof)) - math.log(0.5 * nu * w_reg)
    return loc, math.log(4.0) + math.log(loc)


def irs_config(cfg: EngineConfig):
    c = L.IrsConfig()
    c.dims[:] = list(cfg.dims)
    c.cps[:] = list(cfg.cps) if cfg.cps else [0, 0, 0]
    c.no_chains, c.no_steps = cfg.no_chains, cfg.no_steps
    c.sobolev_s = cfg.sobolev_s or 0
    if c.sobolev_s:
        k = sobolev_kernel_1d(cfg.sobolev_s, cfg.sobolev_lambda)
        for i, x in enumerate(k):
            c.sobolev_kernel[i] = float(x)
    c.lr = cfg.lr
    c.uniform_alpha = cfg.uniform_noise or 0.0
    c.virtual_decimation = int(cfg.virtual_decimation)
    c.data_loss = L.IRS_DATA_GMM_LCC if cfg.data_loss == 'GMM' else L.IRS_DATA_SSD
    c.lcc_s, c.gmm_components, c.ssd_sigma = cfg.lcc_s, cfg.gmm_components, cfg.ssd_sigma
    c.gmm_lr_log_std, c.gmm_lr_logits, c.gmm_lr_decay = cfg.gmm_lr_log_std, cfg.gmm_lr_logits, cfg.gmm_lr_decay
    c.adam_beta1, c.adam_beta2, c.adam_eps = 0.9, 0.999, 1e-8
    c.scale_prior_loc, c.scale_prior_scale = cfg.scale_prior
    conc = list(cfg.dirichlet_alpha)
    if len(conc) == 1:
        conc = conc * cfg.gmm_components
    for i, x in enumerate(conc):
        c.dirichlet_concentration[i] = float(x)
    c.reg_loss = {'RegLoss_L2': L.IRS_REG_L2, 'RegLoss_LogNormal': L.IRS_REG_LOGNORMAL, 'RegLoss_Student': L.IRS_REG_STUDENT,
                  'RegLoss_LogNormal_L2': L.IRS_REG_LOGNORMAL_L2}[cfg.reg_loss]
    c.reg_learnable = int(cfg.reg_learnable)
    c.w_reg, c.dof = cfg.w_reg, cfg.dof
    c.reg_lr0, c.reg_lr1, c.reg_lr_decay = cfg.reg_lr[0], cfg.reg_lr[1], cfg.reg_lr_decay
    c.loc_prior_nu = cfg.loc_prior_nu
    c.loc_prior_w_reg = cfg.w_reg if cfg.loc_prior_w_reg is None else cfg.loc_prior_w_reg
    c.reg_scale_prior_loc, c.reg_scale_prior_scale = cfg.reg_scale_prior
    shape = 0.5 * cfg.dof
    c.w_reg_prior_shape, c.w_reg_prior_rate = shape, 1.0 / shape
    if cfg.reg_loss == 'RegLoss_Student':
        c.w_reg_prior_shape, c.w_reg_prior_rate = float(cfg.student[0]), float(cfg.student[1])
    c.seed = cfg.seed
    return c


def _on_device(fn):
    import functools

    @functools.wraps(fn)
    def wrapped(self, *a, **k):
        with torch.cuda.device(self.device):
            return fn(self, *a, **k)
    return wrapped


class TransitionEngine:
    def __init__(self, cfg: EngineConfig, device='cuda:0'):
        self.cfg = cfg
        self.device = torch.device(device)
        self.lib = L.load()
        self._c = c = irs_config(cfg)
        with torch.cuda.device(self.device):
            self._ctx = self._create(c)
        self._keep = {}
        if cfg.reg_loss == 'RegLoss_LogNormal':
            st = self.state()
            st.reg_param[0], st.reg_param[1] = lognormal_init(cfg.w_reg, cfg.dof)
            self.set_state(st)

    def _stream(self):
        return C.c_void_p(torch.cuda.current_stream(self.device).cuda_stream)

    def _create(self, c):
        ctx = C.c_void_p()
        L.check(self.lib.irs_create(C.byref(c), C.byref(ctx)))
        return ctx

    def __del__(self):
        ctx, self._ctx = getattr(self, '_ctx', None), None
        if ctx:
            try:
                self.lib.irs_destroy(ctx)
            except Exception:
                pass

    def option(self, name, value):
        L.option_set(name, value, self._ctx)

    @_on_device
    def flush(self):
        L.check(self.lib.irs_flush(self._ctx, self._stream()))

    @property
    def recovered_transitions(self):
        n = C.c_uint64()
        L.check(self.lib.irs_recovered_transitions(self._ctx, C.byref(n)))
        return int(n.value)

    def set_sparse_adjoint(self, on):
        L.check(self.lib.irs_sparse_adjoint_set(self._ctx, int(bool(on))))

    @_on_device
    def sparse_adjoint(self):
        n, ch = self.cfg.no_steps, self.cfg.no_chains
        buf = (C.c_int32 * (n * ch * 4))()
        L.check(self.lib.irs_sparse_adjoint_get(self._ctx, buf, self._stream()))
        keys = ('engaged', 'piece_len', 'pieces', 'run_planes')
        return [[dict(zip(keys, buf[(k * ch + c) * 4:(k * ch + c) * 4 + 4])) for c in range(ch)] for k in range(n)]

    def set_sparse_data(self, on):
        L.check(self.lib.irs_sparse_data_set(self._ctx, int(on)))

    @_on_device
    def sparse_data(self):
        ch = self.cfg.no_chains
        buf = (C.c_int32 * (4 * ch * 4))()
        L.check(self.lib.irs_sparse_data_get(self._ctx, buf, self._stream()))
        keys = ('engaged', 'piece_len', 'pieces', 'run_planes')
        return {name: [dict(zip(keys, buf[(k * ch + c) * 4:(k * ch + c) * 4 + 4])) for c in range(ch)]
                for k, name in enumerate(('warp', 'map', 'stats', 'data_term'))}

    @property
    def workspace_bytes(self):
        return int(self.lib.irs_workspace_bytes(self._ctx))

    @_on_device
    def state(self):
        st = L.IrsState()
        L.check(self.lib.irs_get_state(self._ctx, C.byref(st), self._stream()))
        return st

    @_on_device
    def set_state(self, st):
        L.check(self.lib.irs_set_state(self._ctx, C.byref(st), self._stream()))

    @_on_device
    def scalars(self):
        sc = L.IrsScalars()
        L.check(self.lib.irs_get_scalars(self._ctx, C.byref(sc), self._stream()))
        n = self.cfg.no_chains
        return {k: [getattr(sc, k)[i] for i in range(n)] for k in ('alpha', 'data_term', 'reg_term', 'reg_energy', 'n_mask')}

    def _io(self, fixed, moving, v, sigma=None, eps=None, unif=None, outputs=None):
        io = L.IrsIO()
        f_im, m_im, mask = fixed['im'], moving['im'], fixed['mask']
        io.fixed_im, io.moving_im = L.dev_ptr(f_im, torch.float32), L.dev_ptr(m_im, torch.float32)
        io.mask = L.dev_ptr(mask, torch.bool)
        io.fixed_chains, io.moving_chains, io.mask_chains = f_im.shape[0], m_im.shape[0], mask.shape[0]
        io.v = L.dev_ptr(v, torch.float32, allow_none=True)
        io.sigma = L.dev_ptr(sigma, torch.float32, allow_none=True)
        io.eps = L.dev_ptr(eps, torch.float32, allow_none=True)
        io.unif = L.dev_ptr(unif, torch.float32, allow_none=True)
        for k in ('curr_state', 'im_moving_warped', 'residuals', 'displacement', 'transformation', 'grad_v'):
            t = (outputs or {}).get(k)
            setattr(io, k, L.dev_ptr(t, torch.float32, allow_none=True))
        return io

    @staticmethod
    def _base(t):
        if t.dim() == 5 and t.stride(0) == 0 and t.shape[0] > 1:
            t = t[:1]
        return t.contiguous()

    @_on_device
    def prepare(self, fixed, moving):
        fixed = {k: self._base(v) for k, v in fixed.items() if k in ('im', 'mask')}
        moving = {k: self._base(v) for k, v in moving.items() if k in ('im',)}
        self._keep['fixed'], self._keep['moving'] = fixed, moving
        L.check(self.lib.irs_set_fixed(self._ctx, L.dev_ptr(fixed['im'], torch.float32), fixed['im'].shape[0],
                                       self._stream()))
        return fixed, moving

    @_on_device
    def gmm_init(self, fixed, moving, v_sample=None, warm_up=25):
        io = self._io(fixed, moving, None)
        L.check(self.lib.irs_gmm_init(self._ctx, C.byref(io), L.dev_ptr(v_sample, torch.float32, allow_none=True),
                                      warm_up, self._stream()))

    @_on_device
    def transition(self, fixed, moving, v, sigma=None, eps=None, unif=None, outputs=None, timed=False):
        io = self._io(fixed, moving, v, sigma, eps, unif, outputs)
        if timed:
            tm = L.IrsTimings()
            L.check(self.lib.irs_transition_timed(self._ctx, C.byref(io), self._stream(), C.byref(tm)))
            return {n: getattr(tm, n) for n, _ in tm._fields_}
        L.check(self.lib.irs_transition(self._ctx, C.byref(io), self._stream()))
        return None
```

Before: 259.4 transitions/s.

## Restrict SVF forward scaling-and-squaring steps to mask-reachable tile runs

Adds a forward plan, built from the data mask extents and per-step ghost widths derived from the displacement bound hints, which lists only the tile/z-run pieces whose outputs can influence masked voxels at later steps. The forward exp march kernel gets a plan variant that iterates those list entries instead of all dense segments. This is meant to skip forward integration work outside the region that matters for the data term, at the cost of extra plan-building launches, extra workspace, and reliance on the hint bounds being conservative.

```diff
diff --git a/include/irsgmcmc.h b/include/irsgmcmc.h
--- a/include/irsgmcmc.h
+++ b/include/irsgmcmc.h
@@ -354,6 +354,8 @@
 int irs_sparse_adjoint_get(irs_ctx* ctx, int32_t* out, void* stream);
 int irs_sparse_data_set(irs_ctx* ctx, int on);
 int irs_sparse_data_get(irs_ctx* ctx, int32_t* out, void* stream);
+int irs_sparse_forward_set(irs_ctx* ctx, int on);
+int irs_sparse_forward_get(irs_ctx* ctx, int32_t* out, void* stream);
 
 typedef struct irs_timings {
     float total_ms;
diff --git a/ir_sgmcmc_amd/_lib.py b/ir_sgmcmc_amd/_lib.py
--- a/ir_sgmcmc_amd/_lib.py
+++ b/ir_sgmcmc_amd/_lib.py
@@ -237,6 +237,8 @@
     'irs_sparse_adjoint_get': [_P, _I32P, _P],
     'irs_sparse_data_set': [_P, _I],
     'irs_sparse_data_get': [_P, _I32P, _P],
+    'irs_sparse_forward_set': [_P, _I],
+    'irs_sparse_forward_get': [_P, _I32P, _P],
     'irs_transition_timed': [_P, C.POINTER(IrsIO), _P, C.POINTER(IrsTimings)],
     'irs_comm_unique_id': [C.POINTER(C.c_uint8 * IRS_COMM_ID_BYTES)],
     'irs_comm_create_rccl': [C.POINTER(C.c_uint8 * IRS_COMM_ID_BYTES), _I, _I, C.POINTER(_P)],
diff --git a/ir_sgmcmc_amd/csrc/adjoint_plan.h b/ir_sgmcmc_amd/csrc/adjoint_plan.h
--- a/ir_sgmcmc_amd/csrc/adjoint_plan.h
+++ b/ir_sgmcmc_amd/csrc/adjoint_plan.h
@@ -20,6 +20,7 @@
 constexpr int kPlanMinLen = 8;
 constexpr int kPlanMinForced = 4;
 constexpr int kPlanStats = 4;
+constexpr int kForwardStats = 5;
 
 struct PlanEntry {
     int chain, tile, z0, z1, fill, pad;
@@ -70,14 +71,23 @@
 constexpr int kWarpTX = 64, kWarpTY = 8;
 constexpr int kDataKernels = 4;
 enum PlanFill { kFillNext = 0, kFillAll = 1, kFillNone = 2 };
+constexpr int kPlanMaxLists = 32;
 struct PlanShape {
     int tx, ty;
     int reach0, reach_dec;
     int fill[2];
     int G[2];
     int lmin;
+    int n_reach;
+    int reach[kPlanMaxLists];
 };
-IRS_HD int plan_reach(const PlanShape& s, int k) { return s.reach0 - k * s.reach_dec; }
+IRS_HD int plan_reach(const PlanShape& s, int k) { return s.n_reach > 0 ? s.reach[k] : s.reach0 - k * s.reach_dec; }
+
+IRS_HD int plan_forward_reach(const int* h, int n, int S, int k) {
+    int m = 3 * S;
+    for (int i = k + 1; i < n; ++i) m += h[i];
+    return m;
+}
 IRS_HD int plan_fill_of(const PlanShape& s, int k) { return s.fill[k > 0 ? 1 : 0]; }
 IRS_HD int plan_resident_of(const PlanShape& s, int k) { return s.G[k > 0 ? 1 : 0]; }
 IRS_HD void plan_tile_window(int t, int size, int m, int n, int& a, int& b) {
diff --git a/ir_sgmcmc_amd/csrc/adjoint_plan.hip b/ir_sgmcmc_amd/csrc/adjoint_plan.hip
--- a/ir_sgmcmc_amd/csrc/adjoint_plan.hip
+++ b/ir_sgmcmc_amd/csrc/adjoint_plan.hip
@@ -190,15 +190,15 @@
     size_t ext, runs, colplan, entries, count, stats, total;
     int cap, ntx, nty;
 };
-static PlanLayout plan_layout(Vol vol, int C, int no_steps) {
+static PlanLayout plan_layout(Vol vol, int C, int no_steps, int tx = kPlanTX, int ty = kPlanTY, bool own_ext = true) {
     PlanLayout l;
-    l.ntx = (vol.W + kPlanTX - 1) / kPlanTX;
-    l.nty = (vol.H + kPlanTY - 1) / kPlanTY;
+    l.ntx = (vol.W + tx - 1) / tx;
+    l.nty = (vol.H + ty - 1) / ty;
     const size_t cols = (size_t)C * l.ntx * l.nty;
     l.cap = plan_entries_cap((int)cols, vol.D);
     size_t off = 0;
     auto take = [&](size_t bytes) { const size_t o = off; off += plan_align(bytes); return o; };
-    l.ext = take(sizeof(int) * 2 * (size_t)C * vol.H * vol.W);
+    l.ext = take(own_ext ? sizeof(int) * 2 * (size_t)C * vol.H * vol.W : 0);
     l.runs = take(sizeof(int) * 2 * cols * no_steps);
     l.colplan = take(sizeof(ColPlan) * cols * no_steps);
     l.entries = take(sizeof(PlanEntry) * (size_t)l.cap * no_steps);
@@ -210,10 +210,9 @@
 
 size_t adjoint_plan_bytes(Vol vol, int C, int no_steps) { return plan_layout(vol, C, no_steps).total; }
 
-AdjointPlan adjoint_plan_views(char* base, Vol vol, int C, int no_steps) {
-    const PlanLayout l = plan_layout(vol, C, no_steps);
+static AdjointPlan plan_views(char* base, const PlanLayout& l, bool own_ext) {
     AdjointPlan p;
-    p.ext = (int*)(base + l.ext);
+    p.ext = own_ext ? (int*)(base + l.ext) : nullptr;
     p.runs = (int*)(base + l.runs);
     p.colplan = (ColPlan*)(base + l.colplan);
     p.entries = (PlanEntry*)(base + l.entries);
@@ -224,6 +223,7 @@
     p.nty = l.nty;
     return p;
 }
+AdjointPlan adjoint_plan_views(char* base, Vol vol, int C, int no_steps) { return plan_views(base, plan_layout(vol, C, no_steps), true); }
 
 void launch_adjoint_plan(const float* g_warped, const unsigned* dmax, const AdjointPlan& plan, int no_steps, int C, Vol vol,
                          int64_t G, int forced_len, hipStream_t st) {
@@ -233,6 +233,24 @@
     hipLaunchKernelGGL(plan_runs_kernel, dim3((unsigned)(C * plan.ntx * plan.nty), (unsigned)no_steps), dim3(kWave), 0, st, plan.ext, C, dmax,
                        plan.runs, vol, C, no_steps, plan.ntx, plan.nty, shape);
     hipLaunchKernelGGL(plan_lists_kernel, dim3((unsigned)no_steps), dim3(kPlanBlock), 0, st, plan.runs, dmax, plan.colplan, plan.entries, plan.count,
+                       plan.stats, vol, C, no_steps, plan.ntx, plan.nty, plan.cap, shape, forced_len);
+}
+
+size_t forward_plan_bytes(Vol vol, int C, int no_steps) { return plan_layout(vol, C, no_steps, kWarpTX, kWarpTY, false).total; }
+AdjointPlan forward_plan_views(char* base, Vol vol, int C, int no_steps) {
+    return plan_views(base, plan_layout(vol, C, no_steps, kWarpTX, kWarpTY, false), false);
+}
+int forward_plan_run_bound(const AdjointPlan& plan, int C, Vol vol, int64_t G, int forced_len) {
+    return plan_run_bound(C * plan.ntx * plan.nty, vol.D, (int)(G > 0 ? G : 1024), forced_len);
+}
+void launch_forward_plan(const int* ext, int ext_chains, const AdjointPlan& plan, const int* width, int S, int no_steps, int C, Vol vol,
+                         int64_t G, int forced_len, hipStream_t st) {
+    const int g = (int)(G > 0 ? G : 1024);
+    PlanShape shape{kWarpTX, kWarpTY, 0, 0, {kFillNone, kFillNone}, {g, g}, kPlanMinLen, no_steps, {}};
+    for (int k = 0; k < no_steps && k < kPlanMaxLists; ++k) shape.reach[k] = plan_forward_reach(width, no_steps, S, k);
+    hipLaunchKernelGGL(plan_runs_kernel, dim3((unsigned)(C * plan.ntx * plan.nty), (unsigned)no_steps), dim3(kWave), 0, st, ext, ext_chains, nullptr,
+                       plan.runs, vol, C, no_steps, plan.ntx, plan.nty, shape);
+    hipLaunchKernelGGL(plan_lists_kernel, dim3((unsigned)no_steps), dim3(kPlanBlock), 0, st, plan.runs, nullptr, plan.colplan, plan.entries, plan.count,
                        plan.stats, vol, C, no_steps, plan.ntx, plan.nty, plan.cap, shape, forced_len);
 }
 
diff --git a/ir_sgmcmc_amd/csrc/api_ctx.hip b/ir_sgmcmc_amd/csrc/api_ctx.hip
--- a/ir_sgmcmc_amd/csrc/api_ctx.hip
+++ b/ir_sgmcmc_amd/csrc/api_ctx.hip
@@ -45,6 +45,7 @@
     c->kn = global_knobs();
     c->sparse_adjoint = true;
     c->sparse_data = 1;
+    c->sparse_forward = 1;
     c->cfg = *cfg;
     c->C = C;
     c->vol = make_vol(D, H, W);
@@ -117,6 +118,7 @@
     const bool planned = !sl;
     const size_t o_plan = take(planned ? adjoint_plan_bytes(c->vol, C, cfg->no_steps) : 0);
     const size_t o_dplan = take(planned ? data_plan_bytes(c->vol, C) : 0);
+    const size_t o_fplan = take(planned && !c->ffd ? forward_plan_bytes(c->vol, C, cfg->no_steps) : 0);
     const size_t o_state = take(sizeof(DevState));
     c->slab_bytes = off;
     if (hipMalloc((void**)&c->slab, off) != hipSuccess) {
@@ -151,6 +153,7 @@
     c->cmm = (float*)(c->slab + o_cmm);
     if (planned) c->plan = adjoint_plan_views(c->slab + o_plan, c->vol, C, cfg->no_steps);
     if (planned) c->dplan = data_plan_views(c->slab + o_dplan, c->vol, C);
+    if (planned && !c->ffd) c->fplan = forward_plan_views(c->slab + o_fplan, c->vol, C, cfg->no_steps);
     c->state = (DevState*)(c->slab + o_state);
 
     if (ensure_lin_tables(c->lin, D, H, W, nullptr)) {
@@ -289,7 +292,7 @@
 }
 
 static int forward_pass(irs_ctx* c, const irs_io* io, const float* v, bool with_noise, bool with_jitter, float* vs,
-                        float* warped, float* z, float* gradm, int chains, hipStream_t st, int timed, int data_on = 0) {
+                        float* warped, float* z, float* gradm, int chains, hipStream_t st, int timed, int data_on = 0, bool fwd_lists = false) {
     const irs_config& cfg = c->cfg;
     const int C = chains;
     const uint64_t* it = &c->state->st.iteration;
@@ -322,8 +325,12 @@
     for (int k = 0; k < cfg.no_steps; ++k) {
         const float* in = k == 0 ? dense : c->steps + (int64_t)(k - 1) * field;
         float* out = c->steps + (int64_t)k * field;
-        launch_exp_step_fwd_march(in, out, k == 0, cfg.no_steps, C, c->vol, lin, c->dmax + (int64_t)k * c->C * 4,
-                                  c->dmax + (int64_t)(k + 1) * c->C * 4, predicted_small(c, k), fwd_lay(c, k), st);
+        if (fwd_lists)
+            launch_exp_step_fwd_plan(in, out, k == 0, cfg.no_steps, C, c->vol, lin, c->dmax + (int64_t)(k + 1) * c->C * 4, fwd_lay(c, k), c->fplan, k,
+                                     c->sparse_forward > 1 ? c->sparse_forward : 0, st);
+        else
+            launch_exp_step_fwd_march(in, out, k == 0, cfg.no_steps, C, c->vol, lin, c->dmax + (int64_t)k * c->C * 4,
+                                      c->dmax + (int64_t)(k + 1) * c->C * 4, predicted_small(c, k), fwd_lay(c, k), st);
     }
     if (timed) HIP_TRY(hipEventRecord(c->ev[2], st));
     const float* d_last = c->steps + (int64_t)(cfg.no_steps - 1) * field;
@@ -404,7 +411,24 @@
         launch_data_plan(io->mask, io->mask_chains, c->dplan, lcc ? cfg.lcc_s : 0, lcc, C, vol, st);
     }
     c->data_on = data_on;
-    if (forward_pass(c, io, io->v, true, cfg.uniform_alpha > 0.0f, vs, warped, z, fuse_warp_bwd ? c->gA : nullptr, C, st, timed, data_on)) return 1;
+    const int fwd_forced = c->sparse_forward > 1 ? c->sparse_forward : 0;
+    bool fwd_on = c->sparse_forward != 0 && data_on > 0 && c->fplan.entries != nullptr && !c->ffd && !io->transformation && !io->displacement &&
+                  c->kn.predict_variants == 1 && !no_assumptions && !is_capturing(st) && c->hint != nullptr && cfg.no_steps <= kPlanMaxLists &&
+                  (fwd_forced > 0 || exp_fwd_dense_allows_lists(vol, C));
+    for (int k = 0; k < cfg.no_steps && fwd_on; ++k) {
+        bool valid;
+        const float m = hint_row_max(c->hint + (size_t)k * C * 4, C * 4, &valid);
+        const int h = !valid ? -1 : c->kn.slab_force_h > 0 ? c->kn.slab_force_h : ghost_width_from_bound(m, true);
+        fwd_on = skip_any[k] && h >= 1 && h <= 255;
+        c->fwd_width[k] = h;
+    }
+    c->fwd_on = fwd_on;
+    if (fwd_on) {
+        for (int k = 0; k < cfg.no_steps; ++k) vd.width[k] = (unsigned char)c->fwd_width[k];
+        launch_forward_plan(c->dplan.ext, io->mask_chains, c->fplan, c->fwd_width, lcc ? cfg.lcc_s : 0, cfg.no_steps, C, vol, exp_fwd_plan_resident(),
+                            fwd_forced, st);
+    }
+    if (forward_pass(c, io, io->v, true, cfg.uniform_alpha > 0.0f, vs, warped, z, fuse_warp_bwd ? c->gA : nullptr, C, st, timed, data_on, fwd_on)) return 1;
     const int64_t field = (int64_t)C * 3 * vol.V;
     const float* d_last = c->steps + (int64_t)(cfg.no_steps - 1) * field;
     if (io->transformation || io->displacement) launch_svf_outputs(d_last, io->transformation, io->displacement, C, vol, lin, st);
@@ -586,6 +610,31 @@
     return 0;
 }
 
+int irs_sparse_forward_set(irs_ctx* c, int on) {
+    if (!c) return fail("irs_sparse_forward_set: null argument");
+    if (on < 0) return fail("irs_sparse_forward_set: 0 (off), 1 (on) or a piece length");
+    c->sparse_forward = on;
+    return 0;
+}
+
+int irs_sparse_forward_get(irs_ctx* c, int32_t* out, void* stream) {
+    if (!c || !out) return fail("irs_sparse_forward_get: null argument");
+    const int n = c->cfg.no_steps, C = c->C;
+    memset(out, 0, (size_t)n * C * kForwardStats * sizeof(int32_t));
+    if (!c->fplan.stats || !c->fwd_on || c->n_enqueued == 0) return 0;
+    int width[32];
+    memcpy(width, c->fwd_width, sizeof(width));
+    if (irs_flush(c, stream)) return 1;
+    int32_t stats[32 * IRS_MAX_CHAINS * kPlanStats];
+    HIP_TRY(hipMemcpyAsync(stats, c->fplan.stats, (size_t)n * C * kPlanStats * sizeof(int32_t), hipMemcpyDeviceToHost, (hipStream_t)stream));
+    HIP_TRY(hipStreamSynchronize((hipStream_t)stream));
+    for (int i = 0; i < n * C; ++i) {
+        memcpy(out + (size_t)i * kForwardStats, stats + (size_t)i * kPlanStats, sizeof(int32_t) * kPlanStats);
+        out[(size_t)i * kForwardStats + kPlanStats] = width[i / C];
+    }
+    return 0;
+}
+
 int irs_sparse_data_set(irs_ctx* c, int on) {
     if (!c) return fail("irs_sparse_data_set: null argument");
     if (on < 0) return fail("irs_sparse_data_set: 0 (off), 1 (on) or a piece length");
diff --git a/ir_sgmcmc_amd/csrc/ctx.h b/ir_sgmcmc_amd/csrc/ctx.h
--- a/ir_sgmcmc_amd/csrc/ctx.h
+++ b/ir_sgmcmc_amd/csrc/ctx.h
@@ -1,4 +1,5 @@
 #pragma once
+#include <math.h>
 #include <stdlib.h>
 #include <string.h>
 
@@ -58,6 +59,10 @@
     irs::DataPlan dplan;
     int sparse_data = 1;
     int data_on = 0;
+    irs::AdjointPlan fplan;
+    int sparse_forward = 1;
+    bool fwd_on = false;
+    int fwd_width[32] = {};
     float* cmm;
     unsigned* hint = nullptr;
     irs::DevState* state;
@@ -125,6 +130,11 @@
     return m;
 }
 
+inline int ghost_width_from_bound(float m, bool safety) {
+    if (!(m >= 0.0f) || m > 1.0e6f) return -1;
+    return (int)floorf(safety ? 1.25f * m + 0.25f : m) + 1;
+}
+
 inline bool predicted_below(const irs_ctx* c, int k, float bound) {
     const int mode = c->kn.predict_variants;
     if (mode == 2 || mode == 3) return true;
diff --git a/ir_sgmcmc_amd/csrc/exp_kernels.hip b/ir_sgmcmc_amd/csrc/exp_kernels.hip
--- a/ir_sgmcmc_amd/csrc/exp_kernels.hip
+++ b/ir_sgmcmc_amd/csrc/exp_kernels.hip
@@ -1218,29 +1218,34 @@
 #else
 #define IRS_TR(slot)
 #endif
-template <bool PRESCALE, int R, int FROWS, int PF>
+template <bool PRESCALE, int R, int FROWS, int PF, bool PLAN = false>
 __device__ __forceinline__ void exp_fwd_march_tile(const float* __restrict__ din, float* __restrict__ dout, const Vol vol,
                                                    const Lin lin, const Scale3L sc, const unsigned* __restrict__ dmax_in,
                                                    unsigned* __restrict__ dmax_out, const int seg_len, const int nseg,
                                                    const int h_lo, const int h_hi, const int swz_run, const int tile_id,
-                                                   const dim3 tiles, const int lay) {
+                                                   const dim3 tiles, const int lay, const PlanEntry piece = PlanEntry{}) {
     using M = MarchF<R, FROWS>;
     constexpr int PX = M::PX, PN = M::PN, NIT = M::NIT, PITCH = M::PITCH, PNP = M::PNP, kFwdBlock = M::kFwdBlock;
     constexpr int NS = M::NP + 1;
     __shared__ float2 r_xy[NS * PNP];
     __shared__ float r_z[NS * PNP];
     __shared__ float red[3 * (kFwdBlock / kWave)];
-    const int tile_ = xcd_swizzle_runs(tile_id, (int)(tiles.x * tiles.y * tiles.z), swz_run);
+    const int tile_ = PLAN ? piece.tile : xcd_swizzle_runs(tile_id, (int)(tiles.x * tiles.y * tiles.z), swz_run);
     const int tbx = tile_ % tiles.x, tby = (tile_ / tiles.x) % tiles.y, tbz = tile_ / (tiles.x * tiles.y);
-    const int chain = tbz / nseg, seg = tbz % nseg;
-    if (dmax_in) {
+    const int chain = PLAN ? piece.chain : tbz / nseg, seg = tbz % nseg;
+    if (!PLAN && dmax_in) {
         const int need = max(max((int)ceilf(__uint_as_float(dmax_in[chain * 4 + 0])), (int)ceilf(__uint_as_float(dmax_in[chain * 4 + 1]))),
                              (int)ceilf(__uint_as_float(dmax_in[chain * 4 + 2])));
         if (need <= h_lo || need > h_hi) return;
     }
     const int ox = tbx * FTX, oy = tby * FTY;
     int z0, z1;
-    seg_range(vol, seg, seg_len, z0, z1);
+    if (PLAN) {
+        z0 = piece.z0;
+        z1 = piece.z1;
+    } else {
+        seg_range(vol, seg, seg_len, z0, z1);
+    }
     const int64_t V = vol.V;
     const int64_t cb = (int64_t)chain * 3 * V;
     auto run = [&](auto LC) {
@@ -1473,8 +1478,38 @@
     }
 }
 
-void launch_exp_step_fwd_march(const float* din, float* dout, bool prescale_in, int no_steps, int C, Vol vol, Lin lin,
-                               const unsigned* dmax_in, unsigned* dmax_out, bool only_r1, int lay, hipStream_t st) {
+static_assert(FTX == kWarpTX && FTY == kWarpTY, "the forward lists are cut over the forward tile's columns");
+template <bool PRESCALE>
+__global__ __launch_bounds__(FTX * FTY / FROWS_BIG, IRS_FWD_WAVES) void exp_fwd_march_plan_kernel(
+    const float* __restrict__ din, float* __restrict__ dout, Vol vol, Lin lin, Scale3L sc, unsigned* __restrict__ dmax_out,
+    const PlanEntry* __restrict__ entries, const int* __restrict__ count, int cap, int swz_run, dim3 tiles, int lay) {
+    const int id = (int)blockIdx.x, group = 8 * swz_run;
+    const int g = swz_run > 1 ? id / group : 0, w = id - g * group;
+    const int swz = swz_run > 1 ? g * group + (w & 7) * swz_run + (w >> 3) : id;
+    const PlanEntry e_swz = entries[min(swz, cap - 1)], e_plain = entries[min(id, cap - 1)];
+    const int n_run = count[1];
+    if (id >= n_run) return;
+    exp_fwd_march_tile<PRESCALE, 1, FROWS_BIG, 1, true>(din, dout, vol, lin, sc, nullptr, dmax_out, 0, 1, 0, 0, 0, id, tiles, lay,
+                                                        plan_swizzle(id, n_run, swz_run) == id ? e_plain : e_swz);
+}
+int64_t exp_fwd_plan_resident() {
+    static int cache = 0;
+    return resident_blocks((const void*)exp_fwd_march_plan_kernel<false>, FTX * FTY / FROWS_BIG, &cache);
+}
+void launch_exp_step_fwd_plan(const float* din, float* dout, bool prescale_in, int no_steps, int C, Vol vol, Lin lin, unsigned* dmax_out, int lay,
+                              const AdjointPlan& plan, int step, int forced_len, hipStream_t st) {
+    const dim3 tiles((vol.W + FTX - 1) / FTX, (vol.H + FTY - 1) / FTY, 1);
+    const Scale3L sc = make_scale_l(vol, no_steps);
+    const int swz_env = global_knobs().swz_run;
+    const int swz_run = swz_env >= 0 ? swz_env : (int)tiles.x;
+    const int grid = forward_plan_run_bound(plan, C, vol, exp_fwd_plan_resident(), forced_len);
+    with_bool(prescale_in, [&](auto P) {
+        hipLaunchKernelGGL((exp_fwd_march_plan_kernel<decltype(P)::value>), dim3((unsigned)(grid > 0 ? grid : 1)), dim3(FTX * FTY / FROWS_BIG), 0, st, din,
+                           dout, vol, lin, sc, dmax_out, plan.entries + (int64_t)step * plan.cap, plan.count + 2 * step, plan.cap, swz_run, tiles, lay);
+    });
+}
+
+static int exp_fwd_dense_seg_len(Vol vol, int C, bool* small_out) {
     const int seg_env = global_knobs().march_seg_fwd;
     const int64_t per_layer = (int64_t)((vol.W + FTX - 1) / FTX) * ((vol.H + FTY - 1) / FTY) * C;
     int seg_len = pick_seg_len(vol.nz + vol.nzb, per_layer, 8, seg_env);
@@ -1486,6 +1521,21 @@
                                   : resident_blocks((const void*)exp_fwd_march_kernel<false, 1, FROWS_BIG, 1>, FTX * FTY / FROWS_BIG, &cache_big);
         if (res > 0) seg_len = pick_seg_len_fit(vol.nz, vol.nzb, per_layer, 8, 2, res, 0);
     }
+    *small_out = small;
+    return seg_len;
+}
+bool exp_fwd_dense_allows_lists(Vol vol, int C) {
+    bool small;
+    const int seg_len = exp_fwd_dense_seg_len(vol, C, &small);
+    return !small && seg_len > kPlanMinLen;
+}
+
+void launch_exp_step_fwd_march(const float* din, float* dout, bool prescale_in, int no_steps, int C, Vol vol, Lin lin,
+                               const unsigned* dmax_in, unsigned* dmax_out, bool only_r1, int lay, hipStream_t st) {
+    const int seg_env = global_knobs().march_seg_fwd;
+    const int64_t per_layer = (int64_t)((vol.W + FTX - 1) / FTX) * ((vol.H + FTY - 1) / FTY) * C;
+    bool small;
+    const int seg_len = exp_fwd_dense_seg_len(vol, C, &small);
     const int nseg = vol_nseg(vol, seg_len);
     const dim3 tiles((vol.W + FTX - 1) / FTX, (vol.H + FTY - 1) / FTY, (unsigned)(nseg * C));
     const int total = (int)(tiles.x * tiles.y * tiles.z);
diff --git a/ir_sgmcmc_amd/csrc/kernels.h b/ir_sgmcmc_amd/csrc/kernels.h
--- a/ir_sgmcmc_amd/csrc/kernels.h
+++ b/ir_sgmcmc_amd/csrc/kernels.h
@@ -70,6 +70,15 @@
 AdjointPlan adjoint_plan_views(char* base, Vol vol, int C, int no_steps);
 void launch_adjoint_plan(const float* g_warped, const unsigned* dmax, const AdjointPlan& plan, int no_steps, int C, Vol vol,
                          int64_t G, int forced_len, hipStream_t st);
+size_t forward_plan_bytes(Vol vol, int C, int no_steps);
+AdjointPlan forward_plan_views(char* base, Vol vol, int C, int no_steps);
+void launch_forward_plan(const int* ext, int ext_chains, const AdjointPlan& plan, const int* width, int S, int no_steps, int C, Vol vol,
+                         int64_t G, int forced_len, hipStream_t st);
+int forward_plan_run_bound(const AdjointPlan& plan, int C, Vol vol, int64_t G, int forced_len);
+void launch_exp_step_fwd_plan(const float* din, float* dout, bool prescale, int no_steps, int C, Vol vol, Lin lin, unsigned* dmax_out, int lay,
+                              const AdjointPlan& plan, int step, int forced_len, hipStream_t st);
+int64_t exp_fwd_plan_resident();
+bool exp_fwd_dense_allows_lists(Vol vol, int C);
 struct DataPlan {
     int* ext = nullptr;
     int* runs = nullptr;
diff --git a/ir_sgmcmc_amd/csrc/slab.hip b/ir_sgmcmc_amd/csrc/slab.hip
--- a/ir_sgmcmc_amd/csrc/slab.hip
+++ b/ir_sgmcmc_amd/csrc/slab.hip
@@ -648,11 +648,6 @@
         return vd;
     }
 };
-
-int ghost_width_from_bound(float m, bool safety) {
-    if (!(m >= 0.0f) || m > 1.0e6f) return -1;
-    return (int)floorf(safety ? 1.25f * m + 0.25f : m) + 1;
-}
 
 float hint_bound(const irs_ctx* c, const unsigned* slot, int k) {
     bool valid;
diff --git a/ir_sgmcmc_amd/engine.py b/ir_sgmcmc_amd/engine.py
--- a/ir_sgmcmc_amd/engine.py
+++ b/ir_sgmcmc_amd/engine.py
@@ -170,6 +170,17 @@
         return {name: [dict(zip(keys, buf[(k * ch + c) * 4:(k * ch + c) * 4 + 4])) for c in range(ch)]
                 for k, name in enumerate(('warp', 'map', 'stats', 'data_term'))}
 
+    def set_sparse_forward(self, on):
+        L.check(self.lib.irs_sparse_forward_set(self._ctx, int(on)))
+
+    @_on_device
+    def sparse_forward(self):
+        n, ch = self.cfg.no_steps, self.cfg.no_chains
+        buf = (C.c_int32 * (n * ch * 5))()
+        L.check(self.lib.irs_sparse_forward_get(self._ctx, buf, self._stream()))
+        keys = ('engaged', 'piece_len', 'pieces', 'run_planes', 'width')
+        return [[dict(zip(keys, buf[(k * ch + c) * 5:(k * ch + c) * 5 + 5])) for c in range(ch)] for k in range(n)]
+
     @property
     def workspace_bytes(self):
         return int(self.lib.irs_workspace_bytes(self._ctx))
```

New measurement: 271.6 transitions/s (median of 6 runs). 4.7% higher.
